# martinruenz/maskfusion

Measured on NVIDIA H100. Metric: frames/sec on 640x480 .klg replay, higher is better.
Workload: dtype f32

## Files before the change

maskfusion_b200/csrc/mf_capi.cu:

```cuda
#include "mf_host.h"
#include <string.h>
#include <stdio.h>
#include <zlib.h>
#include <limits.h>
#include <new>
#include <stack>

using namespace mfb;
namespace mfb { bool decodeJPEG(const uint8_t* data, size_t size, int& W, int& H, std::vector<uint8_t>& rgb, std::string& err); }

struct mf_context { MaskFusion* mf; };

static thread_local std::string g_err;
extern "C" const char* mf_last_error(void) { return g_err.c_str(); }
void mf_set_error(const std::string& e) { g_err = e; }
extern "C" int mf_abi_version(void) { return MF_ABI_VERSION; }

#define MF_TRY try {
#define MF_CATCH(ret)                                                              \
    } catch (const CudaError& e) { g_err = e.what; return ret; }                   \
    catch (const std::exception& e) { g_err = e.what(); return ret; }              \
    catch (...) { g_err = "unknown error"; return ret; }
static int mf_finalise(mf_context* ctx)
{
    try {
        cudaCheck(cudaSetDevice(ctx->mf->device), "cudaSetDevice");
        ctx->mf->finalisePending(); return 0;
    }
    catch (const CudaError& e) { g_err = e.what; return -1; }
    catch (...) { g_err = "unknown error"; return -1; }
}
#define MF_NEED(ctx) if (!(ctx) || !(ctx)->mf) { g_err = "null context"; return -1; } if (mf_finalise(ctx) != 0) return -1;
#define MF_MODEL(ctx, i) if ((i) < 0 || (i) >= (int)(ctx)->mf->models.size()) { g_err = "model index out of range"; return -2; } Model* m = (ctx)->mf->models[i].get();

#define MF_OWNED(m) if (!(m)->owned) { g_err = "model is owned by another rank (sharded mode): no device buffers here"; return -4; }

static Mat4 fromColMajor(const float* p) { Mat4 r; for (int rr = 0; rr < 4; ++rr) for (int c = 0; c < 4; ++c) r.m[rr * 4 + c] = p[c * 4 + rr]; return r; }
static void toColMajor(const Mat4& T, float* p) { for (int rr = 0; rr < 4; ++rr) for (int c = 0; c < 4; ++c) p[c * 4 + rr] = T.m[rr * 4 + c]; }

extern "C" void mf_config_defaults(mf_config* c, int width, int height)
{
    memset(c, 0, sizeof *c);
    c->width = width; c->height = height;
    if (width == 640 && height == 480) { c->fx = 528; c->fy = 528; c->cx = 320; c->cy = 240; }
    else { c->fx = 528.f * width / 640.f; c->fy = c->fx; c->cx = width / 2.f; c->cy = height / 2.f; }
    c->depthCutoff = 4.0f; c->maxDepthProcessed = 20.0f; c->icpWeight = 20.0f;
    c->rgbOnly = 0; c->pyramid = 1; c->fastOdom = 0; c->so3 = 1; c->frameToFrameRGB = 0;
    c->confGlobal = 10.0f; c->confObject = 0.01f;
    c->timeDelta = INT_MAX / 2;
    c->outlierCoeff = 0.1f;
    c->capacityGlobal = 3072 * 3072; c->capacityObject = 1024 * 1024;
    c->enableMultipleModels = 0; c->trackAllModels = 0; c->modelSpawnOffset = 22;
    c->minRelSizeNew = 0.015f; c->maxRelSizeNew = 0.4f;
    c->segThreshold = 0.3f; c->segWeightDistance = 150.f; c->segWeightConvexity = 2.8f;
    c->segMorphEdgeIterations = 0; c->segMorphEdgeRadius = 1; c->segMorphMaskIterations = 0; c->segMorphMaskRadius = 2;
}

extern "C" mf_context* mf_create(const mf_config* cfg, int device, void* stream)
{
    MF_TRY
    if (!cfg) { g_err = "null config"; return nullptr; }
    int n = 0;
    cudaError_t e = cudaGetDeviceCount(&n);
    if (e != cudaSuccess || n == 0) { g_err = std::string("no CUDA device: this library has no CPU fallback (") + cudaGetErrorString(e) + ")"; return nullptr; }
    mf_context* c = new mf_context;
    c->mf = new MaskFusion(*cfg, device, (cudaStream_t)stream);
    return c;
    MF_CATCH(nullptr)
}
extern "C" void mf_destroy(mf_context* ctx) { if (ctx) { delete ctx->mf; delete ctx; } }

extern "C" int mf_process_frame(mf_context* ctx, const uint8_t* rgb, const float* depth, int64_t ts, const uint8_t* mask, const float* in_pose,
                                float weight_multiplier, int bootstrap)
{
    MF_TRY MF_NEED(ctx)
    if (!rgb || !depth || ts < 0) { g_err = "processFrame: rgb/depth must be non-null and timestamp >= 0 (MaskFusion.cpp:201-203)"; return -3; }
    Mat4 ip; if (in_pose) ip = fromColMajor(in_pose);
    ctx->mf->processFrame(rgb, depth, ts, mask, in_pose ? &ip : nullptr, weight_multiplier, bootstrap != 0, false);
    return 0;
    MF_CATCH(-1)
}
extern "C" int mf_process_frame_device(mf_context* ctx, const void* d_rgb, const void* d_depth, int64_t ts, const void* d_mask, const float* in_pose,
                                       float weight_multiplier, int bootstrap)
{
    MF_TRY MF_NEED(ctx)
    if (!d_rgb || !d_depth || ts < 0) { g_err = "processFrame: rgb/depth must be non-null and timestamp >= 0"; return -3; }
    Mat4 ip; if (in_pose) ip = fromColMajor(in_pose);
    ctx->mf->processFrame((const uint8_t*)d_rgb, (const float*)d_depth, ts, (const uint8_t*)d_mask, in_pose ? &ip : nullptr, weight_multiplier,
                          bootstrap != 0, true);
    return 0;
    MF_CATCH(-1)
}
extern "C" int mf_set_input_event(mf_context* ctx, void* ev) { if (!ctx || !ctx->mf) { g_err = "null context"; return -1; } ctx->mf->inputReady = (cudaEvent_t)ev; return 0; }
extern "C" int mf_sync(mf_context* ctx) { MF_TRY MF_NEED(ctx) ctx->mf->sync(); return 0; MF_CATCH(-1) }
extern "C" int mf_tick(mf_context* ctx) { if (!ctx || !ctx->mf) return -1; return ctx->mf->tick; }
extern "C" int64_t mf_kernel_launches(mf_context* ctx) { if (!ctx || !ctx->mf) return -1; return ctx->mf->launches; }

extern "C" int mf_model_count(mf_context* ctx) { if (!ctx || !ctx->mf) return -1; return (int)ctx->mf->models.size(); }
extern "C" int mf_model_id(mf_context* ctx, int i) { MF_NEED(ctx) MF_MODEL(ctx, i) return m->id; }
extern "C" int mf_get_pose(mf_context* ctx, int i, float* p) { MF_NEED(ctx) MF_MODEL(ctx, i) toColMajor(m->pose, p); return 0; }
extern "C" int mf_set_pose(mf_context* ctx, int i, const float* p) { MF_NEED(ctx) MF_MODEL(ctx, i) m->overridePose(fromColMajor(p)); return 0; }
extern "C" int mf_model_set_conf_threshold(mf_context* ctx, int i, float t) { MF_NEED(ctx) MF_MODEL(ctx, i) m->confidenceThreshold = t; return 0; }
extern "C" int mf_model_surfel_count(mf_context* ctx, int i) { MF_TRY MF_NEED(ctx) MF_MODEL(ctx, i) return (int)m->lastCount(); MF_CATCH(-1) }

extern "C" int mf_download_surfels(mf_context* ctx, int i, float* out, int max_surfels)
{
    MF_TRY MF_NEED(ctx) MF_MODEL(ctx, i) MF_OWNED(m)
    MaskFusion* o = ctx->mf;
    uint32_t n = m->lastCount();
    if ((int)n > max_surfels) n = (uint32_t)max_surfels;
    if (!n) return 0;
    DevBuf<float4> tmp; tmp.alloc((size_t)n * 3);
    launch_planes_to_aos(m->current(), n, tmp, o->stream);
    cudaCheck(cudaMemcpyAsync(out, tmp.p, (size_t)n * 48, cudaMemcpyDeviceToHost, o->stream), "surfel D2H");
    o->sync();
    return (int)n;
    MF_CATCH(-1)
}
extern "C" int mf_upload_surfels(mf_context* ctx, int i, const float* in, int n)
{
    MF_TRY MF_NEED(ctx) MF_MODEL(ctx, i) MF_OWNED(m)
    MaskFusion* o = ctx->mf;
    if (n < 0 || (uint32_t)n > m->capacity) { g_err = "upload exceeds model capacity"; return -4; }
    if (n) {
        DevBuf<float4> tmp; tmp.alloc((size_t)n * 3);
        cudaCheck(cudaMemcpyAsync(tmp.p, in, (size_t)n * 48, cudaMemcpyHostToDevice, o->stream), "surfel H2D");
        launch_aos_to_planes(tmp, (uint32_t)n, m->current(), o->stream);
        o->sync();
    }
    uint32_t c = (uint32_t)n;
    cudaCheck(cudaMemcpyAsync(m->dCount(), &c, sizeof c, cudaMemcpyHostToDevice, o->stream), "count H2D");
    o->sync();
    return 0;
    MF_CATCH(-1)
}
extern "C" int mf_pose_log_size(mf_context* ctx, int i) { MF_NEED(ctx) MF_MODEL(ctx, i) return (int)(m->poseLog.size() / 8); }
extern "C" int mf_get_pose_log(mf_context* ctx, int i, double* out8, int max_entries)
{
    MF_NEED(ctx) MF_MODEL(ctx, i)
    int n = (int)(m->poseLog.size() / 8); if (n > max_entries) n = max_entries;
    memcpy(out8, m->poseLog.data(), (size_t)n * 8 * sizeof(double));
    return n;
}

extern "C" int mf_export_poses(mf_context* ctx, const char* export_dir)
{
    MF_TRY MF_NEED(ctx)
    if (!export_dir) { g_err = "export_poses: null directory"; return -2; }
    ctx->mf->sync();
    int written = 0;
    std::vector<Model*> all;
    for (auto& m : ctx->mf->models) all.push_back(m.get());
    for (auto& m : ctx->mf->inactiveModels) all.push_back(m.get());
    for (Model* m : all) {
        const std::string filename = std::string(export_dir) + "poses-" + std::to_string((int)m->id) + ".txt";
        FILE* fp = fopen(filename.c_str(), "w");
        if (!fp) { g_err = "cannot write " + filename; return -3; }
        for (size_t e = 0; e + 8 <= m->poseLog.size(); e += 8) {
            fprintf(fp, "%.6f", m->poseLog[e] * 1e-6);
            for (int k = 1; k < 8; ++k) fprintf(fp, " %.6f", (double)(float)m->poseLog[e + k]);
            fprintf(fp, "\n");
        }
        fclose(fp);
        ++written;
    }
    return written;
    MF_CATCH(-1)
}

extern "C" int mf_set_frame(mf_context* ctx, const uint8_t* rgb, const float* depth, const uint8_t* mask)
{
    MF_TRY MF_NEED(ctx)
    MaskFusion* o = ctx->mf;
    if (!mask) o->mask.zero(o->stream);
    o->setFrame(rgb, depth, mask, false);
    o->generateCUDATextures();
    return 0;
    MF_CATCH(-1)
}
extern "C" int mf_model_perform_tracking(mf_context* ctx, int i, float* transform16)
{
    MF_TRY MF_NEED(ctx) MF_MODEL(ctx, i) MF_OWNED(m)
    std::vector<Model*> ms{m};
    ctx->mf->trackModels(ms);
    ctx->mf->finalisePending();
    if (transform16) toColMajor(m->lastTransform, transform16);
    return 0;
    MF_CATCH(-1)
}
extern "C" int mf_model_predict_indices(mf_context* ctx, int i, int time)
{
    MF_TRY MF_NEED(ctx) MF_MODEL(ctx, i) MF_OWNED(m)
    m->predictIndices(time, ctx->mf->cfg.maxDepthProcessed, ctx->mf->cfg.timeDelta); return 0;
    MF_CATCH(-1)
}
extern "C" int mf_model_fuse(mf_context* ctx, int i, int time, float depth_cutoff, float weight_multiplier)
{
    MF_TRY MF_NEED(ctx) MF_MODEL(ctx, i) MF_OWNED(m)
    m->fuse(time, depth_cutoff, weight_multiplier); return 0;
    MF_CATCH(-1)
}
extern "C" int mf_model_clean(mf_context* ctx, int i, int time)
{
    MF_TRY MF_NEED(ctx) MF_MODEL(ctx, i) MF_OWNED(m)
    m->clean(time, ctx->mf->cfg.timeDelta, ctx->mf->cfg.maxDepthProcessed); return 0;
    MF_CATCH(-1)
}
extern "C" int mf_model_combined_predict(mf_context* ctx, int i, int time, int max_time)
{
    MF_TRY MF_NEED(ctx) MF_MODEL(ctx, i) MF_OWNED(m)
    m->combinedPredict(ctx->mf->cfg.maxDepthProcessed, time, max_time, ctx->mf->cfg.timeDelta); return 0;
    MF_CATCH(-1)
}
extern "C" int mf_model_init_from_frame(mf_context* ctx, int i, int time)
{
    MF_TRY MF_NEED(ctx) MF_MODEL(ctx, i) MF_OWNED(m)
    m->initialise(time); return 0;
    MF_CATCH(-1)
}

template <typename T>
static void d2h(MaskFusion* o, void* dst, const T* src, size_t n)
{
    if (!dst) return;
    cudaCheck(cudaMemcpyAsync(dst, src, n * sizeof(T), cudaMemcpyDeviceToHost, o->stream), "D2H");
}
static void planarOut(MaskFusion* o, const float4* map, int P, float* out)
{
    if (!out) return;
    launch_map_to_planar(map, P, o->scratch, o->stream);
    cudaCheck(cudaMemcpyAsync(out, o->scratch.p, (size_t)P * 3 * sizeof(float), cudaMemcpyDeviceToHost, o->stream), "D2H");
    o->sync();
}
extern "C" int mf_download_filtered_depth(mf_context* ctx, float* out)
{
    MF_TRY MF_NEED(ctx) d2h(ctx->mf, out, ctx->mf->depthFilt, ctx->mf->P); ctx->mf->sync(); return 0; MF_CATCH(-1)
}
extern "C" int mf_download_frame_maps(mf_context* ctx, int level, float* depth, float* vmap, float* nmap)
{
    MF_TRY MF_NEED(ctx)
    MaskFusion* o = ctx->mf;
    if (level < 0 || level > 2) { g_err = "level out of range"; return -2; }
    int Pl = (o->W >> level) * (o->H >> level);
    d2h(o, depth, level == 0 ? o->depthFilt : o->depthPyr[level].p, Pl); o->sync();
    planarOut(o, o->vmap[level], Pl, vmap);
    planarOut(o, o->nmap[level], Pl, nmap);
    return 0;
    MF_CATCH(-1)
}
extern "C" int mf_download_model_maps(mf_context* ctx, int i, int level, float* vmap, float* nmap)
{
    MF_TRY MF_NEED(ctx) MF_MODEL(ctx, i) MF_OWNED(m)
    MaskFusion* o = ctx->mf;
    if (level < 0 || level > 2) { g_err = "level out of range"; return -2; }
    int Pl = (o->W >> level) * (o->H >> level);
    planarOut(o, m->vmapG[level], Pl, vmap);
    planarOut(o, m->nmapG[level], Pl, nmap);
    return 0;
    MF_CATCH(-1)
}
extern "C" int mf_download_index_map(mf_context* ctx, int i, uint32_t* idx, float* vc, float* ct, float* nr)
{
    MF_TRY MF_NEED(ctx) MF_MODEL(ctx, i) MF_OWNED(m)
    MaskFusion* o = ctx->mf;
    m->flushIndex();
    d2h(o, idx, m->idx.p, o->P); d2h(o, vc, m->vertConf.p, o->P); d2h(o, ct, m->colorTime.p, o->P); d2h(o, nr, m->normRad.p, o->P);
    o->sync(); return 0;
    MF_CATCH(-1)
}
extern "C" int mf_download_prediction(mf_context* ctx, int i, uint8_t* image4, float* vc, float* nr, uint16_t* time)
{
    MF_TRY MF_NEED(ctx) MF_MODEL(ctx, i) MF_OWNED(m)
    MaskFusion* o = ctx->mf;
    d2h(o, image4, m->splatImage.p, o->P); d2h(o, vc, m->splatVertex.p, o->P); d2h(o, nr, m->splatNormal.p, o->P); d2h(o, time, m->splatTime.p, o->P);
    o->sync(); return 0;
    MF_CATCH(-1)
}
extern "C" int mf_download_fill_in(mf_context* ctx, int i, uint8_t* image4, float* v4, float* n4)
{
    MF_TRY MF_NEED(ctx) MF_MODEL(ctx, i) MF_OWNED(m)
    MaskFusion* o = ctx->mf;
    if (!m->fillIn) { g_err = "model has no fill-in textures"; return -5; }
    d2h(o, image4, m->fillImage.p, o->P); d2h(o, v4, m->fillVertex.p, o->P); d2h(o, n4, m->fillNormal.p, o->P);
    o->sync(); return 0;
    MF_CATCH(-1)
}
extern "C" int mf_download_association(mf_context* ctx, int i, uint8_t* flag, uint32_t* best, float* meas12)
{
    MF_TRY MF_NEED(ctx) MF_MODEL(ctx, i) MF_OWNED(m)
    MaskFusion* o = ctx->mf;
    d2h(o, flag, m->aflag.p, o->P); d2h(o, best, m->abest.p, o->P);
    if (meas12) {
        DevBuf<float4> tmp; tmp.alloc((size_t)o->P * 3);
        launch_planes_to_aos(SurfelPlanes{m->meas[0].p, m->meas[1].p, m->meas[2].p}, (uint32_t)o->P, tmp, o->stream);
        cudaCheck(cudaMemcpyAsync(meas12, tmp.p, (size_t)o->P * 48, cudaMemcpyDeviceToHost, o->stream), "D2H");
        o->sync();
    }
    o->sync(); return 0;
    MF_CATCH(-1)
}
extern "C" int mf_download_track_stats(mf_context* ctx, int i, double* A36, double* b6, float* err6)
{
    MF_TRY MF_NEED(ctx) MF_MODEL(ctx, i) MF_OWNED(m)
    MaskFusion* o = ctx->mf;
    TrackState st;
    cudaCheck(cudaMemcpyAsync(&st, m->trackState.p, sizeof st, cudaMemcpyDeviceToHost, o->stream), "D2H");
    o->sync();
    if (A36) memcpy(A36, st.lastA, sizeof st.lastA);
    if (b6) memcpy(b6, st.lastb, sizeof st.lastb);
    if (err6) { err6[0] = st.lastICPError; err6[1] = st.lastICPCount; err6[2] = st.lastRGBError; err6[3] = st.lastRGBCount; err6[4] = st.lastSO3Error; err6[5] = st.lastSO3Count; }
    return 0;
    MF_CATCH(-1)
}
extern "C" int mf_download_edge_map(mf_context* ctx, float* edge, uint8_t* binary)
{
    MF_TRY MF_NEED(ctx)
    MaskFusion* o = ctx->mf;
    if (!o->frameMapsValid) o->generateCUDATextures();
    launch_geometric_edges(o->vmap[0], o->nmap[0], o->W, o->H, o->cfg.segWeightDistance, o->cfg.segWeightConvexity, o->cfg.segThreshold,
                           o->edgeMap, o->edgeBinary, o->stream);
    launch_morph_close_invert(o->edgeBinary, o->edgeBuf, o->W, o->H, o->cfg.segMorphEdgeRadius, o->cfg.segMorphEdgeIterations, o->edgeInv, o->stream);
    o->launches += 2 + 2 * o->cfg.segMorphEdgeIterations;
    d2h(o, edge, o->edgeMap.p, o->P); d2h(o, binary, o->edgeInv.p, o->P);
    o->sync(); return 0;
    MF_CATCH(-1)
}

extern "C" int mf_morph_close(mf_context* ctx, uint8_t* image, int radius, int iterations, int ellipse, uint8_t* inverted)
{
    MF_TRY MF_NEED(ctx)
    if (!image || radius < 0 || iterations < 0) { g_err = "morph_close: bad arguments"; return -3; }
    MaskFusion* o = ctx->mf;
    DevBuf<uint8_t> a, b, c; a.alloc(o->P); b.alloc(o->P); c.alloc(o->P);
    cudaCheck(cudaMemcpyAsync(a.p, image, o->P, cudaMemcpyHostToDevice, o->stream), "H2D");
    if (ellipse) o->launches += launch_morph_close_ellipse(a, b, o->W, o->H, radius, iterations, nullptr, o->stream);
    else { launch_morph_close_invert(a, b, o->W, o->H, radius, iterations, c, o->stream); o->launches += 1 + 2 * iterations; }
    d2h(o, image, a.p, o->P);
    if (inverted && !ellipse) d2h(o, inverted, c.p, o->P);
    o->sync(); return 0;
    MF_CATCH(-1)
}

extern "C" int mf_attach_backbone(mf_context* ctx, void* backbone, int every_k)
{
    MF_TRY MF_NEED(ctx)
    ctx->mf->attachBackbone(backbone, every_k); return 0;
    MF_CATCH(-1)
}

extern "C" int mf_attach_detector(mf_context* ctx, mf_detector* detector, int every_k)
{
    MF_TRY MF_NEED(ctx)
    ctx->mf->attachDetector(detector, every_k); return 0;
    MF_CATCH(-1)
}
extern "C" int mf_download_frame_masks(mf_context* ctx, uint8_t* mask, int32_t* class_ids_256, int* n_masks)
{
    MF_TRY MF_NEED(ctx)
    MaskFusion* o = ctx->mf;
    if (!o->cfg.enableMultipleModels) { g_err = "not a multi-model context"; return -5; }
    FrameHdr h;
    cudaCheck(cudaMemcpyAsync(&h, o->dHdr, sizeof h, cudaMemcpyDeviceToHost, o->stream), "D2H");
    d2h(o, mask, o->frameMask, o->P);
    o->sync();
    if (mask && h.nMasks == 0) memset(mask, 0, o->P);
    if (class_ids_256) memcpy(class_ids_256, h.classIDs, sizeof h.classIDs);
    if (n_masks) *n_masks = h.nMasks;
    return 0;
    MF_CATCH(-1)
}

extern "C" int mf_debug_track_timing(int64_t* out, int cap) { return debug_track_timing((long long*)out, cap); }

extern "C" int mf_set_frame_classes(mf_context* ctx, const int32_t* class_ids, int n)
{
    MF_TRY MF_NEED(ctx)
    if (n < 0 || n > 256) { g_err = "class id list must have 0..256 entries"; return -3; }
    ctx->mf->setFrameClasses(class_ids, n);
    return 0;
    MF_CATCH(-1)
}
extern "C" int mf_download_segmentation(mf_context* ctx, uint8_t* mask, uint8_t* projected_ids)
{
    MF_TRY MF_NEED(ctx)
    MaskFusion* o = ctx->mf;
    d2h(o, mask, o->mask.p, o->P);
    if (projected_ids) { if (!o->projectedIDs.p) { g_err = "not a multi-model context"; return -5; } d2h(o, projected_ids, o->projectedIDs.p, o->P); }
    o->sync(); return 0;
    MF_CATCH(-1)
}
extern "C" int mf_shard_configure(mf_context* ctx, int rank, int world) { MF_TRY MF_NEED(ctx) ctx->mf->configureShard(rank, world); return 0; MF_CATCH(-1) }
extern "C" int mf_shard_frame_begin(mf_context* ctx, const void* rgb, const void* depth, int64_t ts, const void* mask, int on_device)
{
    MF_TRY MF_NEED(ctx)
    if (!rgb || !depth || ts < 0) { g_err = "frame_begin: rgb/depth must be non-null and timestamp >= 0"; return -3; }
    ctx->mf->frameBegin((const uint8_t*)rgb, (const float*)depth, ts, (const uint8_t*)mask, nullptr, false, on_device != 0);
    return 0;
    MF_CATCH(-1)
}
extern "C" int mf_shard_get_poses(mf_context* ctx, float* out, int capacity_models)
{
    MF_TRY MF_NEED(ctx)
    if (capacity_models < MF_MAX_MODELS) { g_err = "get_poses: the buffer must hold 64 rows of 32 floats"; return -2; }
    ctx->mf->getShardPoses(out);
    return (int)ctx->mf->models.size();
    MF_CATCH(-1)
}
extern "C" int mf_shard_unique_id(uint8_t* out128)
{
    MF_TRY
    if (!out128) { g_err = "null buffer"; return -1; }
    shardUniqueId(out128); return 0;
    MF_CATCH(-1)
}
extern "C" int mf_shard_comm_init(mf_context* ctx, const uint8_t* id128, int rank, int world)
{
    MF_TRY MF_NEED(ctx)
    if (!id128) { g_err = "null id"; return -1; }
    ctx->mf->initShardComm(id128, rank, world); return 0;
    MF_CATCH(-1)
}
extern "C" int mf_shard_process_frame(mf_context* ctx, const uint8_t* rgb, const float* depth, int64_t ts, const uint8_t* mask, const int32_t* class_ids,
                                      int n_class_ids, float weight_multiplier, int inputs_on_device)
{
    MF_TRY MF_NEED(ctx)
    MaskFusion* o = ctx->mf;
    if (!o->shardNccl) { g_err = "mf_shard_process_frame needs a communicator (mf_shard_comm_init)"; return -2; }
    if (o->rank == 0) {
        if (!rgb || !depth || ts < 0) { g_err = "processFrame: rgb/depth must be non-null and timestamp >= 0 on the loader rank"; return -3; }
        if (n_class_ids < 0 || n_class_ids > 256) { g_err = "class id list must have 0..256 entries"; return -3; }
        o->setFrameClasses(class_ids, class_ids ? n_class_ids : 0);
    }
    o->processFrame(rgb, depth, ts, mask, nullptr, weight_multiplier, false, inputs_on_device != 0);
    return 0;
    MF_CATCH(-1)
}
extern "C" int mf_shard_stats(mf_context* ctx, int64_t* out4)
{
    if (!ctx || !ctx->mf || !out4) { g_err = "null argument"; return -1; }
    MaskFusion* o = ctx->mf;
    out4[0] = (int64_t)o->shard.bytesMoved; out4[1] = o->shard.calls; out4[2] = o->shardNccl ? o->shard.world : 0; out4[3] = o->shard.version;
    return 0;
}
extern "C" int mf_shard_set_poses(mf_context* ctx, const float* gathered) { MF_TRY MF_NEED(ctx) ctx->mf->setShardPoses(gathered); return 0; MF_CATCH(-1) }
extern "C" int mf_shard_project(mf_context* ctx) { MF_TRY MF_NEED(ctx) ctx->mf->frameProject(); return 0; MF_CATCH(-1) }
extern "C" void* mf_shard_projection_keys(mf_context* ctx) { if (!ctx || !ctx->mf) return nullptr; return ctx->mf->projKeys.p; }
extern "C" int mf_shard_frame_end(mf_context* ctx, float weight_multiplier) { MF_TRY MF_NEED(ctx) ctx->mf->frameEnd(weight_multiplier); return 0; MF_CATCH(-1) }
extern "C" int mf_shard_attach_detector(mf_context* ctx, mf_detector* detector, int every_k, int detector_rank)
{
    MF_TRY MF_NEED(ctx)
    ctx->mf->attachShardDetector(detector, every_k, detector_rank); return 0;
    MF_CATCH(-1)
}
extern "C" int mf_shard_frame_masks(mf_context* ctx, void** d_ptr, size_t* bytes)
{
    MF_TRY MF_NEED(ctx)
    if (!d_ptr || !bytes) { g_err = "frame_masks: null output"; return -3; }
    void* p = nullptr; size_t n = 0;
    if (!ctx->mf->shardFrameMasks(&p, &n)) return 0;
    *d_ptr = p; *bytes = n;
    return 1;
    MF_CATCH(-1)
}
extern "C" int mf_model_owner(mf_context* ctx, int i) { MF_NEED(ctx) MF_MODEL(ctx, i) return m->ownerRank; }
extern "C" int mf_track_shares(int n_jobs, unsigned light_mask, int total_ctas, int ratio, int* shares)
{
    if (!shares || n_jobs < 1 || n_jobs > TRACK_MAX_JOBS || total_ctas < n_jobs) return -1;
    track_shares(n_jobs, light_mask, total_ctas, ratio, shares);
    return 0;
}
extern "C" int mf_shard_pick_owner(const int64_t* loads, int world) { if (!loads || world < 1 || world > 64) return -1; return MaskFusion::pickOwner(loads, world); }

extern "C" int mf_model_class_id(mf_context* ctx, int i) { MF_NEED(ctx) MF_MODEL(ctx, i) return m->classID; }
extern "C" int mf_set_profiling(mf_context* ctx, int on)
{
    MF_TRY MF_NEED(ctx)
    ctx->mf->sync();
    ctx->mf->prof.on = on != 0; ctx->mf->prof.used = 0;
    if (on) ctx->mf->prof.acc.clear();
    return 0;
    MF_CATCH(-1)
}
extern "C" int mf_get_stage_times(mf_context* ctx, char* buf, int bufsize)
{
    MF_TRY MF_NEED(ctx)
    ctx->mf->sync();
    std::string out;
    char line[256];
    for (auto& kv : ctx->mf->prof.acc) { snprintf(line, sizeof line, "%s %ld %.6f\n", kv.first.c_str(), kv.second.first, kv.second.second); out += line; }
    if ((int)out.size() + 1 > bufsize) { g_err = "buffer too small"; return -6; }
    memcpy(buf, out.c_str(), out.size() + 1);
    return (int)out.size();
    MF_CATCH(-1)
}
extern "C" int mf_debug_set_poses(mf_context* ctx, int i, const float* pose16, const float* last16)
{
    MF_NEED(ctx) MF_MODEL(ctx, i)
    m->pose = fromColMajor(pose16); m->lastPose = fromColMajor(last16);
    m->pushPose();
    return 0;
}
extern "C" int mf_icp_step(mf_context* ctx, int i, int level, const float* Rcurr9, const float* tcurr3, float* out29)
{
    MF_TRY MF_NEED(ctx) MF_MODEL(ctx, i) MF_OWNED(m)
    MaskFusion* o = ctx->mf;
    if (level < 0 || level > 2) { g_err = "level out of range"; return -2; }
    TrackPoses pp; memset(&pp, 0, sizeof pp);
    memcpy(pp.p[0], Rcurr9, 9 * sizeof(float)); memcpy(pp.p[0] + 9, tcurr3, 3 * sizeof(float));
    const float* P = m->pose.m;
    float R[9] = {P[0], P[1], P[2], P[4], P[5], P[6], P[8], P[9], P[10]};
    float c00 = R[4] * R[8] - R[5] * R[7], c01 = R[5] * R[6] - R[3] * R[8], c02 = R[3] * R[7] - R[4] * R[6];
    float det = (R[0] * c00 + R[1] * c01) + R[2] * c02, id = 1.0f / det;
    float Ri[9] = {c00 * id, (R[2] * R[7] - R[1] * R[8]) * id, (R[1] * R[5] - R[2] * R[4]) * id,
                   c01 * id, (R[0] * R[8] - R[2] * R[6]) * id, (R[2] * R[3] - R[0] * R[5]) * id,
                   c02 * id, (R[1] * R[6] - R[0] * R[7]) * id, (R[0] * R[4] - R[1] * R[3]) * id};
    memcpy(pp.p[1], Ri, sizeof Ri); pp.p[1][9] = P[3]; pp.p[1][10] = P[7]; pp.p[1][11] = P[11];
    DevBuf<float> out; out.alloc(32);
    DevBuf<unsigned> ticket; ticket.alloc(1); ticket.zero(o->stream);
    launch_icp_only(o->vmap[level], o->nmap[level], m->vmapG[level], m->nmapG[level], o->W >> level, o->H >> level, camLevel(o->cam, level), pp,
                    m->partial, ticket, out, o->numSMs, o->stream);
    o->launches += 1;
    cudaCheck(cudaMemcpyAsync(out29, out.p, 29 * sizeof(float), cudaMemcpyDeviceToHost, o->stream), "D2H");
    o->sync();
    return 0;
    MF_CATCH(-1)
}

struct mf_klg {
    FILE* fp; int W, H, numFrames, currentFrame; int flip;
    std::vector<unsigned char> dbuf, rbuf, dec;
};
extern "C" mf_klg* mf_klg_open(const char* path, int width, int height, int flip_colors)
{
    if (!path) { g_err = "mf_klg_open: null path"; return nullptr; }
    if (width <= 0 || height <= 0 || width > 16384 || height > 16384) { g_err = "mf_klg_open: width/height must be in 1..16384"; return nullptr; }
    FILE* fp = fopen(path, "rb");
    if (!fp) { g_err = std::string("Could not open log-file: ") + path; return nullptr; }
    int32_t n = 0;
    if (!fread(&n, sizeof(int32_t), 1, fp)) { fclose(fp); g_err = std::string("Could not open log-file: ") + path; return nullptr; }
    mf_klg* k = nullptr;
    try {
        k = new mf_klg;
        k->fp = fp; k->W = width; k->H = height; k->numFrames = n; k->currentFrame = 0; k->flip = flip_colors;
        size_t P = (size_t)width * height;
        k->dbuf.resize(P * 2 + 1024); k->rbuf.resize(P * 3 + 1024); k->dec.resize(P * 2);
    } catch (...) { fclose(fp); delete k; g_err = "mf_klg_open: out of memory"; return nullptr; }
    return k;
}
extern "C" int mf_klg_num_frames(mf_klg* k) { return k ? k->numFrames : -1; }
extern "C" int mf_klg_has_more(mf_klg* k) { return k ? (k->currentFrame + 1 < k->numFrames) : 0; }
extern "C" int mf_klg_get_next(mf_klg* k, uint8_t* rgb, float* depth, int64_t* timestamp)
{
    if (!k || !rgb || !depth) { g_err = "mf_klg_get_next: null reader or output buffer"; return -1; }
    MF_TRY
    const size_t P = (size_t)k->W * k->H;
    int64_t ts; int32_t dsz, rsz;
    if (!fread(&ts, sizeof ts, 1, k->fp) || !fread(&dsz, sizeof dsz, 1, k->fp) || !fread(&rsz, sizeof rsz, 1, k->fp)) { g_err = "klg: truncated frame header"; return -2; }
    if (dsz < 0 || rsz < 0 || (size_t)dsz > k->dbuf.size() || (size_t)rsz > k->rbuf.size()) { g_err = "klg: implausible frame sizes"; return -3; }
    if (dsz && !fread(k->dbuf.data(), dsz, 1, k->fp)) { g_err = "klg: truncated depth"; return -2; }
    if (rsz > 0 && !fread(k->rbuf.data(), rsz, 1, k->fp)) { g_err = "klg: truncated rgb"; return -2; }
    const uint16_t* d16 = (const uint16_t*)k->dbuf.data();
    if ((size_t)dsz != P * 2) {
        unsigned long len = (unsigned long)(P * 2);
        if (uncompress(k->dec.data(), &len, k->dbuf.data(), (unsigned long)dsz) != Z_OK) { g_err = "klg: zlib depth decode failed"; return -4; }
        d16 = (const uint16_t*)k->dec.data();
    }
    for (size_t i = 0; i < P; ++i) depth[i] = (float)((double)d16[i] * 0.001);
    if (rsz > 0) {
        if ((size_t)rsz != P * 3) {
            int jw = 0, jh = 0; std::vector<uint8_t> dec; std::string err;
            if (!mfb::decodeJPEG(k->rbuf.data(), (size_t)rsz, jw, jh, dec, err)) { g_err = "klg: " + err; return -5; }
            if (jw != k->W || jh != k->H) { g_err = "klg: JPEG frame size differs from the reader's resolution"; return -5; }
            for (size_t i = 0; i < P * 3; i += 3) { rgb[i] = dec[i + 2]; rgb[i + 1] = dec[i + 1]; rgb[i + 2] = dec[i]; }
        } else memcpy(rgb, k->rbuf.data(), P * 3);
    } else memset(rgb, 0, P * 3);
    if (k->flip) for (size_t i = 0; i < P * 3; i += 3) { uint8_t t = rgb[i]; rgb[i] = rgb[i + 2]; rgb[i + 2] = t; }
    if (timestamp) *timestamp = ts;
    k->currentFrame++;
    return 0;
    MF_CATCH(-6)
}
extern "C" void mf_klg_close(mf_klg* k) { if (k) { if (k->fp) fclose(k->fp); delete k; } }
extern "C" int mf_klg_write(const char* path, int width, int height, int num_frames, const int64_t* timestamps, const uint16_t* depth_mm, const uint8_t* rgb)
{
    if (!path || width <= 0 || height <= 0 || num_frames < 0 || (num_frames > 0 && (!timestamps || !depth_mm || !rgb))) { g_err = "mf_klg_write: bad arguments"; return -1; }
    FILE* fp = fopen(path, "wb");
    if (!fp) { g_err = std::string("cannot write ") + path; return -1; }
    const size_t P = (size_t)width * height;
    int32_t n = num_frames, dsz = (int32_t)(P * 2), rsz = (int32_t)(P * 3);
    fwrite(&n, sizeof n, 1, fp);
    for (int f = 0; f < num_frames; ++f) {
        fwrite(&timestamps[f], sizeof(int64_t), 1, fp);
        fwrite(&dsz, sizeof dsz, 1, fp); fwrite(&rsz, sizeof rsz, 1, fp);
        fwrite(depth_mm + (size_t)f * P, 2, P, fp);
        fwrite(rgb + (size_t)f * P * 3, 1, P * 3, fp);
    }
    fclose(fp);
// ... 3 lines not shown
```

maskfusion_b200/csrc/mf_common.cuh:

```cuda
#pragma once
#include <cuda_runtime.h>
#include <stdint.h>
#include <math.h>

#define MF_HD __host__ __device__ __forceinline__
#define MF_D __device__ __forceinline__

namespace mfb {

struct Cam { float fx, fy, cx, cy; };
MF_HD Cam camLevel(Cam c, int level) {
    int div = 1 << level;
    return Cam{c.fx / div, c.fy / div, c.cx / div, c.cy / div};
}

struct Rt { float m[12]; };

MF_D float qnanf() { return __int_as_float(0x7fffffff); }

MF_D float3 xform(const Rt& T, float3 p) {
    return make_float3(((T.m[0] * p.x + T.m[1] * p.y) + T.m[2] * p.z) + T.m[3],
                       ((T.m[4] * p.x + T.m[5] * p.y) + T.m[6] * p.z) + T.m[7],
                       ((T.m[8] * p.x + T.m[9] * p.y) + T.m[10] * p.z) + T.m[11]);
}
MF_D float3 rotate(const Rt& T, float3 n) {
    return make_float3((T.m[0] * n.x + T.m[1] * n.y) + T.m[2] * n.z,
                       (T.m[4] * n.x + T.m[5] * n.y) + T.m[6] * n.z,
                       (T.m[8] * n.x + T.m[9] * n.y) + T.m[10] * n.z);
}
MF_D float dot3(float3 a, float3 b) { return (a.x * b.x + a.y * b.y) + a.z * b.z; }
MF_D float3 cross3(float3 a, float3 b) {
    return make_float3(a.y * b.z - a.z * b.y, a.z * b.x - a.x * b.z, a.x * b.y - a.y * b.x);
}
MF_D float3 normalize3(float3 v) {
    float l = sqrtf(dot3(v, v));
    return make_float3(v.x / l, v.y / l, v.z / l);
}
MF_D float3 sub3(float3 a, float3 b) { return make_float3(a.x - b.x, a.y - b.y, a.z - b.z); }
MF_D float3 add3(float3 a, float3 b) { return make_float3(a.x + b.x, a.y + b.y, a.z + b.z); }

MF_D float det_expf(float x) {
    const float xin = x;
    x = fminf(fmaxf(x, -87.0f), 88.0f);
    float t = x * 1.44269504088896341f;
    float n = floorf(t + 0.5f);
    float r = (x - n * 0.693359375f) - n * (-2.12194440e-4f);
    float p = 1.9875691500e-4f;
    p = p * r + 1.3981999507e-3f;
    p = p * r + 8.3334519073e-3f;
    p = p * r + 4.1665795894e-2f;
    p = p * r + 1.6666665459e-1f;
    p = p * r + 5.0000001201e-1f;
    float r2 = r * r;
    float y = (p * r2 + r) + 1.0f;
    float res = y * __int_as_float((uint32_t)((int)n + 127) << 23);
    if (xin > 88.0f) res = __int_as_float(0x7f800000);
    if (!(xin > -87.0f)) res = (xin != xin) ? xin : 0.0f;
    return res;
}
MF_D float det_acosf(float x) {
    float a = fabsf(x);
    if (!(a <= 1.0f)) return qnanf();
    float p = -0.0012624911f;
    p = p * a + 0.0066700901f;
    p = p * a + -0.0170881256f;
    p = p * a + 0.0308918810f;
    p = p * a + -0.0501743046f;
    p = p * a + 0.0889789874f;
    p = p * a + -0.2145988016f;
    p = p * a + 1.5707963050f;
    float r = sqrtf(1.0f - a) * p;
    return x < 0.0f ? 3.14159265358979f - r : r;
}

MF_D float encodeColor(float r, float g, float b) {
    int rgb = (int)floorf(r * 255.0f + 0.5f);
    rgb = (rgb << 8) + (int)floorf(g * 255.0f + 0.5f);
    rgb = (rgb << 8) + (int)floorf(b * 255.0f + 0.5f);
    return (float)rgb;
}
MF_D float3 decodeColor(float c) {
    int ci = (int)c;
    return make_float3((float)((ci >> 16) & 0xFF) / 255.0f, (float)((ci >> 8) & 0xFF) / 255.0f, (float)(ci & 0xFF) / 255.0f);
}
MF_D float surfelRadius(float depth, float norm_z, float ifx, float ify) {
    float meanFocal = ((1.0f / fabsf(ifx)) + (1.0f / fabsf(ify))) / 2.0f;
    float radius = (depth / meanFocal) * 1.41421356237f;
    float radius_n = radius / fabsf(norm_z);
    float r2 = 2.0f * radius;
    return r2 < radius_n ? r2 : radius_n;
}
MF_D float surfelConfidence(float x, float y, float weighting, float cx, float cy) {
    float px = x - cx, py = y - cy;
    float radialDist = sqrtf(px * px + py * py) / 400.0f;
    return det_expf((-(radialDist * radialDist) / 0.72f)) * weighting;
}

MF_D int clampi(int v, int lo, int hi) { return v < lo ? lo : (v > hi ? hi : v); }

MF_D float4 ldStream(const float4* p) {
    float4 r;
    asm volatile("ld.global.nc.L1::no_allocate.v4.f32 {%0,%1,%2,%3}, [%4];" : "=f"(r.x), "=f"(r.y), "=f"(r.z), "=f"(r.w) : "l"(p));
    return r;
}
MF_D void stStream(float4* p, float4 v) {
    asm volatile("st.global.L1::no_allocate.v4.f32 [%0], {%1,%2,%3,%4};" ::"l"(p), "f"(v.x), "f"(v.y), "f"(v.z), "f"(v.w) : "memory");
}

constexpr uint64_t KEY_EMPTY = ~0ull;

}
```

maskfusion_b200/csrc/mf_host.cu:

```cuda
#include "mf_host.h"
#include <math.h>
#include <float.h>
#include <string.h>
#include <stdio.h>
#include <limits.h>
#include <stdlib.h>

namespace mfb {

void cudaCheck(cudaError_t e, const char* where)
{
    if (e != cudaSuccess) throw CudaError{std::string(where) + ": " + cudaGetErrorString(e)};
}

Profiler* g_prof = nullptr;
void prof_mark(cudaStream_t s, const char* name)
{
    Profiler* p = g_prof;
    if (!p || !p->on) return;
    if (p->used == (int)p->events.size()) {
        cudaEvent_t e; cudaEventCreate(&e); p->events.push_back(e); p->names.push_back(nullptr);
    }
    p->names[p->used] = name;
    cudaEventRecord(p->events[p->used], s);
    p->used++;
}
void Profiler::resolve()
{
    for (int i = 0; i + 1 < used; ++i) {
        if (!names[i]) continue;
        float ms = 0;
        if (cudaEventElapsedTime(&ms, events[i], events[i + 1]) == cudaSuccess) { auto& a = acc[names[i]]; a.first += 1; a.second += ms; }
    }
    used = 0;
}

Mat4 rigidInverse(const Mat4& T)
{
    Mat4 o = Mat4::identity();
    const float* m = T.m;
    float R[9] = {m[0], m[1], m[2], m[4], m[5], m[6], m[8], m[9], m[10]}, t[3] = {m[3], m[7], m[11]};
    for (int r = 0; r < 3; ++r) {
        for (int c = 0; c < 3; ++c) o.m[r * 4 + c] = R[c * 3 + r];
        o.m[r * 4 + 3] = -((R[0 * 3 + r] * t[0] + R[1 * 3 + r] * t[1]) + R[2 * 3 + r] * t[2]);
    }
    return o;
}
Mat4 mul(const Mat4& A, const Mat4& B)
{
    Mat4 o;
    for (int r = 0; r < 4; ++r)
        for (int c = 0; c < 4; ++c) {
            float s = 0;
            for (int k = 0; k < 4; ++k) s += A.m[r * 4 + k] * B.m[k * 4 + c];
            o.m[r * 4 + c] = s;
        }
    return o;
}
Rt toRt(const Mat4& T) { Rt r; for (int i = 0; i < 12; ++i) r.m[i] = T.m[i]; return r; }

static void rodrigues2(const float* R, float* out)
{
    double rx = R[7] - R[5], ry = R[2] - R[6], rz = R[3] - R[1];
    double s = sqrt((rx * rx + ry * ry + rz * rz) * 0.25);
    double c = ((double)(R[0] + R[4] + R[8]) - 1) * 0.5;
    c = c > 1. ? 1. : c < -1. ? -1. : c;
    double theta = acos(c);
    if (s < 1e-5) {
        double t;
        if (c > 0) rx = ry = rz = 0;
        else {
            t = (R[0] + 1) * 0.5; rx = sqrt(t > 0 ? t : 0.0);
            t = (R[4] + 1) * 0.5; ry = sqrt(t > 0 ? t : 0.0) * (R[1] < 0 ? -1.0 : 1.0);
            t = (R[8] + 1) * 0.5; rz = sqrt(t > 0 ? t : 0.0) * (R[2] < 0 ? -1.0 : 1.0);
            if (fabs(rx) < fabs(ry) && fabs(rx) < fabs(rz) && (R[5] > 0) != (ry * rz > 0)) rz = -rz;
            theta /= sqrt(rx * rx + ry * ry + rz * rz);
            rx *= theta; ry *= theta; rz *= theta;
        }
    } else {
        double vth = 1 / (2 * s); vth *= theta; rx *= vth; ry *= vth; rz *= vth;
    }
    out[0] = (float)rx; out[1] = (float)ry; out[2] = (float)rz;
}

static void rotToQuat(const float* R, float* q)
{
    float t = R[0] + R[4] + R[8];
    if (t > 0) {
        t = sqrtf(t + 1.0f); q[3] = 0.5f * t; t = 0.5f / t;
        q[0] = (R[7] - R[5]) * t; q[1] = (R[2] - R[6]) * t; q[2] = (R[3] - R[1]) * t;
    } else {
        int i = 0; if (R[4] > R[0]) i = 1; if (R[8] > R[i * 4]) i = 2;
        int j = (i + 1) % 3, k = (j + 1) % 3;
        t = sqrtf(R[i * 4] - R[j * 4] - R[k * 4] + 1.0f);
        q[i] = 0.5f * t; t = 0.5f / t;
        q[3] = (R[k * 3 + j] - R[j * 3 + k]) * t;
        q[j] = (R[j * 3 + i] + R[i * 3 + j]) * t;
        q[k] = (R[k * 3 + i] + R[i * 3 + k]) * t;
    }
}

Model::Model(MaskFusion* o, unsigned char id_, float conf, bool enableFillIn, int cap, int ownerRank_, bool ghost)
    : owner(o), ownerRank(ownerRank_), owned(!ghost), id(id_), pose(Mat4::identity()), lastPose(Mat4::identity()), initialC2Winv(Mat4::identity()),
      confidenceThreshold(conf), maxDepth(FLT_MAX), fillIn(enableFillIn), capacity((uint32_t)cap), lastTransform(Mat4::identity())
{
    const int W = o->W, H = o->H, P = o->P;
    cudaStream_t s = o->stream;
    if (ghost) return;
    pos[0].alloc(capacity); col[0].alloc(capacity); nrm[0].alloc(capacity);
    count.alloc(2); count.zero(s);
    cudaCheck(cudaMallocHost((void**)&hCount, 2 * sizeof(uint32_t)), "cudaMallocHost"); hCount[0] = hCount[1] = 0;
    cudaCheck(cudaMallocHost((void**)&hTrackOut, 40 * sizeof(float)), "cudaMallocHost");
    key.alloc(P); launch_fill_u64(key, KEY_EMPTY, P, s);
    idx.alloc(P); vertConf.alloc(P); colorTime.alloc(P); normRad.alloc(P); cleanTex.alloc((size_t)P); cleanTex.zero(s);
    idx.zero(s); vertConf.zero(s); colorTime.zero(s); normRad.zero(s);
    splatImage.alloc(P); splatVertex.alloc(P); splatNormal.alloc(P); splatTime.alloc(P);
    splatImage.zero(s); splatVertex.zero(s); splatNormal.zero(s); splatTime.zero(s);
    nonBlack.alloc(1); nonBlack.zero(s);
    if (fillIn) { fillImage.alloc(P); fillVertex.alloc(P); fillNormal.alloc(P); fillImage.zero(s); fillVertex.zero(s); fillNormal.zero(s); }
    aflag.alloc(P); abest.alloc(P); aflag.zero(s); abest.zero(s);
    for (int k = 0; k < 3; ++k) { meas[k].alloc(P); meas[k].zero(s); }
    slot.alloc(capacity); launch_fill_u32(slot, 0xffffffffu, capacity, s);
    keep.alloc((size_t)capacity + P);
    size_t nblk = ((size_t)capacity + P + 511) / 512 + 1;
    blockSums.alloc(nblk); blockSums2.alloc(nblk);
    cleanTicket.alloc(4); cleanTicket.zero(s); cleanLoaded.alloc(nblk); cleanLoaded.zero(s);
    cudaCheck(cudaMallocHost((void**)&hCleanStat, 2 * sizeof(uint32_t)), "cudaMallocHost"); hCleanStat[0] = hCleanStat[1] = 0;
    cand.alloc((size_t)capacity + P); candCount.alloc(1); candCount.zero(s);
    for (int l = 0; l < 3; ++l) {
        size_t Pl = (size_t)(W >> l) * (H >> l);
        vmapG[l].alloc(Pl); nmapG[l].alloc(Pl); cloud[l].alloc(Pl); lastDepth[l].alloc(Pl); lastImage[l].alloc(Pl); corres[l].alloc(l == 0 ? Pl + (size_t)o->numSMs * 512 : 1);
        vmapG[l].zero(s); nmapG[l].zero(s); lastDepth[l].zero(s); lastImage[l].zero(s);
    }
    if (id_ != 0) for (int l = 0; l < 3; ++l) { validBits[l].alloc(((size_t)(W >> l) * (H >> l) + 31) / 32 + 1); validBits[l].zero(s); }
    lastNextImage2.alloc((size_t)(W >> 2) * (H >> 2)); lastNextImage2.zero(s);
    trackState.alloc(1); trackState.zero(s);
    partial.alloc((size_t)TRACK_MAX_BLOCKS * 128); partial.zero(s);
    dpose.alloc(1); pushPose();
    o->launches += 3;
}

void Model::pushPose()
{
    if (!owned || !dpose.p) return;
    launch_set_pose(dpose, pose.m, lastPose.m, owner->stream);
    owner->launches += 1;
}

Model::~Model()
{
    if (hCount) cudaFreeHost(hCount);
    if (hTrackOut) cudaFreeHost(hTrackOut);
    if (hCleanStat) cudaFreeHost(hCleanStat);
}

unsigned Model::lastCount()
{
    if (!owned) throw CudaError{"model is owned by another rank (sharded mode): no surfel store here"};
    cudaCheck(cudaMemcpyAsync(hCount, dCount(), sizeof(uint32_t), cudaMemcpyDeviceToHost, owner->stream), "count D2H");
    owner->sync();
    return hCount[0];
}

void Model::initialise(int time)
{
    MaskFusion* o = owner;
    launch_init_model(o->rgb, o->depthRaw, o->depthFilt, o->cam, o->W, o->H, time, o->cfg.maxDepthProcessed, o->initFlagR, o->initFlagF,
                      blockSums, blockSums2, capacity, current(), dCount(), o->stream);
    o->launches += 5;
}

void Model::prepareTracking()
{
    MaskFusion* o = owner;
    cudaStream_t s = o->stream;
    const int W = o->W, H = o->H;
    float denom = (float)((H / 20) * (W / 20));
    float4* v[3] = {vmapG[0].p, vmapG[1].p, vmapG[2].p};
    float4* n[3] = {nmapG[0].p, nmapG[1].p, nmapG[2].p};
    const uint32_t* nb = fillIn ? nonBlack.p : nullptr;
    launch_model_maps(splatVertex, splatNormal, fillIn ? fillVertex.p : splatVertex.p, fillIn ? fillNormal.p : splatNormal.p, nb, denom, W, H,
                      dpose, 6.0f , v, n, lastDepth[0], s);
    o->launches += 1;
    if (validBits[0].p) {
        uint32_t* b3[3] = {validBits[0].p, validBits[1].p, validBits[2].p};
        launch_valid_bits3(n, W, H, b3, s);
        o->launches += 1;
    }
    const bool rgb = o->cfg.rgbOnly || o->cfg.icpWeight < 100;
    if (rgb) {
        launch_intensity_select(splatImage, fillIn ? fillImage.p : splatImage.p, nb, denom, (o->cfg.frameToFrameRGB && fillIn) ? 1 : 0, o->P, lastImage[0], s);
        launch_pyrdown2_pair(lastDepth[0], lastDepth[1], lastDepth[2], lastImage[0], lastImage[1], lastImage[2], W, H, s);
        const float* d3[3] = {lastDepth[0].p, lastDepth[1].p, lastDepth[2].p};
        float4* c3[3] = {cloud[0].p, cloud[1].p, cloud[2].p};
        launch_project_points3(d3, W, H, o->cam, c3, s);
        o->launches += 3;
    }
}

float Model::computeFusionWeight(float weightMultiplier) const
{
    Mat4 diff = mul(rigidInverse(pose), lastPose);
    const float* d = diff.m;
    float R[9] = {d[0], d[1], d[2], d[4], d[5], d[6], d[8], d[9], d[10]};
    float tn = sqrtf((d[3] * d[3] + d[7] * d[7]) + d[11] * d[11]);
    float rv[3]; rodrigues2(R, rv);
    float rn = sqrtf((rv[0] * rv[0] + rv[1] * rv[1]) + rv[2] * rv[2]);
    float weighting = tn > rn ? tn : rn;
    const float largest = 0.01f, minWeight = 0.5f;
    if (weighting > largest) weighting = largest;
    float w = 1.0f - (weighting / largest);
    return (w > minWeight ? w : minWeight) * weightMultiplier;
}

void Model::predictIndices(int time, float depthCutoff, int timeDelta, bool forClean)
{
    MaskFusion* o = owner;
    if (forClean) {
        idxDeferred = true; idxTime = time; idxDelta = timeDelta; idxDepth = depthCutoff;
        return;
    }
    idxDeferred = false;
    launch_predict_indices(current(), dCount(), dpose, o->cam, o->W, o->H, depthCutoff, time, timeDelta, key, idx, vertConf,
                           colorTime, normRad, forClean ? cleanTex.p : nullptr, confidenceThreshold, o->stream);
    if (forClean) { cleanTexTime = time; cleanTexConf = confidenceThreshold; }
    o->launches += 2;
}

void Model::flushIndex()
{
    if (!idxDeferred) return;
    idxDeferred = false;
    MaskFusion* o = owner;
    launch_predict_indices(current(), dCount(), dpose, o->cam, o->W, o->H, idxDepth, idxTime, idxDelta, key, idx, vertConf, colorTime, normRad, cleanTex.p, confidenceThreshold, o->stream);
    cleanTexTime = idxTime; cleanTexConf = confidenceThreshold;
    o->launches += 2;
}

void Model::fuse(int time, float depthCutoff, float weightMultiplier)
{
    MaskFusion* o = owner;
    flushIndex();
    float md = depthCutoff < maxDepth ? depthCutoff : maxDepth;
    float4* m[3] = {meas[0].p, meas[1].p, meas[2].p};
    launch_associate(o->rgb, o->depthRaw, o->depthFilt, o->mask, idx, vertConf, normRad, dpose, o->cam, o->W, o->H, md, time,
                     weightMultiplier, id, aflag, abest, m, slot, o->stream);
    launch_fuse_update(aflag, abest, m, slot, o->P, time, current(), o->stream);
    o->launches += 3;
}

void Model::clean(int time, int timeDelta, float )
{
    MaskFusion* o = owner;
    float4* m[3] = {meas[0].p, meas[1].p, meas[2].p};
    bool pingPong = false;
    if (capacity >= (1u << 20) && hCleanStat[1] > 0) {
        const uint32_t first = hCleanStat[0], nb = hCleanStat[1];
        pingPong = first < nb && (uint64_t)(nb - first) * 10 > (uint64_t)nb * 4;
    }
    if (pingPong && !pos[1 - target].p) { pos[1 - target].alloc(capacity); col[1 - target].alloc(capacity); nrm[1 - target].alloc(capacity); }
    int other = pingPong ? 1 - target : target, otherCount = 1 - countSel;
    const bool fused = idxDeferred && idxTime == time && idxDelta == timeDelta && (size_t)capacity + (size_t)o->P < 0x80000000ull;
    if (!fused) flushIndex();
    IndexFused f{key.p, idx.p, vertConf.p, colorTime.p, normRad.p, cleanTex.p, idxDepth};
    idxDeferred = false;
    const bool packedOK = fused || (cleanTexTime == time && cleanTexConf == confidenceThreshold);
    CleanWindowImages win{packedOK ? cleanTex.p : nullptr, vertConf.p, colorTime.p, idx.p};
    if (++cleanEpoch == 0) ++cleanEpoch;
    CleanInPlace ip{cleanTicket.p, cleanLoaded.p, cleanTicket.p + 1, cleanEpoch, pingPong};
    launch_clean(planes(target), planes(other), dCount(), count.p + otherCount, capacity, aflag, m, dpose, o->cam, o->W, o->H,
                 time, timeDelta, confidenceThreshold, o->cfg.outlierCoeff, id, win, o->depthFilt, o->mask, keep, blockSums,
                 cand, candCount, o->stream, ip, fused ? &f : nullptr);
    if (capacity >= (1u << 20))
        cudaCheck(cudaMemcpyAsync(hCleanStat, cleanTicket.p + 1, 2 * sizeof(uint32_t), cudaMemcpyDeviceToHost, o->stream), "clean statistic D2H");
    target = other; countSel = otherCount;
    o->launches += fused ? 6 : 5;
}

void Model::combinedPredict(float depthCutoff, int time, int maxTime, int timeDelta)
{
    MaskFusion* o = owner;
    launch_combined_predict(current(), dCount(), dpose, o->cam, o->W, o->H, depthCutoff, confidenceThreshold, time, maxTime,
                            timeDelta, o->rayTab, key, splatImage, splatVertex, splatNormal, splatTime, fillIn ? 1 : 0, o->depthFilt, o->rgb, 0,
                            o->cfg.frameToFrameRGB ? 1 : 0, fillImage, fillVertex, fillNormal, fillIn ? nonBlack.p : nullptr, o->stream, capacity);
    o->launches += 2;
}

MaskFusion::MaskFusion(const mf_config& c, int dev, cudaStream_t st) : cfg(c), device(dev)
{
    cudaCheck(cudaSetDevice(dev), "cudaSetDevice");
    cudaDeviceProp prop;
    cudaCheck(cudaGetDeviceProperties(&prop, dev), "cudaGetDeviceProperties");
    numSMs = prop.multiProcessorCount;
    set_num_sms(numSMs);
    W = c.width; H = c.height; P = W * H;
    if (W % 4 || H % 4) throw CudaError{"width and height must be multiples of 4 (3-level pyramid)"};
    cam = Cam{c.fx, c.fy, c.cx, c.cy};
    ownStream = (st == nullptr);
    if (ownStream) cudaCheck(cudaStreamCreateWithFlags(&stream, cudaStreamNonBlocking), "cudaStreamCreate"); else stream = st;
    g_prof = &prof;
    for (int k = 0; k < 2; ++k) { inBuf[k].alloc(packetBytes()); inBuf[k].zero(stream); rgbBuf[k].alloc(P); depthFiltBuf[k].alloc(P); }
    selectSet(0);
    mask.alloc(P); mask.zero(stream);
    cudaCheck(cudaStreamCreateWithFlags(&preStream, cudaStreamNonBlocking), "cudaStreamCreate");
    cudaCheck(cudaEventCreateWithFlags(&preDone, cudaEventDisableTiming), "cudaEventCreate");
    cudaCheck(cudaEventCreateWithFlags(&inputsCopied, cudaEventDisableTiming), "cudaEventCreate");
    cudaCheck(cudaEventCreateWithFlags(&evMain, cudaEventDisableTiming), "cudaEventCreate");
    cudaCheck(cudaEventCreateWithFlags(&evComm, cudaEventDisableTiming), "cudaEventCreate");
    for (int l = 0; l < 3; ++l) {
        size_t Pl = (size_t)(W >> l) * (H >> l);
        if (l > 0) depthPyr[l].alloc(Pl);
        vmap[l].alloc(Pl); nmap[l].alloc(Pl); nextImage[l].alloc(Pl); nextGrad[l].alloc(Pl); rgbValid[l].alloc(Pl);
    }
    edgeMap.alloc(P); edgeBinary.alloc(P); edgeBuf.alloc(P); edgeInv.alloc(P);
    dJobs.alloc(TRACK_MAX_JOBS);
    cudaCheck(cudaMallocHost((void**)&hJobs, TRACK_MAX_JOBS * sizeof(TrackJob)), "cudaMallocHost");
    initFlagR.alloc(P); initFlagF.alloc(P);
    scratch.alloc((size_t)P * 4);
    rayTab.alloc(P); launch_ray_table(cam, W, H, rayTab, stream);
    if (c.enableMultipleModels) {
        dRes.alloc(1); dRes.zero(stream);
        cudaCheck(cudaMallocHost((void**)&hRes, sizeof(FrameResult)), "cudaMallocHost"); memset(hRes, 0, sizeof(FrameResult));
        cudaCheck(cudaEventCreateWithFlags(&resEvt, cudaEventDisableTiming), "cudaEventCreate");
        poseTable.alloc((size_t)MF_MAX_MODELS * 32); poseTable.zero(stream);
        gathered.alloc((size_t)64 * MF_MAX_MODELS * 32); gathered.zero(stream);
        compModel.alloc(((size_t)P / 2 + 2) * MF_MAX_MODELS); compMask.alloc(((size_t)P / 2 + 2) * 256);
        projKeys.alloc(P); launch_fill_u64(projKeys, KEY_EMPTY, P, stream); projectedIDs.alloc(P); projectedIDs.zero(stream);
        ccL.alloc(P); ccDense.alloc(P); ccLabA.alloc(P); ccLabB.alloc(P); ccArea.alloc((size_t)P + 1); ccBox.alloc(((size_t)P / 2 + 2) * 4); mapToMask.alloc((size_t)P / 2 + 2); absorbId.alloc((size_t)P / 2 + 2);
        maskPixels.alloc(256); ccCounter.alloc(1); ccCounter.zero(stream);
        segTmp.alloc(P); ignoreMap.alloc(P); ignoreMap.zero(stream);
        tblIdToIndex.alloc(256); tblIndexToId.alloc(256); tblIsModel.alloc(256); tblMaskToID.alloc(256); tblIsPerson.alloc(256);
        tblIdToIndex.zero(stream); tblIndexToId.zero(stream); tblIsModel.zero(stream); tblIsPerson.zero(stream);
        tblMaskToID.zero(stream); cudaCheck(cudaMemsetAsync(tblMaskToID.p + 255, 255, 1, stream), "memset");
        maskOverlap.alloc((size_t)MF_MAX_MODELS * 256);
    }
    models.emplace_back(new Model(this, nextID++, c.confGlobal, true, c.capacityGlobal));
    sync();
}

MaskFusion::~MaskFusion()
{
    if (detector && bbMoldDone) cudaEventSynchronize(bbMoldDone);
    cudaStreamSynchronize(stream);
    if (g_prof == &prof) g_prof = nullptr;
    for (cudaEvent_t e : prof.events) cudaEventDestroy(e);
    if (trackDone) cudaEventDestroy(trackDone);
    if (preStream) { cudaStreamSynchronize(preStream); cudaStreamDestroy(preStream); }
    if (preDone) cudaEventDestroy(preDone);
    if (inputsCopied) cudaEventDestroy(inputsCopied);
    if (evMain) cudaEventDestroy(evMain);
    if (evComm) cudaEventDestroy(evComm);
    models.clear();
    inactiveModels.clear();
    if (hJobs) cudaFreeHost(hJobs);
    if (hRes) cudaFreeHost(hRes);
    if (resEvt) cudaEventDestroy(resEvt);
    if (bbFrameReady) cudaEventDestroy(bbFrameReady);
    if (bbMoldDone) cudaEventDestroy(bbMoldDone);
    if (ownStream) cudaStreamDestroy(stream);
}

void MaskFusion::sync()
{
    if (prof.on) prof_mark(stream, nullptr);
    cudaCheck(cudaStreamSynchronize(stream), "cudaStreamSynchronize");
    if (prof.on) prof.resolve();
    finalisePending();
}

void MaskFusion::uploadInputs(const uint8_t* rgbIn, const float* depthIn, const uint8_t* maskIn, int64_t timestamp, bool onDevice, cudaStream_t s)
{
    if (!s) s = stream;
    cudaMemcpyKind kind = onDevice ? cudaMemcpyDeviceToDevice : cudaMemcpyHostToDevice;
    g_prof = &prof;
    prof_mark(s, onDevice ? "copy_d2d_frame" : "copy_h2d_frame");
    if (onDevice && inputReady) { cudaCheck(cudaStreamWaitEvent(s, inputReady, 0), "cudaStreamWaitEvent"); inputReady = nullptr; }
    cudaCheck(cudaMemcpyAsync(rgb3, rgbIn, (size_t)P * 3, kind, s), "rgb upload");
    cudaCheck(cudaMemcpyAsync(depthRaw, depthIn, (size_t)P * sizeof(float), kind, s), "depth upload");
    if (cfg.enableMultipleModels) {
        FrameHdr h; memset(&h, 0, sizeof h);
        h.timestamp = timestamp;
        h.maskGiven = maskIn != nullptr;
        if (maskIn && !classIDs.empty()) {
            if (classIDs.size() > 256) throw CudaError{"more than 256 mask labels"};
            cudaCheck(cudaMemcpyAsync(frameMask, maskIn, (size_t)P, kind, s), "mask upload");
            h.nMasks = (int)classIDs.size();
            for (size_t i = 0; i < classIDs.size(); ++i) h.classIDs[i] = classIDs[i];
        }
        launch_frame_header(h, dHdr, s);
        launches += 1;
    }
    if (!onDevice) { cudaCheck(cudaEventRecord(inputsCopied, s), "cudaEventRecord"); copyPending = true; }
    else if (s != stream) { cudaCheck(cudaEventRecord(inputsCopied, s), "cudaEventRecord"); cudaCheck(cudaStreamWaitEvent(stream, inputsCopied, 0), "cudaStreamWaitEvent"); }
}

void MaskFusion::preprocess(cudaStream_t s)
{
    if (!s) s = stream;
    launch_unpack_rgb(rgb3, rgb, P, s);
    launch_bilateral(depthRaw, depthFilt, W, H, s);
    launches += 2;
    frameMapsValid = false; intensityValid = false;
}

void MaskFusion::setFrame(const uint8_t* rgbIn, const float* depthIn, const uint8_t* maskIn, bool onDevice, cudaStream_t s)
{
    if (!s) s = stream;
    if (maskIn) cudaCheck(cudaMemcpyAsync(mask, maskIn, (size_t)P, onDevice ? cudaMemcpyDeviceToDevice : cudaMemcpyHostToDevice, s), "mask upload");
    uploadInputs(rgbIn, depthIn, nullptr, 0, onDevice, s);
    preprocess(s);
}

void MaskFusion::generateCUDATextures(cudaStream_t s)
{
    if (!s) s = stream;
    const float* d[3] = {depthFilt, depthPyr[1].p, depthPyr[2].p};
    float4* v3[3] = {vmap[0].p, vmap[1].p, vmap[2].p};
    float4* n3[3] = {nmap[0].p, nmap[1].p, nmap[2].p};
    launch_pyrdown2_f(depthFilt, W, H, depthPyr[1], depthPyr[2], s);
    launch_vmap_nmap3(d, W, H, cam, cfg.depthCutoff, v3, n3, s);
    launches += 2;
    frameMapsValid = true;
}

void MaskFusion::frameIntensity(cudaStream_t s)
{
    if (!s) s = stream;
    const bool rgbTerm = cfg.rgbOnly || cfg.icpWeight < 100;
    launch_intensity(rgb, P, nextImage[0], s);
    launch_pyrdown2_u8(nextImage[0], W, H, nextImage[1], nextImage[2], s);
    launches += 2;
    if (rgbTerm) {
        const uint8_t* i3[3] = {nextImage[0].p, nextImage[1].p, nextImage[2].p};
        short2* g3[3] = {nextGrad[0].p, nextGrad[1].p, nextGrad[2].p};
        uint8_t* r3[3] = {rgbValid[0].p, rgbValid[1].p, rgbValid[2].p};
        launch_sobel3(i3, W, H, g3, r3, s);
        launches += 1;
    }
    intensityValid = true;
}

void MaskFusion::trackModels(const std::vector<Model*>& ms, bool viaResult)
{
    if (ms.empty()) return;
    if ((int)ms.size() > TRACK_MAX_JOBS) throw CudaError{"too many tracked models for one batch"};
    const bool rgbTerm = cfg.rgbOnly || cfg.icpWeight < 100;
    if (!frameMapsValid) generateCUDATextures();
    if ((rgbTerm || cfg.so3) && !intensityValid) frameIntensity();
    unsigned lightMask = 0;
    for (size_t j = 0; j < ms.size(); ++j) {
        Model* m = ms[j];
        if (!viaResult) m->lastPose = m->pose;
        m->prepareTracking();
        TrackJob& J = hJobs[j];
        for (int l = 0; l < 3; ++l) {
            J.vmapC[l] = vmap[l]; J.nmapC[l] = nmap[l]; J.nextImage[l] = nextImage[l]; J.nextGrad[l] = nextGrad[l]; J.rgbValid[l] = rgbValid[l];
            J.vmapG[l] = m->vmapG[l]; J.nmapG[l] = m->nmapG[l]; J.lastDepth[l] = m->lastDepth[l]; J.lastImage[l] = m->lastImage[l];
            J.cloud[l] = m->cloud[l]; J.corres[l] = m->corres[l];
        }
        J.lastNextImage2 = m->lastNextImage2; J.st = m->trackState; J.partial = m->partial;
        J.dpose = m->dpose;
        for (int l = 0; l < 3; ++l) J.validBits[l] = m->validBits[l].p;
        if (J.validBits[0] != nullptr) lightMask |= 1u << j;
    }
    if (preWaitPending) {
        cudaCheck(cudaStreamWaitEvent(stream, preDone, 0), "cudaStreamWaitEvent");
        preWaitPending = false;
    }
    prof_mark(stream, "copy_jobs");
    cudaCheck(cudaMemcpyAsync(dJobs, hJobs, ms.size() * sizeof(TrackJob), cudaMemcpyHostToDevice, stream), "jobs upload");
    launches += launch_tracking(dJobs, (int)ms.size(), W, H, cam, cfg.rgbOnly != 0, cfg.icpWeight, cfg.pyramid != 0, cfg.fastOdom != 0,
                                cfg.so3 != 0, numSMs, stream, lightMask);
    prof_mark(stream, "copy_pose_d2h");
    for (Model* m : ms) {
        if (!viaResult)
            cudaCheck(cudaMemcpyAsync(m->hTrackOut, (const char*)m->trackState.p + offsetof(TrackState, out), 40 * sizeof(float),
                                      cudaMemcpyDeviceToHost, stream), "pose D2H");
        if (cfg.so3)
            cudaCheck(cudaMemcpyAsync(m->lastNextImage2, nextImage[2], (size_t)(W >> 2) * (H >> 2), cudaMemcpyDeviceToDevice, stream), "so3 swap");
    }
    if (viaResult) return;
    if (!trackDone) cudaCheck(cudaEventCreateWithFlags(&trackDone, cudaEventDisableTiming), "cudaEventCreate");
    cudaCheck(cudaEventRecord(trackDone, stream), "cudaEventRecord");
    pendingModels = ms; pendingTrack = true;
}

void MaskFusion::finalisePending()
{
    if (pendingTrack) {
        cudaCheck(cudaEventSynchronize(trackDone), "cudaEventSynchronize");
        for (Model* m : pendingModels) {
            memcpy(m->pose.m, m->hTrackOut, 16 * sizeof(float));
            memcpy(m->lastTransform.m, m->hTrackOut + 16, 16 * sizeof(float));
        }
        pendingTrack = false; pendingModels.clear();
    }
    if (pendingResult) applyFrameResult();
    if (pendingLog) { pendingLog = false; logPoses(pendingTimestamp); }
}

void MaskFusion::logPoses(int64_t timestamp)
{
    Model* g = models[0].get();
    for (size_t i = 0; i < models.size(); ++i) {
        Model* m = models[i].get();
        Mat4 T = (i == 0) ? g->pose : mul(g->pose, rigidInverse(m->pose));
        float R[9] = {T.m[0], T.m[1], T.m[2], T.m[4], T.m[5], T.m[6], T.m[8], T.m[9], T.m[10]}, q[4];
        rotToQuat(R, q);
        double e[8] = {(double)timestamp, T.m[3], T.m[7], T.m[11], q[0], q[1], q[2], q[3]};
        m->poseLog.insert(m->poseLog.end(), e, e + 8);
    }
}

void MaskFusion::predict()
{
    for (auto& m : models) if (m->owned) m->combinedPredict(cfg.maxDepthProcessed, tick, tick, cfg.timeDelta);
}

void MaskFusion::globalProjection() { segTables(); projectLocal(); projectResolve(); }

void MaskFusion::segTables()
{
    if (models.size() > MF_MAX_MODELS - 1) throw CudaError{"global projection / segmentation support up to 63 models"};
    SegTables t; memset(&t, 0, sizeof t);
    for (size_t i = 0; i < models.size(); ++i) { t.idToIndex[models[i]->id] = (uint8_t)i; t.indexToId[i] = models[i]->id; t.isModel[models[i]->id] = 1; }
    launch_seg_tables(t, tblIdToIndex, tblIndexToId, tblIsModel, stream);
    launches += 1;
}

void MaskFusion::projectLocal()
{
    if (models.size() > MF_MAX_MODELS - 1) throw CudaError{"global projection supports up to 63 models"};
    for (size_t i = 0; i < models.size(); ++i) {
        Model* m = models[i].get();
        if (!m->owned) continue;
        launch_splat_project_only(m->current(), m->dCount(), m->dpose, cam, W, H, cfg.depthCutoff, 12.0f , tick, tick,
                                  cfg.timeDelta, (uint32_t)i << 26, rayTab, projKeys, stream, m->capacity);
        launches += 1;
    }
}

void MaskFusion::projectResolve()
{
    launch_proj_resolve(projKeys, P, tblIndexToId, projectedIDs, stream);
    launches += 1;
}

void MaskFusion::performSegmentation(bool allowNew)
{
    const int nModels = (int)models.size();
    if (!frameMapsValid) generateCUDATextures();
    launch_geometric_edges(vmap[0], nmap[0], W, H, cfg.segWeightDistance, cfg.segWeightConvexity, cfg.segThreshold, edgeMap, edgeBinary, stream);
    launch_morph_close_invert(edgeBinary, edgeBuf, W, H, cfg.segMorphEdgeRadius, cfg.segMorphEdgeIterations, edgeInv, stream);
    launches += 2 + 2 * cfg.segMorphEdgeIterations;
    if (detWaitPending) { cudaCheck(cudaStreamWaitEvent(stream, bbMoldDone, 0), "cudaStreamWaitEvent"); detWaitPending = false; }
    if (maskCommPending) { cudaCheck(cudaStreamWaitEvent(stream, evComm, 0), "cudaStreamWaitEvent"); maskCommPending = false; }
    launch_person_table(dHdr, personClassID, tblIsPerson, stream);
    launch_apply_ignore(frameMask, tblIsPerson, dHdr, P, ignoreMap, edgeInv, stream);
    launch_cc(edgeInv, W, H, ccL, ccDense, ccLabA, ccArea, ccBox, ccCounter, stream);
    launch_remove_edges(ccLabA, ccLabB, depthRaw, ccArea, W, H, 5, stream);
    int* lab = ccLabB;
    launch_clear_hist(ccCounter, dHdr, nModels, compModel, compMask, stream);
    maskPixels.zero(stream);
// ... 444 lines not shown
```

maskfusion_b200/csrc/mf_host.h:

```cpp
#pragma once
#include <cuda_runtime.h>
#include <stdint.h>
#include <memory>
#include <string>
#include <vector>
#include <map>
#include "../../include/maskfusion_b200.h"
#include "mf_kernels.h"

namespace mfb {

struct Mat4 {
    float m[16];
    static Mat4 identity() { Mat4 r; for (int i = 0; i < 16; ++i) r.m[i] = (i % 5 == 0) ? 1.f : 0.f; return r; }
};
Mat4 rigidInverse(const Mat4& T);
Mat4 mul(const Mat4& A, const Mat4& B);
Rt toRt(const Mat4& T);

struct Profiler {
    bool on = false; int used = 0;
    std::vector<cudaEvent_t> events; std::vector<const char*> names;
    std::map<std::string, std::pair<long, double>> acc;
    void resolve();
};
extern Profiler* g_prof;

class MaskFusion;

struct ShardComm {
    void* comm = nullptr; int rank = 0, world = 1, version = 0; size_t bytesMoved = 0; long calls = 0;
    ~ShardComm();
    void init(const unsigned char* id128, int rank, int world);
    void broadcast(void* buf, size_t bytes, int root, cudaStream_t s);
    void allGatherFloats(const float* send, float* recv, size_t countPerRank, cudaStream_t s);
    void allReduceMinU64(uint64_t* buf, size_t count, cudaStream_t s);
};
void shardUniqueId(unsigned char* out128);
void launch_pack_rows(const LifeParams& lp, float* table, cudaStream_t s);
void launch_lifecycle(const LifeParams& lp, const float* gathered, FrameResult* res, cudaStream_t s);
void launch_set_count(uint32_t* c, uint32_t v, cudaStream_t s);

class Model {
public:
    Model(MaskFusion* owner, unsigned char id, float confidenceThresh, bool enableFillIn, int capacity, int ownerRank = 0, bool ghost = false);
    ~Model();
    Model(const Model&) = delete;

    void initialise(int time);
    void prepareTracking();
    void predictIndices(int time, float depthCutoff, int timeDelta, bool forClean = true);
    void fuse(int time, float depthCutoff, float weightMultiplier);
    void clean(int time, int timeDelta, float depthCutoff);
    void combinedPredict(float depthCutoff, int time, int maxTime, int timeDelta);
    float computeFusionWeight(float weightMultiplier) const;
    void overridePose(const Mat4& p) { lastPose = pose; pose = p; pushPose(); }
    void makeStatic(const Mat4& globalPose) { initialC2Winv = mul(pose, rigidInverse(globalPose)); isStatic = true; }
    void updateStaticPose(const Mat4& globalPose) { overridePose(mul(initialC2Winv, globalPose)); }
    void pushPose();
    bool allowsFillIn() const { return fillIn; }
    unsigned lastCount();
    SurfelPlanes planes(int b) const { return SurfelPlanes{pos[b].p, col[b].p, nrm[b].p}; }
    SurfelPlanes current() const { return planes(target); }
    uint32_t* dCount() const { return count.p + countSel; }

    MaskFusion* owner;
    int ownerRank = 0; bool owned = true;
    unsigned char id; int classID = -1;
    Mat4 pose, lastPose, initialC2Winv;
    bool isStatic = false, nonstatic = false; unsigned age = 0;
    float confidenceThreshold, maxDepth;
    bool fillIn;
    uint32_t capacity;
    int target = 0, countSel = 0;
    DevBuf<float4> pos[2], col[2], nrm[2];
    DevBuf<uint32_t> count;
    uint32_t* hCount = nullptr;
    DevBuf<uint64_t> key;
    DevBuf<uint32_t> idx; DevBuf<float4> vertConf, colorTime, normRad, cleanTex;
    DevBuf<uchar4> splatImage, fillImage; DevBuf<float4> splatVertex, splatNormal, fillVertex, fillNormal; DevBuf<uint16_t> splatTime;
    DevBuf<uint32_t> nonBlack;
    DevBuf<uint8_t> aflag; DevBuf<uint32_t> abest; DevBuf<float4> meas[3]; DevBuf<uint32_t> slot;
    DevBuf<uint8_t> keep; DevBuf<uint32_t> blockSums, blockSums2, cand, candCount;
    uint32_t* hCleanStat = nullptr;
    DevBuf<uint32_t> cleanTicket, cleanLoaded; uint32_t cleanEpoch = 0;
    DevBuf<float4> vmapG[3], nmapG[3], cloud[3];
    DevBuf<float> lastDepth[3]; DevBuf<uint8_t> lastImage[3]; DevBuf<uint8_t> lastNextImage2;
    DevBuf<DataTerm> corres[3];
    DevBuf<uint32_t> validBits[3];
    DevBuf<TrackState> trackState; DevBuf<float> partial;
    DevBuf<DevPose> dpose;
    float* hTrackOut = nullptr;
    Mat4 lastTransform;
    std::vector<double> poseLog;
    bool tracked = false;
    bool idxDeferred = false; int idxTime = 0, idxDelta = 0; float idxDepth = 0.f;
    int cleanTexTime = -1; float cleanTexConf = -1.f;
    void flushIndex();
};

class MaskFusion {
public:
    MaskFusion(const mf_config& cfg, int device, cudaStream_t stream);
    ~MaskFusion();

    bool processFrame(const uint8_t* rgb, const float* depth, int64_t timestamp, const uint8_t* mask, const Mat4* inPose,
                      float weightMultiplier, bool bootstrap, bool inputsOnDevice);
    void setFrame(const uint8_t* rgb, const float* depth, const uint8_t* mask, bool onDevice, cudaStream_t s = nullptr);
    void uploadInputs(const uint8_t* rgb, const float* depth, const uint8_t* mask, int64_t timestamp, bool onDevice, cudaStream_t s = nullptr);
    void preprocess(cudaStream_t s = nullptr);
    void generateCUDATextures(cudaStream_t s = nullptr);
    void frameIntensity(cudaStream_t s = nullptr);
    void trackModels(const std::vector<Model*>& ms, bool viaResult = false);
    void predict();
    void sync();
    void finalisePending();
    void logPoses(int64_t timestamp);
    bool pendingTrack = false, pendingLog = false; int64_t pendingTimestamp = 0; std::vector<Model*> pendingModels; cudaEvent_t trackDone = nullptr;
    void globalProjection();
    void segTables();
    void performSegmentation(bool allowNew);
    unsigned char getNextModelID(bool assign);
    Model* spawnObjectModel();
    void setFrameClasses(const int32_t* ids, int n) { classIDs.assign(ids, ids + n); }

    void configureShard(int rank, int world);
    void initShardComm(const unsigned char* id128, int rank, int world);
    void frameBegin(const uint8_t* rgb, const float* depth, int64_t timestamp, const uint8_t* mask, const Mat4* inPose, bool bootstrap, bool onDevice);
    void getShardPoses(float* out);
    void setShardPoses(const float* gathered);
    void frameProject();
    void frameEnd(float weightMultiplier);
    void applyFrameResult();
    LifeParams lifeParams() const;
    ShardComm shard; bool shardNccl = false;
    void* backbone = nullptr; int backboneEvery = 0; cudaEvent_t bbFrameReady = nullptr, bbMoldDone = nullptr; bool bbMoldPending = false;
    void attachBackbone(void* bb, int everyK);
    void runBackbone(cudaStream_t producer = nullptr);
    mf_detector* detector = nullptr; int detectorEvery = 0; bool detWaitPending = false;
    void attachDetector(mf_detector* det, int everyK);
    void runDetector(cudaStream_t producer, bool wanted);
    void waitDetector();
    int detRank = -1; bool fExchange = false, maskCommPending = false;
    void attachShardDetector(mf_detector* det, int everyK, int detectorRank);
    bool shardFrameMasks(void** ptr, size_t* bytes);
    bool spawnedInApply = false, commOnPre = false; cudaEvent_t evMain = nullptr, evComm = nullptr;
    FrameResult* hRes = nullptr; DevBuf<FrameResult> dRes; cudaEvent_t resEvt = nullptr; bool pendingResult = false;
    DevBuf<float> poseTable, gathered;
    float fWeight = 1.f; int fTick = 0; bool fTracked = false;
    std::vector<std::unique_ptr<Model>> inactiveModels;
    bool enableSmartModelDelete = true; unsigned modelKeepMinSurfels = 4000; float modelKeepConfThreshold = 0.3f;
    void projectLocal(); void projectResolve();
    static int pickOwner(const int64_t* loads, int world);
    int rank = 0, world = 1;
    int64_t fTimestamp = 0; Mat4 fInPose; bool fHasPose = false, fBootstrap = false;

    mf_config cfg; Cam cam; int W, H, P; int device; cudaStream_t stream; bool ownStream;
    int numSMs = 132;
    int tick = 1;
    int64_t launches = 0;
    std::vector<std::unique_ptr<Model>> models;
    unsigned char nextID = 0;
    DevBuf<uint8_t> inBuf[2]; DevBuf<uchar4> rgbBuf[2]; DevBuf<float> depthFiltBuf[2];
    uint8_t* rgb3 = nullptr; uchar4* rgb = nullptr; float* depthRaw = nullptr; float* depthFilt = nullptr;
    uint8_t* frameMask = nullptr; FrameHdr* dHdr = nullptr;
    int curSet = 0;
    size_t packetBytes() const { return (size_t)P * 8 + sizeof(FrameHdr); }
    void selectSet(int k)
    {
        curSet = k; rgb3 = inBuf[k].p; depthRaw = reinterpret_cast<float*>(inBuf[k].p + (size_t)P * 3); frameMask = inBuf[k].p + (size_t)P * 7;
        dHdr = reinterpret_cast<FrameHdr*>(inBuf[k].p + (size_t)P * 8); rgb = rgbBuf[k]; depthFilt = depthFiltBuf[k];
    }
    cudaStream_t preStream = nullptr; cudaEvent_t preDone = nullptr, inputsCopied = nullptr; bool preWaitPending = false, copyPending = false;
    cudaEvent_t inputReady = nullptr;
    DevBuf<uint8_t> mask;
    DevBuf<float> depthPyr[3]; DevBuf<float4> vmap[3], nmap[3];
    DevBuf<uint8_t> nextImage[3]; DevBuf<short2> nextGrad[3]; DevBuf<uint8_t> rgbValid[3];
    DevBuf<float> edgeMap; DevBuf<uint8_t> edgeBinary, edgeBuf, edgeInv;
    DevBuf<TrackJob> dJobs; TrackJob* hJobs = nullptr;
    DevBuf<uint8_t> initFlagR, initFlagF;
    DevBuf<float> scratch;
    DevBuf<float4> rayTab;
    bool frameMapsValid = false, intensityValid = false;
    Profiler prof;
    std::vector<int32_t> classIDs;
    int spawnOffset = 0;
    DevBuf<uint64_t> projKeys; DevBuf<uint8_t> projectedIDs;
    DevBuf<int> ccL, ccDense, ccLabA, ccLabB, ccArea, ccBox, mapToMask, absorbId, maskPixels, compModel, compMask;
    DevBuf<uint32_t> ccCounter; DevBuf<unsigned> maskOverlap;
    DevBuf<uint8_t> segTmp, ignoreMap, tblIdToIndex, tblIndexToId, tblIsModel, tblMaskToID, tblIsPerson;
    float minMaskModelOverlap = 0.05f; int minMappedComponentSize = 160; int personClassID = 255;
};

}
```

maskfusion_b200/csrc/mf_kernels.h:

```cpp
#pragma once
#include <cuda_runtime.h>
#include <cuda_bf16.h>
#include <stdint.h>
#include <string>
#include <vector>
#include "mf_common.cuh"

struct mf_backbone;
struct mf_rpn;
struct mf_detector;

namespace mfb {

struct SurfelPlanes { float4* pos; float4* col; float4* nrm; };

struct CudaError { std::string what; };
void cudaCheck(cudaError_t e, const char* where);

template <typename T>
struct DevBuf {
    T* p = nullptr; size_t n = 0;
    DevBuf() {}
    DevBuf(const DevBuf&) = delete;
    DevBuf& operator=(const DevBuf&) = delete;
    ~DevBuf() { if (p) cudaFree(p); }
    void alloc(size_t count) { if (p) cudaFree(p); p = nullptr; n = 0; if (count) cudaCheck(cudaMalloc((void**)&p, count * sizeof(T)), "cudaMalloc"); n = count; }
    void zero(cudaStream_t s) { if (n) cudaCheck(cudaMemsetAsync(p, 0, n * sizeof(T), s), "memset"); }
    operator T*() const { return p; }
};

struct DataTerm { short2 zero; short2 one; float diff; int valid; };

#define TRACK_MAX_JOBS 32
#define TRACK_MAX_BLOCKS 1024
struct TrackPoses { float p[TRACK_MAX_JOBS][16]; };

struct DevPose { Rt pose; Rt tinv; float fusionW; float pad[7]; };

#ifdef __CUDACC__
__device__ inline void rodrigues2Dev(const float* R, float* out)
{
    double rx = R[7] - R[5], ry = R[2] - R[6], rz = R[3] - R[1];
    double s = sqrt((rx * rx + ry * ry + rz * rz) * 0.25);
    double c = ((double)(R[0] + R[4] + R[8]) - 1) * 0.5;
    c = c > 1. ? 1. : c < -1. ? -1. : c;
    double theta = acos(c);
    if (s < 1e-5) {
        double t;
        if (c > 0) rx = ry = rz = 0;
        else {
            t = (R[0] + 1) * 0.5; rx = sqrt(t > 0 ? t : 0.0);
            t = (R[4] + 1) * 0.5; ry = sqrt(t > 0 ? t : 0.0) * (R[1] < 0 ? -1.0 : 1.0);
            t = (R[8] + 1) * 0.5; rz = sqrt(t > 0 ? t : 0.0) * (R[2] < 0 ? -1.0 : 1.0);
            if (fabs(rx) < fabs(ry) && fabs(rx) < fabs(rz) && (R[5] > 0) != (ry * rz > 0)) rz = -rz;
            theta /= sqrt(rx * rx + ry * ry + rz * rz);
            rx *= theta; ry *= theta; rz *= theta;
        }
    } else {
        double vth = 1 / (2 * s); vth *= theta; rx *= vth; ry *= vth; rz *= vth;
    }
    out[0] = (float)rx; out[1] = (float)ry; out[2] = (float)rz;
}

__device__ inline void derivePose(DevPose* d, const float* m, const float* last)
{
    float inv[16];
    {
        const float R[9] = {m[0], m[1], m[2], m[4], m[5], m[6], m[8], m[9], m[10]}, t[3] = {m[3], m[7], m[11]};
        for (int r = 0; r < 3; ++r) {
            for (int c = 0; c < 3; ++c) inv[r * 4 + c] = R[c * 3 + r];
            inv[r * 4 + 3] = -((R[0 * 3 + r] * t[0] + R[1 * 3 + r] * t[1]) + R[2 * 3 + r] * t[2]);
        }
        inv[12] = 0.f; inv[13] = 0.f; inv[14] = 0.f; inv[15] = 1.f;
    }
    for (int k = 0; k < 12; ++k) { d->pose.m[k] = m[k]; d->tinv.m[k] = inv[k]; }
    float diff[16];
    for (int r = 0; r < 4; ++r)
        for (int c = 0; c < 4; ++c) {
            float s = 0;
            for (int k = 0; k < 4; ++k) s += inv[r * 4 + k] * last[k * 4 + c];
            diff[r * 4 + c] = s;
        }
    const float R[9] = {diff[0], diff[1], diff[2], diff[4], diff[5], diff[6], diff[8], diff[9], diff[10]};
    float tn = sqrtf((diff[3] * diff[3] + diff[7] * diff[7]) + diff[11] * diff[11]);
    float rv[3]; rodrigues2Dev(R, rv);
    float rn = sqrtf((rv[0] * rv[0] + rv[1] * rv[1]) + rv[2] * rv[2]);
    float weighting = tn > rn ? tn : rn;
    const float largest = 0.01f, minWeight = 0.5f;
    if (weighting > largest) weighting = largest;
    float w = 1.0f - (weighting / largest);
    d->fusionW = w > minWeight ? w : minWeight;
}
#endif

struct FrameHdr { long long timestamp; int nMasks; int detectError; int classIDs[256]; int maskGiven; };
#define MF_MAX_MODELS 64
struct FrameResult {
    int hasNewLabel, newClassID, nMasks, nComponents; long long timestamp;
    int dead[MF_MAX_MODELS]; unsigned deadCount[MF_MAX_MODELS];
    float poses[MF_MAX_MODELS][32];
    int detectError;
};
struct SegTables { unsigned char idToIndex[256], indexToId[256], isModel[256]; };
struct VoteParams {
    int nModels, allowNew, personClassID; unsigned minNew, maxNew; float minMaskModelOverlap; unsigned char nextModelID;
    int modelClass[MF_MAX_MODELS]; unsigned char modelID[MF_MAX_MODELS];
};
struct LifeModel { int tracked, owned, ownerRank, pad; DevPose* dpose; const float* trackOut; unsigned* count; float initialC2Winv[16]; };
struct LifeParams { int nModels, rank; LifeModel m[MF_MAX_MODELS]; };

struct TrackState {
    float Rprev[9], tprev[3], RprevInv[9];
    float Rcurr[9], tcurr[3];
    float trR[9], trT[3];
    double resultRt[16];
    double resultR[9], lastResultR[9];
    float R_lr[9];
    float so3LastError, so3LastCount; int so3Done;
    float krk[9], kt[3];
    float sigmaVal; int levelBreak;
    float lastICPError, lastICPCount, lastRGBError, lastRGBCount, lastSO3Error, lastSO3Count;
    double lastA[36], lastb[6];
    float out[40];
    unsigned ticket[4];
};

struct TrackJob {
    const float4* vmapC[3]; const float4* nmapC[3];
    const uint8_t* nextImage[3]; const short2* nextGrad[3]; const uint8_t* rgbValid[3];
    const float4* vmapG[3]; const float4* nmapG[3];
    const float* lastDepth[3]; const uint8_t* lastImage[3];
    const uint8_t* lastNextImage2;
    const float4* cloud[3];
    DataTerm* corres[3];
    DevPose* dpose;
    TrackState* st;
    float* partial;
    const uint32_t* validBits[3];
};

void set_num_sms(int n);
int num_sms();
void prof_mark(cudaStream_t s, const char* name);

int launch_gemm_bf16(const void* A, const void* B, const float* bias, const void* residual, void* out, int M, int N, int K, int relu, cudaStream_t s,
                     const int* conv3x3 = nullptr, bool outF32 = false);
int cnn_conv(const void* in, int Hin, int Win, int Cin, int Cout, int k, int stride, int pad, const void* W, const float* B, void* col, void* out, int relu,
             cudaStream_t s);
bool cnn_conv_implicit(int k, int stride, int pad, int Cin, int Hin, int Win);
void launch_im2col(const void* in, int nimg, int Hin, int Win, int Cin, int Hout, int Wout, int k, int stride, int pad, int Kpad, void* col, cudaStream_t s);
struct MoldGeom { float scale; int newW, newH, offx, offy; };
MoldGeom cnn_mold_geometry(int S, int W, int H);
const char* cnn_last_error();
int cnn_fail(const std::string& msg);
int cnn_check_launch(const char* what);
int cnn_download(cudaStream_t s, void* dst, const void* src, size_t width, size_t rows = 1, size_t pitch = 0);

mf_backbone* rpn_backbone(mf_rpn* h);
const float* rpn_rois(mf_rpn* h);
const void* rpn_pooled(mf_rpn* h);

enum { MRCNN_BACKBONE, MRCNN_RPN, MRCNN_DETECTOR };
struct LayerGeom { int cin, rows, k, stride, pad, K; };
int mrcnn_num_layers(int part);
LayerGeom mrcnn_layer(int part, int i);
struct WeightStore {
    int part;
    std::vector<size_t> wOff, bOff;
    std::vector<float> hW, hB;
    DevBuf<__nv_bfloat16> dW;
    DevBuf<float> dB;
    WeightStore(int part, unsigned seed, cudaStream_t s);
    int load(const char* path, cudaStream_t s);
    int get(int i, float* w, float* b, int rows = -1) const;
    const __nv_bfloat16* w(int i) const { return dW.p + wOff[i]; }
    const float* b(int i) const { return dB.p + bOff[i]; }
};

cudaStream_t detector_stream(mf_detector* h);
int detector_reserve_image(mf_detector* h, int W, int H);
int detector_frame_masks(mf_detector* h, uint8_t* mask, FrameHdr* hdr);

void launch_unpack_rgb(const uint8_t* rgb3, uchar4* out, int P, cudaStream_t s);
void launch_bilateral(const float* depth, float* out, int W, int H, cudaStream_t s);
void launch_pyrdown2_f(const float* src, int sw, int sh, float* dst1, float* dst2, cudaStream_t s);
void launch_pyrdown2_u8(const uint8_t* src, int sw, int sh, uint8_t* dst1, uint8_t* dst2, cudaStream_t s);
void launch_pyrdown2_pair(const float* srcF, float* dstF1, float* dstF2, const uint8_t* srcU, uint8_t* dstU1, uint8_t* dstU2, int sw, int sh, cudaStream_t s);
void launch_vmap_nmap3(const float* const* depth, int W, int H, Cam cam, float cutoff, float4* const* vmap, float4* const* nmap, cudaStream_t s);
void launch_sobel3(const uint8_t* const* img, int W, int H, short2* const* grad, uint8_t* const* rgbValid, cudaStream_t s);
void launch_project_points3(const float* const* depth, int W, int H, Cam cam, float4* const* cloud, cudaStream_t s);
void launch_intensity(const uchar4* img, int P, uint8_t* out, cudaStream_t s);
void launch_intensity_select(const uchar4* imgPred, const uchar4* imgFill, const uint32_t* nonBlack, float denom, int forceFill, int P, uint8_t* out, cudaStream_t s);
float track_min_scale(int level);
void launch_model_maps(const float4* srcVp, const float4* srcNp, const float4* srcVf, const float4* srcNf, const uint32_t* nonBlack, float denom,
                       int W, int H, const DevPose* dpose, float maxDepthRGB, float4* const* v, float4* const* n, float* depth0, cudaStream_t s);
void launch_valid_bits3(const float4* const* nmap, int W, int H, uint32_t* const* bits, cudaStream_t s);
void launch_map_to_planar(const float4* m, int P, float* out, cudaStream_t s);

void launch_fill_u32(uint32_t* p, uint32_t v, size_t n, cudaStream_t s);
void launch_fill_u64(uint64_t* p, uint64_t v, size_t n, cudaStream_t s);
void launch_set_pose(DevPose* d, const float* pose16, const float* lastPose16, cudaStream_t s);
void launch_predict_indices(const SurfelPlanes& sp, const uint32_t* count, const DevPose* dpose, Cam cam, int W, int H, float maxDepth, int time,
                            int timeDelta, uint64_t* key, uint32_t* idx, float4* vertConf, float4* colorTime, float4* normRad, float4* cleanTex, float cleanConf,
                            cudaStream_t s);
void launch_associate(const uchar4* rgb, const float* depthRaw, const float* depthFilt, const uint8_t* mask, const uint32_t* idx,
                      const float4* vertConf, const float4* normRad, const DevPose* dpose, Cam cam, int W, int H, float maxDepth, int time,
                      float weightMultiplier, uint8_t maskID, uint8_t* flag, uint32_t* best, float4* const* meas, uint32_t* slot, cudaStream_t s);
void launch_fuse_update(const uint8_t* flag, const uint32_t* best, float4* const* meas, uint32_t* slot, int P, int time,
                        const SurfelPlanes& sp, cudaStream_t s);
struct CleanWindowImages { const float4* packed; const float4* vertConf; const float4* colorTime; const uint32_t* idx; };
struct IndexFused { uint64_t* key; uint32_t* idx; float4* vertConf; float4* colorTime; float4* normRad; float4* cleanTex; float maxDepth; };
struct CleanInPlace { uint32_t* ticket; uint32_t* loaded; uint32_t* firstMoved; uint32_t epoch; bool pingPong; };
void launch_clean(const SurfelPlanes& src, const SurfelPlanes& dst, const uint32_t* count, uint32_t* newCount, uint32_t capacity,
                  const uint8_t* aflag, float4* const* meas, const DevPose* dpose, Cam cam, int W, int H, int time, int timeDelta, float confThreshold,
                  float outlierCoeff, uint8_t maskID, const CleanWindowImages& win,
                  const float* depthFilt, const uint8_t* mask, uint8_t* keep, uint32_t* blockSums, uint32_t* cand, uint32_t* candCount, cudaStream_t s,
                  const CleanInPlace& inplace, const IndexFused* fused = nullptr);
void launch_combined_predict(const SurfelPlanes& sp, const uint32_t* count, const DevPose* dpose, Cam cam, int W, int H, float maxDepth,
                             float confThreshold, int time, int maxTime, int timeDelta, const float4* rayTab, uint64_t* key, uchar4* image, float4* vertexConf,
                             float4* normalRad, uint16_t* timeTex, int doFill, const float* depthFilt, const uchar4* rgb, int ptVN, int ptImg,
                             uchar4* fillImage, float4* fillVertex, float4* fillNormal, uint32_t* nonBlackSamples, cudaStream_t s, uint32_t capacity = 0);
void launch_ray_table(Cam cam, int W, int H, float4* tab, cudaStream_t s);
void launch_init_model(const uchar4* rgb, const float* depthRaw, const float* depthFilt, Cam cam, int W, int H, int time, float maxDepth,
                       uint8_t* fr, uint8_t* ff, uint32_t* sumR, uint32_t* sumF, uint32_t capacity, const SurfelPlanes& sp, uint32_t* count,
                       cudaStream_t s);
void launch_planes_to_aos(const SurfelPlanes& sp, uint32_t n, float4* out, cudaStream_t s);
void launch_aos_to_planes(const float4* in, uint32_t n, const SurfelPlanes& sp, cudaStream_t s);

void track_shares(int nJobs, unsigned lightMask, int totalCTAs, int ratio, int* G);
int launch_tracking(TrackJob* d_jobs, int nJobs, int W, int H, Cam cam, bool rgbOnly, float icpWeight,
                    bool pyramid, bool fastOdom, bool so3, int numSMs, cudaStream_t s, unsigned lightMask = false);
int debug_track_timing(long long* out, int cap);
void launch_icp_only(const float4* vmapC, const float4* nmapC, const float4* vmapG, const float4* nmapG, int W, int H, Cam cam,
                     const TrackPoses& pp, float* partial, unsigned* ticket, float* out29, int numSMs, cudaStream_t s);

void launch_geometric_edges(const float4* vmap, const float4* nmap, int W, int H, float wD, float wC, float thr, float* edge, uint8_t* binary, cudaStream_t s);
int launch_morph_close_ellipse(uint8_t* data, uint8_t* buf, int W, int H, int radius, int iterations, const FrameHdr* onlyIfMasks, cudaStream_t s);
void launch_morph_close_invert(uint8_t* data, uint8_t* buf, int W, int H, int radius, int iterations, uint8_t* inverted, cudaStream_t s);

}

namespace mfb {
void launch_cc(const uint8_t* img, int W, int H, int* L, int* dense, int* lab, int* area, int* box, uint32_t* counter, cudaStream_t s);
void launch_remove_edges(int* labA, int* labB, const float* depth, const int* area, int W, int H, int iterations, cudaStream_t s);
void launch_seg_tables(const SegTables& t, uint8_t* idToIndex, uint8_t* indexToId, uint8_t* isModel, cudaStream_t s);
void launch_frame_header(const FrameHdr& h, FrameHdr* d, cudaStream_t s);
void launch_person_table(const FrameHdr* hdr, int personClassID, uint8_t* isPerson, cudaStream_t s);
void launch_clear_hist(const uint32_t* ccCounter, const FrameHdr* hdr, int nModels, int* compModel, int* compMask, cudaStream_t s);
void launch_seg_hist(const int* lab, const uint8_t* projID, const uint8_t* mask, int P, const uint8_t* idToIndex, int nModels, const FrameHdr* hdr,
                     int* compModel, int* compMask, cudaStream_t s);
void launch_component_map(const uint32_t* ccCounter, const int* area, const int* compModel, const int* compMask, int nModels, const FrameHdr* hdr,
                          const uint8_t* indexToId, int minMapped, int* mapToMask, int* absorb, int* maskPixels, cudaStream_t s);
void launch_vote(const FrameHdr* hdr, const VoteParams& vp, const int* maskPixels, const unsigned* maskOverlap, const uint32_t* ccCounter,
                 uint8_t* maskToID, FrameResult* res, cudaStream_t s);
void launch_seg_assign(const int* lab, const int* mapToMask, const uint8_t* ignore, int P, uint8_t* seg, cudaStream_t s);
void launch_mask_overlap(const uint8_t* seg, const uint8_t* projID, const uint8_t* idToIndex, const uint8_t* isModelId, int P, unsigned* maskOverlap, cudaStream_t s);
void launch_seg_final(const uint8_t* seg, const int* lab, const int* mapToMask, const int* absorb, const uint8_t* maskToID, const int* box, int P, int W,
                      uint8_t* out, cudaStream_t s);
void launch_apply_ignore(const uint8_t* mask, const uint8_t* isPerson, const FrameHdr* hdr, int P, uint8_t* ignore, uint8_t* edges, cudaStream_t s);
void launch_proj_resolve(uint64_t* key, int P, const uint8_t* indexToId, uint8_t* out, cudaStream_t s);
void launch_splat_project_only(const SurfelPlanes& sp, const uint32_t* count, const DevPose* dpose, Cam cam, int W, int H, float maxDepth, float confThreshold,
                               int time, int maxTime, int timeDelta, uint32_t drawBase, const float4* rayTab, uint64_t* key, cudaStream_t s, uint32_t capacity = 0);
}
```

maskfusion_b200/csrc/mf_surfel.cu:

```cuda
#include "mf_common.cuh"
#include "mf_kernels.h"
#include "mf_host.h"

namespace mfb {

#define MAX_POINT_SIZE 2047.0f

__global__ void __launch_bounds__(256) k_index_project(const float4* __restrict__ pos, const float4* __restrict__ col,
                                                       const uint32_t* __restrict__ countPtr, const DevPose* __restrict__ dpose, Cam cam, int W, int H,
                                                       float maxDepth, float ftime, float ftimeDelta,
                                                       unsigned long long* __restrict__ key)
{
    const Rt tinv = dpose->tinv;
    const uint32_t count = *countPtr;
    for (uint32_t id = blockIdx.x * blockDim.x + threadIdx.x; id < count; id += gridDim.x * blockDim.x) {
        float4 p = ldStream(pos + id);
        float lastTime = ldStream(col + id).w;
        float3 ph = xform(tinv, make_float3(p.x, p.y, p.z));
        if (ph.z > maxDepth || ph.z <= 0 || ftime - lastTime > ftimeDelta) continue;
        float x = ((cam.fx * ph.x) / ph.z) + cam.cx;
        float y = ((cam.fy * ph.y) / ph.z) + cam.cy;
        float zn = ph.z / maxDepth;
        if (!(zn < 1.0f)) continue;
        float fx_ = floorf(x), fy_ = floorf(y);
        if (!(fx_ >= 0 && fy_ >= 0 && fx_ < (float)W && fy_ < (float)H)) continue;
        unsigned long long k = ((unsigned long long)__float_as_uint(zn) << 32) | id;
        unsigned long long* dst = key + ((int)fy_ * W + (int)fx_);
        if (k < *dst) atomicMin(dst, k);
    }
}

__global__ void k_index_resolve(const float4* __restrict__ pos, const float4* __restrict__ col, const float4* __restrict__ nrm,
                                const DevPose* __restrict__ dpose, int P, unsigned long long* __restrict__ key, uint32_t* __restrict__ idx,
                                float4* __restrict__ vertConf, float4* __restrict__ colorTime, float4* __restrict__ normRad,
                                float4* __restrict__ cleanTex, float cleanConf, float cleanTime)
{
    const Rt tinv = dpose->tinv;
    int i = blockIdx.x * blockDim.x + threadIdx.x;
    if (i >= P) return;
    unsigned long long k = key[i];
    if (k == KEY_EMPTY) {
        idx[i] = 0;
        float4 z = make_float4(0, 0, 0, 0);
        vertConf[i] = z; colorTime[i] = z; normRad[i] = z;
        if (cleanTex) cleanTex[i] = z;
        return;
    }
    key[i] = KEY_EMPTY;
    uint32_t id = (uint32_t)(k & 0xffffffffull);
    float4 p = pos[id], c = col[id], n = nrm[id];
    float3 ph = xform(tinv, make_float3(p.x, p.y, p.z));
    float3 nn = normalize3(rotate(tinv, make_float3(n.x, n.y, n.z)));
    idx[i] = id;
    vertConf[i] = make_float4(ph.x, ph.y, ph.z, p.w);
    colorTime[i] = c;
    normRad[i] = make_float4(nn.x, nn.y, nn.z, n.w);
    if (cleanTex) {
        const uint32_t zb = (__float_as_uint(ph.z) & 0x7fffffffu) | (p.w > cleanConf ? 0x80000000u : 0u);
        const uint32_t tb = (__float_as_uint(c.z) & 0x7fffffffu) | (c.w == cleanTime ? 0x80000000u : 0u);
        cleanTex[i] = id != 0u ? make_float4(ph.x, ph.y, __uint_as_float(zb), __uint_as_float(tb)) : make_float4(0, 0, 0, 0);
    }
}

MF_D float3 getVertex(const float* __restrict__ depth, int W, int H, int tx, int ty, float x, float y, Cam cam, float ifx, float ify)
{
    float z = depth[clampi(ty, 0, H - 1) * W + clampi(tx, 0, W - 1)];
    return make_float3((x - cam.cx) * z * ifx, (y - cam.cy) * z * ify, z);
}
MF_D float3 normalCentral(const float* __restrict__ depth, int W, int H, int tx, int ty, float x, float y, Cam cam, float ifx, float ify, float3 vp)
{
    float3 xf = getVertex(depth, W, H, tx + 1, ty, x + 1, y, cam, ifx, ify);
    float3 xb = getVertex(depth, W, H, tx - 1, ty, x - 1, y, cam, ifx, ify);
    float3 yf = getVertex(depth, W, H, tx, ty + 1, x, y + 1, cam, ifx, ify);
    float3 yb = getVertex(depth, W, H, tx, ty - 1, x, y - 1, cam, ifx, ify);
    float3 dx = make_float3(((xb.x + vp.x) / 2) - ((xf.x + vp.x) / 2), ((xb.y + vp.y) / 2) - ((xf.y + vp.y) / 2), ((xb.z + vp.z) / 2) - ((xf.z + vp.z) / 2));
    float3 dy = make_float3(((yb.x + vp.x) / 2) - ((yf.x + vp.x) / 2), ((yb.y + vp.y) / 2) - ((yf.y + vp.y) / 2), ((yb.z + vp.z) / 2) - ((yf.z + vp.z) / 2));
    return normalize3(cross3(dx, dy));
}
MF_D float3 normalForward(const float* __restrict__ depth, int W, int H, int tx, int ty, Cam cam, float ifx, float ify, float3 vp)
{
    float3 vx = getVertex(depth, W, H, tx + 1, ty, (float)(tx + 1), (float)ty, cam, ifx, ify);
    float3 vy = getVertex(depth, W, H, tx, ty + 1, (float)tx, (float)(ty + 1), cam, ifx, ify);
    return normalize3(cross3(sub3(vx, vp), sub3(vy, vp)));
}

__global__ void __launch_bounds__(256) k_associate(const uchar4* __restrict__ rgb, const float* __restrict__ depthRaw,
                                                   const float* __restrict__ depthFilt, const uint8_t* __restrict__ mask,
                                                   const uint32_t* __restrict__ idx, const float4* __restrict__ vertConf,
                                                   const float4* __restrict__ normRad, const DevPose* __restrict__ dpose, Cam cam, int W, int H,
                                                   float maxDepth, int time, float weightMultiplier, uint8_t maskID,
                                                   uint8_t* __restrict__ flag, uint32_t* __restrict__ best,
                                                   float4* __restrict__ m0, float4* __restrict__ m1, float4* __restrict__ m2,
                                                   uint32_t* __restrict__ slot)
{
    int i = blockIdx.x * blockDim.x + threadIdx.x, j = blockIdx.y * blockDim.y + threadIdx.y;
    if (i >= W || j >= H) return;
    const int p = i * H + j;
    const float ifx = 1.0f / cam.fx, ify = 1.0f / cam.fy;
    float tcx = (float)i / (float)W + 0.5f / (float)W;
    float tcy = (float)j / (float)H + 0.5f / (float)H;
    float x = tcx * (float)W, y = tcy * (float)H;
    uint8_t f = 0;
    float3 vl = getVertex(depthRaw, W, H, i, j, x, y, cam, ifx, ify);
    bool cand = ((int)x) % 2 == time % 2 && ((int)y) % 2 == time % 2 && mask[j * W + i] == maskID && vl.z > 0 && vl.z <= maxDepth;
    if (cand) {
        cand = depthRaw[j * W + clampi(i - 1, 0, W - 1)] != 0 && depthRaw[clampi(j - 1, 0, H - 1) * W + i] != 0 &&
               depthRaw[j * W + clampi(i + 1, 0, W - 1)] != 0 && depthRaw[clampi(j + 1, 0, H - 1) * W + i] != 0;
    }
    if (cand) {
        const Rt pose = dpose->pose;
        const float weighting = dpose->fusionW * weightMultiplier;
        float3 vg = xform(pose, vl);
        float3 vf = getVertex(depthFilt, W, H, i, j, x, y, cam, ifx, ify);
        float3 nl = normalCentral(depthFilt, W, H, i, j, x, y, cam, ifx, ify, vf);
        float3 ng = rotate(pose, nl);
        uchar4 c8 = rgb[j * W + i];
        float enc = encodeColor((float)c8.x / 255.0f, (float)c8.y / 255.0f, (float)c8.z / 255.0f);
        float conf = surfelConfidence(x, y, weighting, cam.cx, cam.cy);
        float rad = surfelRadius(vf.z, nl.z, ifx, ify);

        float bestDist = 1000;
        float xl = (x - cam.cx) * ifx, yl = (y - cam.cy) * ify;
        float lambda = sqrtf((xl * xl + yl * yl) + 1);
        float3 ray = make_float3(xl, yl, 1);
        uint32_t b = 0; int operation = 0;
        for (int dx = -1; dx <= 1; ++dx)
            for (int dy = -1; dy <= 1; ++dy) {
                int q = clampi(j + dy, 0, H - 1) * W + clampi(i + dx, 0, W - 1);
                uint32_t cur = idx[q];
                if (cur > 0u) {
                    float4 vc = vertConf[q];
                    float zdiff = vc.z - vl.z;
                    if (fabsf(zdiff * lambda) < 0.05f) {
                        float3 cr = cross3(ray, make_float3(vc.x, vc.y, vc.z));
                        float dist = sqrtf(dot3(cr, cr));
                        float4 nr = normRad[q];
                        if (dist < bestDist) {
                            float3 a = make_float3(nr.x, nr.y, nr.z);
                            bool okn = fabsf(nr.z) < 0.75f ||
                                       fabsf(det_acosf(dot3(a, nl) / (sqrtf(dot3(a, a)) * sqrtf(dot3(nl, nl))))) < 0.5f;
                            if (okn) { operation = 1; bestDist = dist; b = cur; }
                        }
                    }
                }
            }
        f = operation ? 1 : 2;
        m0[p] = make_float4(vg.x, vg.y, vg.z, conf);
        m1[p] = make_float4(enc, 0.f, (float)time, operation ? -1.f : -2.f);
        m2[p] = make_float4(ng.x, ng.y, ng.z, rad);
        best[p] = b;
        if (operation) atomicMin(slot + b, (uint32_t)p);
    }
    flag[p] = f;
}

__global__ void k_fuse_update(const uint8_t* __restrict__ flag, const uint32_t* __restrict__ best,
                              const float4* __restrict__ m0, const float4* __restrict__ m1, const float4* __restrict__ m2,
                              const uint32_t* __restrict__ slot, int P, int time,
                              float4* __restrict__ pos, float4* __restrict__ col, float4* __restrict__ nrm)
{
    int p = blockIdx.x * blockDim.x + threadIdx.x;
    if (p >= P || flag[p] != 1) return;
    uint32_t id = best[p];
    if (slot[id] != (uint32_t)p) return;
    float4 sp = pos[id], sc = col[id], sn = nrm[id];
    float4 np_ = m0[p], nc = m1[p], nn = m2[p];
    float c_k = sp.w, a = np_.w;
    if (nn.w < (1.0f + 0.5f) * sn.w) {
        float d = c_k + a;
        sp = make_float4(((c_k * sp.x) + (a * np_.x)) / d, ((c_k * sp.y) + (a * np_.y)) / d, ((c_k * sp.z) + (a * np_.z)) / d, d);
        float3 oc = decodeColor(sc.x), ncl = decodeColor(nc.x);
        sc.x = encodeColor(((c_k * oc.x) + (a * ncl.x)) / d, ((c_k * oc.y) + (a * ncl.y)) / d, ((c_k * oc.z) + (a * ncl.z)) / d);
        sc.w = (float)time;
        float4 avg = make_float4(((c_k * sn.x) + (a * nn.x)) / d, ((c_k * sn.y) + (a * nn.y)) / d, ((c_k * sn.z) + (a * nn.z)) / d,
                                 ((c_k * sn.w) + (a * nn.w)) / d);
        float3 u = normalize3(make_float3(avg.x, avg.y, avg.z));
        sn = make_float4(u.x, u.y, u.z, avg.w);
    } else {
        sp.w = c_k + a;
        sc.w = (float)time;
    }
    pos[id] = sp; col[id] = sc; nrm[id] = sn;
}

__global__ void k_slot_release(const uint8_t* __restrict__ flag, const uint32_t* __restrict__ best, int P, uint32_t* __restrict__ slot)
{
    int p = blockIdx.x * blockDim.x + threadIdx.x;
    if (p >= P || flag[p] != 1) return;
    slot[best[p]] = 0xffffffffu;
}

struct CleanParams {
    Rt tinv; Cam cam; int W, H; int time; float ftimeDelta; float confThreshold; float outlierCoeff; uint8_t maskID;
};

struct CleanEntry { float xn, yn, lx, ly, lz, init, rad, lnz; };

struct CleanTexels { const float4* packed; const float4* vertConf; const float4* colorTime; const uint32_t* idx; };
template <bool PACKED>
MF_D void cleanWindow(const CleanEntry& e, const CleanParams& P, const CleanTexels& tx, int& count, int& zCount)
{
    const int W = P.W, H = P.H;
    const float cols = (float)W, rows = (float)H, ftime = (float)P.time;
    const float stepX = 1.0f / cols, stepY = 1.0f / rows;
    const float scale = 1.0f, wm = 2;
    const float ixs = stepX * 0.5f / scale, iys = stepY * 0.5f / scale;
    int txs[5], tys[5]; int nx = 0, ny = 0;
#pragma unroll
    for (int k = 0; k < 5; ++k) { txs[k] = -1; tys[k] = -1; }
    for (float i = e.xn - (scale * ixs * wm); i < e.xn + (scale * ixs * wm); i += ixs) {
        int t = clampi((int)floorf(i * cols), 0, W - 1);
#pragma unroll
        for (int k = 0; k < 5; ++k) if (k == nx) txs[k] = t;
        ++nx;
    }
    for (float j = e.yn - (scale * iys * wm); j < e.yn + (scale * iys * wm); j += iys) {
        int t = clampi((int)floorf(j * rows), 0, H - 1);
#pragma unroll
        for (int k = 0; k < 5; ++k) if (k == ny) tys[k] = t;
        ++ny;
    }
    int mxs[5], mys[5];
#pragma unroll
    for (int a = 0; a < 5; ++a) {
        mxs[a] = 0; mys[a] = 0;
#pragma unroll
        for (int c = 0; c < 5; ++c) { mxs[a] += (txs[c] == txs[a]) ? 1 : 0; mys[a] += (tys[c] == tys[a]) ? 1 : 0; }
    }
    int ux[3] = {0, 0, 0}, wx[3] = {0, 0, 0}, uy[3] = {0, 0, 0}, wy[3] = {0, 0, 0};
    int nux = 0, nuy = 0;
#pragma unroll
    for (int a = 0; a < 5; ++a) {
        if (!(txs[a] < 0 || (a > 0 && txs[a] == txs[a - 1]))) {
#pragma unroll
            for (int k = 0; k < 3; ++k) if (k == nux) { ux[k] = txs[a]; wx[k] = mxs[a]; }
            ++nux;
        }
        if (!(tys[a] < 0 || (a > 0 && tys[a] == tys[a - 1]))) {
#pragma unroll
            for (int k = 0; k < 3; ++k) if (k == nuy) { uy[k] = tys[a]; wy[k] = mys[a]; }
            ++nuy;
        }
    }
    count = 0; zCount = 0;
    if (PACKED) {
        float4 t[3][3];
#pragma unroll
        for (int b = 0; b < 3; ++b)
#pragma unroll
            for (int k = 0; k < 3; ++k) t[b][k] = __ldg(tx.packed + (uy[b] * W + ux[k]));
#pragma unroll
        for (int b = 0; b < 3; ++b)
#pragma unroll
            for (int k = 0; k < 3; ++k) {
                const uint32_t zb = __float_as_uint(t[b][k].z), tb = __float_as_uint(t[b][k].w);
                if (b >= nuy || k >= nux || (zb & 0x7fffffffu) == 0u) continue;
                const float mz = __uint_as_float(zb & 0x7fffffffu), initT = __uint_as_float(tb & 0x7fffffffu);
                const bool confOK = (zb >> 31) != 0u, lastNow = (tb >> 31) != 0u;
                const float ddx = t[b][k].x - e.lx, ddy = t[b][k].y - e.ly;
                if (initT < e.init && confOK && mz > e.lz && mz - e.lz < 0.01f && sqrtf(ddx * ddx + ddy * ddy) < e.rad * 1.4f)
                    count += wx[k] * wy[b];
                if (lastNow && confOK && mz > e.lz && mz - e.lz > 0.01f && e.lnz > 0.85f)
                    zCount += wx[k] * wy[b];
            }
        return;
    }
#pragma unroll
    for (int b = 0; b < 3; ++b) {
        if (b >= nuy) break;
        float4 mc[3], tt[3]; uint32_t oc[3];
#pragma unroll
        for (int k = 0; k < 3; ++k) {
            const int q = uy[b] * W + ux[k];
            mc[k] = __ldg(tx.vertConf + q); tt[k] = __ldg(tx.colorTime + q); oc[k] = __ldg(tx.idx + q);
        }
#pragma unroll
        for (int k = 0; k < 3; ++k) {
            if (k >= nux || oc[k] == 0u) continue;
            const float initT = tt[k].z, lastT = tt[k].w;
            const float ddx = mc[k].x - e.lx, ddy = mc[k].y - e.ly;
            if (initT < e.init && mc[k].w > P.confThreshold && mc[k].z > e.lz && mc[k].z - e.lz < 0.01f && sqrtf(ddx * ddx + ddy * ddy) < e.rad * 1.4f)
                count += wx[k] * wy[b];
            if (lastT == ftime && mc[k].w > P.confThreshold && mc[k].z > e.lz && mc[k].z - e.lz > 0.01f && e.lnz > 0.85f)
                zCount += wx[k] * wy[b];
        }
    }
}

MF_D bool cleanFinish(float4& vp, float4& vc, float x, float y, float lpz, int count, int zCount, const CleanParams& P,
                      const float* __restrict__ depthFilt, const uint8_t* __restrict__ mask)
{
    const int W = P.W, H = P.H;
    const float ftime = (float)P.time;
    bool test = true;
    if (count > 8 || zCount > 4) test = false;
    if (vc.w == -2) vc.w = ftime;
    if (vc.w == -1 || ((ftime - vc.w) > 20 && vp.w < P.confThreshold)) test = false;
    if (vc.w > 0 && ftime - vc.w > P.ftimeDelta) test = true;
    float fxs = floorf(x), fys = floorf(y);
    int sx = (fxs != fxs) ? 0 : (fxs < 0 ? 0 : (fxs > (float)(W - 1) ? W - 1 : (int)fxs));
    int sy = (fys != fys) ? 0 : (fys < 0 ? 0 : (fys > (float)(H - 1) ? H - 1 : (int)fys));
    float wDepth = depthFilt[sy * W + sx];
    uint8_t maskValue = mask[sy * W + sx];
    if ((maskValue != P.maskID) && maskValue < 255 && (wDepth > lpz - 0.05f && wDepth < lpz + 0.05f)) {
        float f = (0.5f + 0.5f * (1 - P.outlierCoeff / 10.0f));
        if (maskValue == 0) vp.w *= f;
        else if (P.maskID == 0) vp.w *= 0.25f * f;
        else vp.w *= f;
    }
    return test;
}

#define SCAN_BLOCK 512
#define CAND_BUF 2048
__global__ void __launch_bounds__(256, 8) k_clean_p1(float4* __restrict__ pos, float4* __restrict__ col, const uint32_t* __restrict__ countPtr,
                                                  const uint8_t* __restrict__ aflag, float4* __restrict__ m0, float4* __restrict__ m1, int Ppix,
                                                  CleanParams P, const DevPose* __restrict__ dpose, const float* __restrict__ depthFilt, const uint8_t* __restrict__ mask,
                                                  uint8_t* __restrict__ keep, uint32_t* __restrict__ cand, uint32_t* __restrict__ candCount,
                                                  unsigned long long* __restrict__ indexKey, float indexMaxDepth)
{
    __shared__ uint32_t sBuf[8][CAND_BUF / 8];
    P.tinv = dpose->tinv;
    const uint32_t count = *countPtr;
    const uint32_t total = count + (uint32_t)Ppix;
    const float cols = (float)P.W, rows = (float)P.H, ftime = (float)P.time;
    const int lane = threadIdx.x & 31, warp = threadIdx.x >> 5;
    uint32_t staged = 0;
    auto flush = [&]() {
        uint32_t gbase = 0;
        if (lane == 0) gbase = atomicAdd(candCount, staged);
        gbase = __shfl_sync(0xffffffffu, gbase, 0);
        for (uint32_t i = lane; i < staged; i += 32) cand[gbase + i] = sBuf[warp][i];
        __syncwarp();
        staged = 0;
    };
    const uint32_t stride = gridDim.x * blockDim.x;
    float4 vpN = make_float4(0, 0, 0, 0), vcN = vpN;
    { const uint32_t e0 = blockIdx.x * blockDim.x + threadIdx.x; if (e0 < count) { vpN = pos[e0]; vcN = col[e0]; } }
    for (uint32_t base = blockIdx.x * blockDim.x; base < total; base += stride) {
        const uint32_t e = base + threadIdx.x;
        bool valid = false, need = false, noWindow = false;
        const bool isOld = e < count;
        float4 vp = vpN, vc = vcN;
        if (e + stride < count) { vpN = pos[e + stride]; vcN = col[e + stride]; }
        if (isOld) valid = true;
        else if (e < total) { uint32_t p = e - count; if (aflag[p] == 2) { vp = m0[p]; vc = m1[p]; valid = true; } }
        if (valid) {
            float3 lp = xform(P.tinv, make_float3(vp.x, vp.y, vp.z));
            float x = ((P.cam.fx * lp.x) / lp.z) + P.cam.cx;
            float y = ((P.cam.fy * lp.y) / lp.z) + P.cam.cy;
            need = ftime - vc.w < P.ftimeDelta && lp.z > 0 && x > 0 && y > 0 && x < cols && y < rows;
            if (indexKey && isOld && !(lp.z > indexMaxDepth || lp.z <= 0 || ftime - vc.w > P.ftimeDelta)) {
                const float zn = lp.z / indexMaxDepth;
                const float fx_ = floorf(x), fy_ = floorf(y);
                if (zn < 1.0f && fx_ >= 0 && fy_ >= 0 && fx_ < cols && fy_ < rows) {
                    const unsigned long long k = ((unsigned long long)__float_as_uint(zn) << 32) | e;
                    unsigned long long* dst = indexKey + ((int)fy_ * P.W + (int)fx_);
                    if (k < *dst) atomicMin(dst, k);
                    if (!need) { need = true; noWindow = true; }
                }
            }
            if (!need) {
                const float w0 = vp.w, t0 = vc.w;
                bool k = cleanFinish(vp, vc, x, y, lp.z, 0, 0, P, depthFilt, mask);
                if (isOld) { if (vp.w != w0) pos[e].w = vp.w; if (vc.w != t0) col[e].w = vc.w; }
                else { uint32_t p = e - count; m0[p].w = vp.w; m1[p].w = vc.w; }
                keep[e] = k ? 1 : 0;
            }
        } else if (e < total) keep[e] = 0;
        const unsigned nb = __ballot_sync(0xffffffffu, need);
        if (nb) {
            if (staged + 32 > CAND_BUF / 8) flush();
            if (need) sBuf[warp][staged + __popc(nb & ((1u << lane) - 1))] = noWindow ? (e | 0x80000000u) : e;
            staged += (uint32_t)__popc(nb);
            __syncwarp();
        }
    }
    if (staged) flush();
}

template <bool PACKED>
__global__ void __launch_bounds__(256, 4) k_clean_p2(float4* __restrict__ pos, float4* __restrict__ col, const float4* __restrict__ nrm,
                                                  const uint32_t* __restrict__ countPtr, float4* __restrict__ m0, float4* __restrict__ m1,
                                                  const float4* __restrict__ m2, CleanParams P, const DevPose* __restrict__ dpose, CleanTexels cleanTex,
                                                  const float* __restrict__ depthFilt, const uint8_t* __restrict__ mask, uint8_t* __restrict__ keep,
                                                  const uint32_t* __restrict__ cand, const uint32_t* __restrict__ candCount)
{
    P.tinv = dpose->tinv;
    const uint32_t count = *countPtr, n = *candCount;
    const float cols = (float)P.W, rows = (float)P.H;
    for (uint32_t j = blockIdx.x * blockDim.x + threadIdx.x; j < n; j += gridDim.x * blockDim.x) {
        const uint32_t ce_ = cand[j];
        const bool noWindow = (ce_ >> 31) != 0;
        const uint32_t e = ce_ & 0x7fffffffu;
        const bool isOld = e < count;
        const uint32_t p = e - count;
        float4 vp, vc, vn;
        if (isOld) { vp = pos[e]; vc = col[e]; vn = nrm[e]; } else { vp = m0[p]; vc = m1[p]; vn = m2[p]; }
        const float w0 = vp.w, t0 = vc.w;
        float3 lp = xform(P.tinv, make_float3(vp.x, vp.y, vp.z));
        float x = ((P.cam.fx * lp.x) / lp.z) + P.cam.cx;
        float y = ((P.cam.fy * lp.y) / lp.z) + P.cam.cy;
        float3 ln = normalize3(rotate(P.tinv, make_float3(vn.x, vn.y, vn.z)));
        CleanEntry ce; ce.xn = x / cols; ce.yn = y / rows; ce.lx = lp.x; ce.ly = lp.y; ce.lz = lp.z; ce.init = vc.z; ce.rad = vn.w; ce.lnz = fabsf(ln.z);
        int c1 = 0, c2 = 0;
        if (!noWindow) cleanWindow<PACKED>(ce, P, cleanTex, c1, c2);
        bool k = cleanFinish(vp, vc, x, y, lp.z, c1, c2, P, depthFilt, mask);
        if (isOld) { if (vp.w != w0) pos[e].w = vp.w; if (vc.w != t0) col[e].w = vc.w; }
        else { m0[p].w = vp.w; m1[p].w = vc.w; }
        keep[e] = k ? 1 : 0;
    }
}

__global__ void __launch_bounds__(256) k_keep_block_sums(const uint8_t* __restrict__ keep, const uint32_t* __restrict__ countPtr, int Ppix,
                                                         uint32_t* __restrict__ blockSums, uint32_t* __restrict__ candCount, uint32_t* __restrict__ ticket)
{
    const uint32_t total = *countPtr + (uint32_t)Ppix;
    const uint32_t nblk = (total + SCAN_BLOCK - 1) / SCAN_BLOCK;
    if (blockIdx.x == 0 && threadIdx.x == 0) { *candCount = 0; *ticket = 0; }
    const uint32_t lane = threadIdx.x & 31, gw = (blockIdx.x * blockDim.x + threadIdx.x) >> 5, nw = (gridDim.x * blockDim.x) >> 5;
    for (uint32_t blk = gw; blk < nblk; blk += nw) {
        const uint32_t e0 = blk * SCAN_BLOCK + lane * 16;
        uint4 v = make_uint4(0, 0, 0, 0);
        if (e0 < total) v = *reinterpret_cast<const uint4*>(keep + e0);
        if (e0 < total && total - e0 < 16) {
            const uint32_t r = total - e0;
            uint32_t w[4] = {v.x, v.y, v.z, v.w};
#pragma unroll
            for (int q = 0; q < 4; ++q) { const uint32_t lo = (uint32_t)q * 4; w[q] = r <= lo ? 0u : (r - lo >= 4 ? w[q] : (w[q] & ((1u << (8 * (r - lo))) - 1u))); }
            v = make_uint4(w[0], w[1], w[2], w[3]);
        }
        uint32_t c = __popc(v.x & 0x01010101u) + __popc(v.y & 0x01010101u) + __popc(v.z & 0x01010101u) + __popc(v.w & 0x01010101u);
#pragma unroll
        for (int off = 16; off > 0; off >>= 1) c += __shfl_xor_sync(0xffffffffu, c, off);
        if (lane == 0) blockSums[blk] = c;
    }
}

__global__ void __launch_bounds__(1024) k_scan_block_sums(uint32_t* __restrict__ blockSums, const uint32_t* __restrict__ countPtr,
                                                          int extra, uint32_t capacity, uint32_t* __restrict__ newCount, uint32_t* __restrict__ firstMoved)
{
    const uint32_t total = *countPtr + (uint32_t)extra;
    const uint32_t nblk = (total + SCAN_BLOCK - 1) / SCAN_BLOCK;
    __shared__ uint32_t wtot[32];
    __shared__ uint32_t sFirst;
    if (threadIdx.x == 0) sFirst = nblk;
    __syncthreads();
    const uint32_t per = (nblk + 1023) / 1024;
    const uint32_t b0 = threadIdx.x * per, b1 = min(b0 + per, nblk);
    uint32_t run = 0, first = 0xffffffffu;
    for (uint32_t i = b0; i < b1; ++i) { const uint32_t v = blockSums[i]; run += v; if (v != SCAN_BLOCK && first == 0xffffffffu) first = i; }
    if (first != 0xffffffffu) atomicMin(&sFirst, first);
    const int lane = threadIdx.x & 31, warp = threadIdx.x >> 5;
    uint32_t incl = run;
#pragma unroll
    for (int off = 1; off < 32; off <<= 1) { const uint32_t t = __shfl_up_sync(0xffffffffu, incl, off); if (lane >= off) incl += t; }
    if (lane == 31) wtot[warp] = incl;
    __syncthreads();
    if (warp == 0) {
        uint32_t w = wtot[lane], wi = w;
#pragma unroll
        for (int off = 1; off < 32; off <<= 1) { const uint32_t t = __shfl_up_sync(0xffffffffu, wi, off); if (lane >= off) wi += t; }
        wtot[lane] = wi - w;
        if (lane == 31) { *newCount = wi < capacity ? wi : capacity; }
    }
    __syncthreads();
    uint32_t offs = wtot[warp] + incl - run;
    for (uint32_t i = b0; i < b1; ++i) { const uint32_t v = blockSums[i]; blockSums[i] = offs; offs += v; }
    if (threadIdx.x == 0) { firstMoved[0] = sFirst; firstMoved[1] = nblk; }
}

__global__ void __launch_bounds__(SCAN_BLOCK) k_clean_scatter(const float4* __restrict__ pos, const float4* __restrict__ col, const float4* __restrict__ nrm,
                                                              const uint32_t* __restrict__ countPtr, const float4* __restrict__ m0,
                                                              const float4* __restrict__ m1, const float4* __restrict__ m2, int Ppix,
                                                              const uint8_t* __restrict__ keep, const uint32_t* __restrict__ blockOffs,
                                                              uint32_t capacity, float4* __restrict__ opos, float4* __restrict__ ocol,
                                                              float4* __restrict__ onrm)
{
    const uint32_t count = *countPtr;
    const uint32_t total = count + (uint32_t)Ppix;
    const uint32_t nblk = (total + SCAN_BLOCK - 1) / SCAN_BLOCK;
    __shared__ uint32_t wsum[SCAN_BLOCK / 32];
    for (uint32_t blk = blockIdx.x; blk < nblk; blk += gridDim.x) {
        uint32_t e = blk * SCAN_BLOCK + threadIdx.x;
        bool k = e < total && keep[e];
        unsigned bal = __ballot_sync(0xffffffffu, k);
        int lane = threadIdx.x & 31, warp = threadIdx.x >> 5;
        if (lane == 0) wsum[warp] = __popc(bal);
        __syncthreads();
        uint32_t woff = 0;
        for (int w = 0; w < warp; ++w) woff += wsum[w];
        uint32_t dst = blockOffs[blk] + woff + __popc(bal & ((1u << lane) - 1));
        if (k && dst < capacity) {
            float4 a, b, c;
            if (e < count) { a = ldStream(pos + e); b = ldStream(col + e); c = ldStream(nrm + e); }
            else { uint32_t p = e - count; a = m0[p]; b = m1[p]; c = m2[p]; }
            stStream(opos + dst, a); stStream(ocol + dst, b); stStream(onrm + dst, c);
        }
        __syncthreads();
    }
}

__global__ void __launch_bounds__(SCAN_BLOCK) k_clean_compact(float4* __restrict__ pos, float4* __restrict__ col, float4* __restrict__ nrm,
                                                              const uint32_t* __restrict__ countPtr, const float4* __restrict__ m0,
                                                              const float4* __restrict__ m1, const float4* __restrict__ m2, int Ppix,
                                                              const uint8_t* __restrict__ keep, const uint32_t* __restrict__ blockOffs,
                                                              uint32_t capacity, uint32_t* __restrict__ ticket, uint32_t* __restrict__ loaded,
                                                              const uint32_t* __restrict__ firstMoved, uint32_t epoch)
{
    const uint32_t count = *countPtr;
    const uint32_t total = count + (uint32_t)Ppix;
    const uint32_t nblk = (total + SCAN_BLOCK - 1) / SCAN_BLOCK;
    const uint32_t first = *firstMoved;
    __shared__ uint32_t wsum[SCAN_BLOCK / 32];
    __shared__ uint32_t sBlk[2];
    const int lane = threadIdx.x & 31, warp = threadIdx.x >> 5;
    if (threadIdx.x == 0) sBlk[0] = first + atomicAdd(ticket, 1u);
    __syncthreads();
    for (uint32_t it = 0;; ++it) {
        const uint32_t blk = sBlk[it & 1];
        if (blk >= nblk) break;
        if (threadIdx.x == 0) sBlk[(it + 1) & 1] = first + atomicAdd(ticket, 1u);
        const uint32_t e = blk * SCAN_BLOCK + threadIdx.x;
        const bool k = e < total && keep[e];
        const unsigned bal = __ballot_sync(0xffffffffu, k);
        if (lane == 0) wsum[warp] = __popc(bal);
        __syncthreads();
        uint32_t woff = 0, nb = 0;
#pragma unroll
        for (int w = 0; w < SCAN_BLOCK / 32; ++w) { const uint32_t c = wsum[w]; if (w < warp) woff += c; nb += c; }
        const uint32_t off = blockOffs[blk];
        const uint32_t dst = off + woff + __popc(bal & ((1u << lane) - 1));
        const bool isOld = e < count;
        const bool move = k && dst < capacity && !(isOld && dst == e);
        float4 a = make_float4(0, 0, 0, 0), b = a, c = a;
        if (move) {
            if (isOld) { a = __ldcg(pos + e); b = __ldcg(col + e); c = __ldcg(nrm + e); }
            else { const uint32_t p = e - count; a = m0[p]; b = m1[p]; c = m2[p]; }
        }
        const unsigned probe = __float_as_uint(a.x) & __float_as_uint(b.y) & __float_as_uint(c.z);
        __syncthreads_or(probe == 0x7fedcba9u);
        if (threadIdx.x == 0) {
            asm volatile("st.release.gpu.global.u32 [%0], %1;" ::"l"(loaded + blk), "r"(epoch) : "memory");
            if (nb) {
                const uint32_t s0 = off / SCAN_BLOCK, s1 = (off + nb - 1) / SCAN_BLOCK;
                for (uint32_t s = s0; s <= s1 && s < blk; ++s) {
                    if (s < first) continue;
                    unsigned v;
                    do { asm volatile("ld.acquire.gpu.global.u32 %0, [%1];" : "=r"(v) : "l"(loaded + s) : "memory"); } while (v != epoch);
                }
            }
        }
        __syncthreads();
        if (move) { stStream(pos + dst, a); stStream(col + dst, b); stStream(nrm + dst, c); }
    }
}

struct SplatVS { float3 pos; float conf; float3 n; float rad, size, xw, yw; bool ok; };

MF_D SplatVS splatVertex(float4 p, float4 c, float4 nr, const Rt& tinv, Cam cam, int W, int H, float maxDepth,
                         float confThreshold, float ftime, float fmaxTime, float ftimeDelta)
{
    SplatVS o; o.ok = false;
    float3 ph = xform(tinv, make_float3(p.x, p.y, p.z));
    if (ph.z > maxDepth || ph.z < 0 || p.w < confThreshold || ftime - c.w > ftimeDelta || c.w > fmaxTime) return o;
    o.pos = ph; o.conf = p.w;
    o.n = normalize3(rotate(tinv, make_float3(nr.x, nr.y, nr.z)));
    o.rad = nr.w;
    float3 x1 = normalize3(make_float3(o.n.y - o.n.z, -o.n.x, o.n.x));
    x1 = make_float3(x1.x * o.rad * 1.41421356f, x1.y * o.rad * 1.41421356f, x1.z * o.rad * 1.41421356f);
    float3 y1 = cross3(o.n, x1);
    float px[4], py[4];
#pragma unroll
    for (int q = 0; q < 4; ++q) {
        float3 d = (q == 0 || q == 3) ? x1 : y1;
        float sg = (q < 2) ? 1.0f : -1.0f;
        float3 pp = make_float3(ph.x + sg * d.x, ph.y + sg * d.y, ph.z + sg * d.z);
        px[q] = ((cam.fx * pp.x) / pp.z) + cam.cx;
        py[q] = ((cam.fy * pp.y) / pp.z) + cam.cy;
    }
    float xmin = fminf(px[0], fminf(px[1], fminf(px[2], px[3]))), xmax = fmaxf(px[0], fmaxf(px[1], fmaxf(px[2], px[3])));
    float ymin = fminf(py[0], fminf(py[1], fminf(py[2], py[3]))), ymax = fmaxf(py[0], fmaxf(py[1], fmaxf(py[2], py[3])));
    float sz = fmaxf(0.0f, fmaxf(fabsf(xmax - xmin), fabsf(ymax - ymin)));
    if (!(sz >= 1.0f)) sz = 1.0f;
    if (sz > MAX_POINT_SIZE) sz = MAX_POINT_SIZE;
    o.size = sz;
    o.xw = ((cam.fx * ph.x) / ph.z) + cam.cx;
    o.yw = ((cam.fy * ph.y) / ph.z) + cam.cy;
    if (!(o.xw >= 0 && o.xw <= (float)W && o.yw >= 0 && o.yw <= (float)H)) return o;
    if (!(ph.z / maxDepth <= 1.0f)) return o;
    o.ok = true;
    return o;
}

MF_D float3 pixelRay(Cam cam, float fcx, float fcy)
{
    return normalize3(make_float3((fcx - cam.cx) / cam.fx, (fcy - cam.cy) / cam.fy, 1.0f));
}
__global__ void k_ray_table(Cam cam, int W, int H, float4* __restrict__ tab)
{
    int px = blockIdx.x * blockDim.x + threadIdx.x, py = blockIdx.y * blockDim.y + threadIdx.y;
    if (px >= W || py >= H) return;
    float3 l = pixelRay(cam, (float)px + 0.5f, (float)py + 0.5f);
    tab[py * W + px] = make_float4(l.x, l.y, l.z, 0.f);
}

MF_D bool splatFragmentRay(const SplatVS& v, float3 l, float3& cp)
{
    float t = dot3(v.pos, v.n) / dot3(l, v.n);
    cp = make_float3(t * l.x, t * l.y, t * l.z);
    float sqrRad = v.rad * v.rad;
    float3 d = sub3(cp, v.pos);
    return !(dot3(d, d) > sqrRad);
}
MF_D bool splatFragment(const SplatVS& v, Cam cam, float fcx, float fcy, float3& cp) { return splatFragmentRay(v, pixelRay(cam, fcx, fcy), cp); }

MF_D void splatRange(const SplatVS& v, int W, int H, int& x0, int& x1, int& y0, int& y1)
{
    float h = v.size * 0.5f;
    float lo = ceilf(v.xw - h - 0.5f), hi = ceilf(v.xw + h - 0.5f) - 1.0f;
    x0 = lo < 0 ? 0 : (int)lo; x1 = hi > (float)(W - 1) ? W - 1 : (int)hi;
    lo = ceilf(v.yw - h - 0.5f); hi = ceilf(v.yw + h - 0.5f) - 1.0f;
    y0 = lo < 0 ? 0 : (int)lo; y1 = hi > (float)(H - 1) ? H - 1 : (int)hi;
}

#define SPLAT_SEG 8
#ifndef SPLAT_BS
#define SPLAT_BS 128
#endif
#ifndef SPLAT_MIN_BLOCKS
#define SPLAT_MIN_BLOCKS 8
#endif
#define SPLAT_Q 64

struct __align__(16) SplatEntry { float px, py, pz, pn, nx, ny, nz, rad; int x0, y0, w; uint32_t id; };

MF_D void splatExact(const SplatEntry& e, int pix, const float4* __restrict__ rayTab, unsigned long long* __restrict__ key, float maxDepth)
{
    SplatVS sv; sv.pos = make_float3(e.px, e.py, e.pz); sv.n = make_float3(e.nx, e.ny, e.nz); sv.rad = e.rad;
    const float4 l4 = __ldg(rayTab + pix);
    float3 cp;
    if (!splatFragmentRay(sv, make_float3(l4.x, l4.y, l4.z), cp)) return;
    const float fd = (cp.z / (2 * maxDepth)) + 0.5f;
    if (!(fd >= 0.0f && fd < 1.0f)) return;
    const unsigned long long k = ((unsigned long long)__float_as_uint(fd) << 32) | e.id;
    if (k < key[pix]) atomicMin(key + pix, k);
}

__global__ void __launch_bounds__(SPLAT_BS, SPLAT_MIN_BLOCKS) k_splat_project(const float4* __restrict__ pos, const float4* __restrict__ col, const float4* __restrict__ nrm,
                                                       const uint32_t* __restrict__ countPtr, const DevPose* __restrict__ dpose, Cam cam, int W, int H,
                                                       float maxDepth, float confThreshold, float ftime, float fmaxTime, float ftimeDelta,
                                                       uint32_t drawBase, const float4* __restrict__ rayTab, unsigned long long* __restrict__ key)
{
    constexpr int NW = SPLAT_BS / 32;
    static_assert(SPLAT_BS % 32 == 0 && SPLAT_BS <= 256, "the queue packs the entry slot into 8 bits");
    __shared__ SplatEntry ent[2][SPLAT_BS];
    __shared__ int offs[2][SPLAT_BS];
    __shared__ __align__(16) float4 spos[SPLAT_BS];
    __shared__ uint32_t queue[NW][SPLAT_Q];
    __shared__ int wtot[NW], wcnt[NW];
    __shared__ Rt tinv;
    __shared__ float inv2md;
    __shared__ __align__(8) unsigned long long bar;
    const uint32_t count = *countPtr;
    const int lane = threadIdx.x & 31, warp = threadIdx.x >> 5;
    const uint32_t stride = gridDim.x * SPLAT_BS;
    const unsigned barAddr = (unsigned)__cvta_generic_to_shared(&bar);
    const unsigned sposAddr = (unsigned)__cvta_generic_to_shared(spos);
    auto fetch = [&](uint32_t b) {
        const unsigned bytes = min((uint32_t)SPLAT_BS, count - b) * 16u;
        asm volatile("mbarrier.arrive.expect_tx.shared::cta.b64 _, [%0], %1;" ::"r"(barAddr), "r"(bytes) : "memory");
        asm volatile("cp.async.bulk.shared::cluster.global.mbarrier::complete_tx::bytes [%0], [%1], %2, [%3];"
                     ::"r"(sposAddr), "l"(pos + b), "r"(bytes), "r"(barAddr) : "memory");
    };
    if (threadIdx.x < 12) tinv.m[threadIdx.x] = dpose->tinv.m[threadIdx.x];
    if (threadIdx.x == 0) {
        inv2md = 1.0f / (2 * maxDepth);
        asm volatile("mbarrier.init.shared::cta.b64 [%0], 1;" ::"r"(barAddr));
        asm volatile("fence.mbarrier_init.release.cluster;" ::: "memory");
        if (blockIdx.x * SPLAT_BS < count) fetch(blockIdx.x * SPLAT_BS);
    }
    __syncthreads();
    unsigned parity = 0;
    for (uint32_t base = blockIdx.x * SPLAT_BS; base < count; base += stride, parity ^= 1u) {
        const uint32_t id = base + threadIdx.x;
        SplatVS v; v.ok = false;
        int x0 = 0, x1 = -1, y0 = 0, y1 = -1;
        asm volatile(
            "{\n\t.reg .pred p;\n\t"
            "SPLAT_WAIT:\n\t"
            "mbarrier.try_wait.parity.shared::cta.b64 p, [%0], %1;\n\t"
            "@!p bra SPLAT_WAIT;\n\t}" ::"r"(barAddr), "r"(parity) : "memory");
        if (id < count) {
            const float4 p = spos[threadIdx.x];
            float3 ph = xform(tinv, make_float3(p.x, p.y, p.z));
            const float cxw = ((cam.fx * ph.x) / ph.z) + cam.cx, cyw = ((cam.fy * ph.y) / ph.z) + cam.cy;
            if (!(ph.z > maxDepth || ph.z < 0 || p.w < confThreshold) && cxw >= 0 && cxw <= (float)W && cyw >= 0 && cyw <= (float)H) {
                float4 c = ldStream(col + id), nr = ldStream(nrm + id);
                v = splatVertex(p, c, nr, tinv, cam, W, H, maxDepth, confThreshold, ftime, fmaxTime, ftimeDelta);
                if (v.ok) splatRange(v, W, H, x0, x1, y0, y1);
            }
        }
        const bool draw = v.ok && x1 >= x0 && y1 >= y0;
        const int nunit = draw ? (y1 - y0 + 1) * ((x1 - x0 + SPLAT_SEG) / SPLAT_SEG) : 0;
        int incl = nunit;
#pragma unroll
        for (int o = 1; o < 32; o <<= 1) { int t = __shfl_up_sync(0xffffffffu, incl, o); if (lane >= o) incl += t; }
        unsigned db = __ballot_sync(0xffffffffu, draw);
        if (lane == 31) wtot[warp] = incl;
        if (lane == 0) wcnt[warp] = __popc(db);
        __syncthreads();
        if (threadIdx.x == 0 && base + stride < count) {
            asm volatile("fence.proxy.async.shared::cta;" ::: "memory");
            fetch(base + stride);
        }
        SplatEntry* __restrict__ E = ent[parity];
        int* __restrict__ O = offs[parity];
        int fbase = 0, sbase = 0, total = 0, nent = 0;
#pragma unroll
        for (int w = 0; w < NW; ++w) { if (w < warp) { fbase += wtot[w]; sbase += wcnt[w]; } total += wtot[w]; nent += wcnt[w]; }
        if (draw) {
            const int slot = sbase + __popc(db & ((1u << lane) - 1));
            SplatEntry e; e.px = v.pos.x; e.py = v.pos.y; e.pz = v.pos.z; e.pn = dot3(v.pos, v.n); e.nx = v.n.x; e.ny = v.n.y; e.nz = v.n.z; e.rad = v.rad;
            e.x0 = x0; e.y0 = y0; e.w = x1 - x0 + 1; e.id = drawBase + id;
            E[slot] = e;
            O[slot] = fbase + incl - nunit;
        }
        __syncthreads();
        uint32_t* __restrict__ q = queue[warp];
        int qn = 0;
        for (int ub = threadIdx.x - lane + blockIdx.y * SPLAT_BS; ub < total; ub += SPLAT_BS * gridDim.y) {
            const int u = ub + lane;
            int slot = 0, pix = 0, n = 0;
            if (u < total) {
                int lo = 0, hi = nent - 1;
                while (lo < hi) { int mid = (lo + hi + 1) >> 1; if (O[mid] <= u) lo = mid; else hi = mid - 1; }
                slot = lo;
                const int t = u - O[slot], w = E[slot].w, x0e = E[slot].x0;
                const int nseg = (w + SPLAT_SEG - 1) / SPLAT_SEG;
                const int row = t / nseg, xs = x0e + (t - row * nseg) * SPLAT_SEG;
                n = min(SPLAT_SEG, x0e + w - xs);
                pix = (E[slot].y0 + row) * W + xs;
            }
            const int nmax = __reduce_max_sync(0xffffffffu, n);
            for (int i = 0; i < nmax; ++i, ++pix) {
                bool cand = false;
                if (i < n) {
                    const float4 pp = *reinterpret_cast<const float4*>(&E[slot].px), nr = *reinterpret_cast<const float4*>(&E[slot].nx);
                    const float4 l4 = __ldg(rayTab + pix);
                    const unsigned long long cur = key[pix];
                    const float ta = __fdividef(pp.w, dot3(make_float3(l4.x, l4.y, l4.z), make_float3(nr.x, nr.y, nr.z)));
                    cand = cur == KEY_EMPTY || !(__fmaf_rn(ta * l4.z, inv2md, 0.5f) > __uint_as_float((unsigned)(cur >> 32)) * 1.00001f);
                    if (cand) {
                        const float ax = __fmaf_rn(ta, l4.x, -pp.x), ay = __fmaf_rn(ta, l4.y, -pp.y), az = __fmaf_rn(ta, l4.z, -pp.z);
                        const float re = nr.w + 8e-6f * fabsf(ta);
                        cand = !(__fmaf_rn(ax, ax, __fmaf_rn(ay, ay, az * az)) > re * re * 1.0001f);
                    }
                }
                const unsigned m = __ballot_sync(0xffffffffu, cand);
                if (cand) q[qn + __popc(m & ((1u << lane) - 1))] = (uint32_t)pix << 8 | (uint32_t)slot;
                qn += __popc(m);
                if (qn >= 32) {
                    qn -= 32;
                    __syncwarp();
                    const uint32_t it = q[qn + lane];
                    __syncwarp();
                    splatExact(E[it & 255u], (int)(it >> 8), rayTab, key, maxDepth);
                }
            }
        }
        __syncwarp();
        if (lane < qn) {
            const uint32_t it = q[lane];
            splatExact(E[it & 255u], (int)(it >> 8), rayTab, key, maxDepth);
        }
    }
}

__global__ void k_splat_resolve(const float4* __restrict__ pos, const float4* __restrict__ col, const float4* __restrict__ nrm,
                                const DevPose* __restrict__ dpose, Cam cam, int W, int H, float maxDepth, float confThreshold, float ftime, float fmaxTime,
                                float ftimeDelta, const float4* __restrict__ rayTab, unsigned long long* __restrict__ key,
                                uchar4* __restrict__ image, float4* __restrict__ vertexConf, float4* __restrict__ normalRad,
                                uint16_t* __restrict__ timeTex,
                                int doFill, const float* __restrict__ depthFilt, const uchar4* __restrict__ rgb, int ptVN, int ptImg,
                                uchar4* __restrict__ fillImage, float4* __restrict__ fillVertex, float4* __restrict__ fillNormal,
                                uint32_t* __restrict__ nonBlackSamples)
{
    const Rt tinv = dpose->tinv;
    int px = blockIdx.x * blockDim.x + threadIdx.x, py = blockIdx.y * blockDim.y + threadIdx.y;
    if (px >= W || py >= H) return;
    int i = py * W + px;
    unsigned long long k = key[i];
    uchar4 im = make_uchar4(0, 0, 0, 0);
    float4 vc = make_float4(0, 0, 0, 0), nr = vc;
    uint16_t tt = 0;
    if (k != KEY_EMPTY) {
        key[i] = KEY_EMPTY;
        uint32_t id = (uint32_t)(k & 0xffffffffull);
        float4 p = pos[id], c = col[id], n = nrm[id];
        SplatVS v = splatVertex(p, c, n, tinv, cam, W, H, maxDepth, confThreshold, ftime, fmaxTime, ftimeDelta);
        float3 cp; float fcx = (float)px + 0.5f, fcy = (float)py + 0.5f;
        const float4 l4 = __ldg(rayTab + i);
        splatFragmentRay(v, make_float3(l4.x, l4.y, l4.z), cp);
        float3 cl = decodeColor(c.x);
        im = make_uchar4((uint8_t)(int)floorf(cl.x * 255.0f + 0.5f), (uint8_t)(int)floorf(cl.y * 255.0f + 0.5f),
                         (uint8_t)(int)floorf(cl.z * 255.0f + 0.5f), 255);
        float z = cp.z;
        vc = make_float4((fcx - cam.cx) * z * (1.f / cam.fx), (fcy - cam.cy) * z * (1.f / cam.fy), z, v.conf);
        nr = make_float4(v.n.x, v.n.y, v.n.z, v.rad);
        tt = (uint16_t)(uint32_t)c.z;
    }
    image[i] = im; vertexConf[i] = vc; normalRad[i] = nr; timeTex[i] = tt;
    if (nonBlackSamples && (px % 20) == 10 && (py % 20) == 10 && px / 20 < W / 20 && py / 20 < H / 20) {
        if (im.x > 0 && im.y > 0 && im.z > 0) atomicAdd(nonBlackSamples, 1u);
    }
    if (doFill) {
        const float ifx = 1.0f / cam.fx, ify = 1.0f / cam.fy;
        float3 vp = getVertex(depthFilt, W, H, px, py, (float)px, (float)py, cam, ifx, ify);
        fillVertex[i] = (vc.z == 0 || ptVN) ? make_float4(vp.x, vp.y, vp.z, 1.f) : vc;
        if (nr.z == 0 || ptVN) {
            float3 n = normalForward(depthFilt, W, H, px, py, cam, ifx, ify, vp);
            fillNormal[i] = make_float4(n.x, n.y, n.z, 1.f);
        } else fillNormal[i] = nr;
        float sum = ((float)im.x / 255.0f + (float)im.y / 255.0f) + (float)im.z / 255.0f;
        fillImage[i] = (sum == 0 || ptImg) ? rgb[i] : im;
    }
}

__global__ void __launch_bounds__(SCAN_BLOCK) k_init_flags(const float* __restrict__ depthRaw, const float* __restrict__ depthFilt,
                                                           int W, int H, float maxDepth, uint8_t* __restrict__ fr, uint8_t* __restrict__ ff,
                                                           uint32_t* __restrict__ sumR, uint32_t* __restrict__ sumF)
{
    const int P = W * H;
    __shared__ uint32_t ws[2][SCAN_BLOCK / 32];
    int p = blockIdx.x * SCAN_BLOCK + threadIdx.x;
    bool kr = false, kf = false;
    if (p < P) {
        int i = p / H, j = p - i * H;
        float zr = depthRaw[j * W + i], zf = depthFilt[j * W + i];
        kr = !(zr <= 0 || zr > maxDepth);
        kf = !(zf <= 0 || zf > maxDepth);
        fr[p] = kr; ff[p] = kf;
    }
    unsigned br = __ballot_sync(0xffffffffu, kr), bf = __ballot_sync(0xffffffffu, kf);
    if ((threadIdx.x & 31) == 0) { ws[0][threadIdx.x >> 5] = __popc(br); ws[1][threadIdx.x >> 5] = __popc(bf); }
    __syncthreads();
    if (threadIdx.x == 0) {
        uint32_t a = 0, b = 0;
        for (int w = 0; w < SCAN_BLOCK / 32; ++w) { a += ws[0][w]; b += ws[1][w]; }
        sumR[blockIdx.x] = a; sumF[blockIdx.x] = b;
    }
}

__global__ void __launch_bounds__(SCAN_BLOCK) k_init_scatter(const uchar4* __restrict__ rgb, const float* __restrict__ depthRaw,
                                                             const float* __restrict__ depthFilt, Cam cam, int W, int H, int time,
                                                             const uint8_t* __restrict__ fr, const uint8_t* __restrict__ ff,
                                                             const uint32_t* __restrict__ offR, const uint32_t* __restrict__ offF,
                                                             uint32_t capacity, float4* __restrict__ pos, float4* __restrict__ col,
                                                             float4* __restrict__ nrm)
{
    const int P = W * H;
    __shared__ uint32_t ws[2][SCAN_BLOCK / 32];
    int p = blockIdx.x * SCAN_BLOCK + threadIdx.x;
    bool kr = p < P && fr[p], kf = p < P && ff[p];
    unsigned br = __ballot_sync(0xffffffffu, kr), bf = __ballot_sync(0xffffffffu, kf);
    int lane = threadIdx.x & 31, warp = threadIdx.x >> 5;
    if (lane == 0) { ws[0][warp] = __popc(br); ws[1][warp] = __popc(bf); }
    __syncthreads();
    uint32_t wr = 0, wf = 0;
    for (int w = 0; w < warp; ++w) { wr += ws[0][w]; wf += ws[1][w]; }
    if (p >= P) return;
    int i = p / H, j = p - i * H;
    const float ifx = 1.0f / cam.fx, ify = 1.0f / cam.fy;
    float tcx = (float)(((double)((float)i / (float)W)) + 1.0 / (double)(2 * (float)W));
    float tcy = (float)(((double)((float)j / (float)H)) + 1.0 / (double)(2 * (float)H));
    float x = tcx * (float)W, y = tcy * (float)H;
    if (kr) {
        uint32_t dst = offR[blockIdx.x] + wr + __popc(br & ((1u << lane) - 1));
        if (dst < capacity) {
            float3 vp = getVertex(depthRaw, W, H, i, j, x, y, cam, ifx, ify);
            uchar4 c8 = rgb[j * W + i];
            pos[dst] = make_float4(vp.x, vp.y, vp.z, surfelConfidence(x, y, 1.0f, cam.cx, cam.cy));
            col[dst] = make_float4(encodeColor((float)c8.x / 255.0f, (float)c8.y / 255.0f, (float)c8.z / 255.0f), 0.f, 1.f, (float)time);
        }
    }
    if (kf) {
        uint32_t dst = offF[blockIdx.x] + wf + __popc(bf & ((1u << lane) - 1));
        if (dst < capacity) {
            float3 vp = getVertex(depthFilt, W, H, i, j, x, y, cam, ifx, ify);
            float3 nl = normalCentral(depthFilt, W, H, i, j, x, y, cam, ifx, ify, vp);
            nrm[dst] = make_float4(nl.x, nl.y, nl.z, surfelRadius(vp.z, nl.z, ifx, ify));
        }
    }
}

__global__ void __launch_bounds__(1024) k_scan_small(uint32_t* __restrict__ a, int n, uint32_t capacity, uint32_t* __restrict__ total)
{
    __shared__ uint32_t sh[1024];
    __shared__ uint32_t carry;
    if (threadIdx.x == 0) carry = 0;
    __syncthreads();
    for (int base = 0; base < n; base += 1024) {
        int i = base + threadIdx.x;
        uint32_t v = i < n ? a[i] : 0;
        sh[threadIdx.x] = v;
        __syncthreads();
        for (int off = 1; off < 1024; off <<= 1) {
            uint32_t t = threadIdx.x >= off ? sh[threadIdx.x - off] : 0;
            __syncthreads();
            sh[threadIdx.x] += t;
            __syncthreads();
        }
        uint32_t incl = sh[threadIdx.x];
        if (i < n) a[i] = carry + incl - v;
        __syncthreads();
        if (threadIdx.x == 1023) carry += incl;
        __syncthreads();
    }
    if (threadIdx.x == 0 && total) *total = carry < capacity ? carry : capacity;
}

__global__ void k_fill_u32(uint32_t* p, uint32_t v, size_t n)
{
    size_t i = (size_t)blockIdx.x * blockDim.x + threadIdx.x;
    if (i < n) p[i] = v;
}
__global__ void k_fill_u64(unsigned long long* p, unsigned long long v, size_t n)
{
    size_t i = (size_t)blockIdx.x * blockDim.x + threadIdx.x;
    if (i < n) p[i] = v;
}
__global__ void k_zero_f4(float4* p, uint32_t from, uint32_t to)
{
    uint32_t i = from + blockIdx.x * blockDim.x + threadIdx.x;
    if (i < to) p[i] = make_float4(0, 0, 0, 0);
}

__global__ void k_planes_to_aos(const float4* __restrict__ pos, const float4* __restrict__ col, const float4* __restrict__ nrm, uint32_t n, float4* __restrict__ out)
{
    uint32_t i = blockIdx.x * blockDim.x + threadIdx.x;
    if (i >= n) return;
    out[(size_t)i * 3] = pos[i]; out[(size_t)i * 3 + 1] = col[i]; out[(size_t)i * 3 + 2] = nrm[i];
}
__global__ void k_aos_to_planes(const float4* __restrict__ in, uint32_t n, float4* __restrict__ pos, float4* __restrict__ col, float4* __restrict__ nrm)
{
    uint32_t i = blockIdx.x * blockDim.x + threadIdx.x;
    if (i >= n) return;
    pos[i] = in[(size_t)i * 3]; col[i] = in[(size_t)i * 3 + 1]; nrm[i] = in[(size_t)i * 3 + 2];
}

static int g_numSMs = 0;
void set_num_sms(int n) { g_numSMs = n > 0 ? n : 132; }
int num_sms()
{
    if (!g_numSMs) { int dev = 0, n = 0; cudaGetDevice(&dev); cudaDeviceGetAttribute(&n, cudaDevAttrMultiProcessorCount, dev); set_num_sms(n); }
    return g_numSMs;
}
static inline int persistentBlocks(int perSM) { return num_sms() * perSM; }

struct Pose2 { float p[16], l[16]; };
__global__ void k_set_pose(DevPose* d, Pose2 in)
{
    if (threadIdx.x == 0 && blockIdx.x == 0) derivePose(d, in.p, in.l);
}
void launch_set_pose(DevPose* d, const float* pose16, const float* lastPose16, cudaStream_t s)
{
    Pose2 in;
    for (int k = 0; k < 16; ++k) { in.p[k] = pose16[k]; in.l[k] = lastPose16[k]; }
    k_set_pose<<<1, 32, 0, s>>>(d, in);
}

void launch_fill_u32(uint32_t* p, uint32_t v, size_t n, cudaStream_t s) { if (n) k_fill_u32<<<(unsigned)((n + 255) / 256), 256, 0, s>>>(p, v, n); }
void launch_fill_u64(uint64_t* p, uint64_t v, size_t n, cudaStream_t s) { if (n) k_fill_u64<<<(unsigned)((n + 255) / 256), 256, 0, s>>>((unsigned long long*)p, v, n); }

void launch_predict_indices(const SurfelPlanes& sp, const uint32_t* count, const DevPose* tinv, Cam cam, int W, int H, float maxDepth, int time,
                            int timeDelta, uint64_t* key, uint32_t* idx, float4* vertConf, float4* colorTime, float4* normRad, float4* cleanTex, float cleanConf, cudaStream_t s)
{
    prof_mark(s, "k_index_project"); k_index_project<<<persistentBlocks(8), 256, 0, s>>>(sp.pos, sp.col, count, tinv, cam, W, H, maxDepth, (float)time, (float)timeDelta,
                                                        (unsigned long long*)key);
    int P = W * H;
    prof_mark(s, "k_index_resolve"); k_index_resolve<<<(P + 255) / 256, 256, 0, s>>>(sp.pos, sp.col, sp.nrm, tinv, P, (unsigned long long*)key, idx, vertConf, colorTime, normRad, cleanTex, cleanConf, (float)time);
}

void launch_associate(const uchar4* rgb, const float* depthRaw, const float* depthFilt, const uint8_t* mask, const uint32_t* idx,
                      const float4* vertConf, const float4* normRad, const DevPose* pose, Cam cam, int W, int H, float maxDepth, int time,
                      float weighting, uint8_t maskID, uint8_t* flag, uint32_t* best, float4* const* meas, uint32_t* slot, cudaStream_t s)
{
    dim3 b(32, 8), g((W + 31) / 32, (H + 7) / 8);
    prof_mark(s, "k_associate"); k_associate<<<g, b, 0, s>>>(rgb, depthRaw, depthFilt, mask, idx, vertConf, normRad, pose, cam, W, H, maxDepth, time, weighting, maskID,
                                flag, best, meas[0], meas[1], meas[2], slot);
}

void launch_fuse_update(const uint8_t* flag, const uint32_t* best, float4* const* meas, uint32_t* slot, int P, int time,
                        const SurfelPlanes& sp, cudaStream_t s)
{
    prof_mark(s, "k_fuse_update"); k_fuse_update<<<(P + 255) / 256, 256, 0, s>>>(flag, best, meas[0], meas[1], meas[2], slot, P, time, sp.pos, sp.col, sp.nrm);
    prof_mark(s, "k_slot_release"); k_slot_release<<<(P + 255) / 256, 256, 0, s>>>(flag, best, P, slot);
}

void launch_clean(const SurfelPlanes& src, const SurfelPlanes& dst, const uint32_t* count, uint32_t* newCount, uint32_t capacity,
                  const uint8_t* aflag, float4* const* meas, const DevPose* tinv, Cam cam, int W, int H, int time, int timeDelta, float confThreshold,
                  float outlierCoeff, uint8_t maskID, const CleanWindowImages& win,
                  const float* depthFilt, const uint8_t* mask, uint8_t* keep, uint32_t* blockSums, uint32_t* cand, uint32_t* candCount, cudaStream_t s,
                  const CleanInPlace& inplace, const IndexFused* fused)
{
    const CleanTexels texels{win.packed, win.vertConf, win.colorTime, win.idx};
    CleanParams P;
    P.tinv = Rt{};
    P.cam = cam; P.W = W; P.H = H; P.time = time; P.ftimeDelta = (float)timeDelta; P.confThreshold = confThreshold;
    P.outlierCoeff = outlierCoeff; P.maskID = maskID;
    int Ppix = W * H;
    int blocks = persistentBlocks(4);
    prof_mark(s, "k_clean_p1"); k_clean_p1<<<persistentBlocks(8), 256, 0, s>>>(src.pos, src.col, count, aflag, meas[0], meas[1], Ppix, P, tinv, depthFilt, mask, keep, cand, candCount,
                                                                               fused ? (unsigned long long*)fused->key : nullptr, fused ? fused->maxDepth : 0.f);
    if (fused) {
        prof_mark(s, "k_index_resolve"); k_index_resolve<<<(Ppix + 255) / 256, 256, 0, s>>>(src.pos, src.col, src.nrm, tinv, Ppix, (unsigned long long*)fused->key, fused->idx, fused->vertConf,
                                                                                          fused->colorTime, fused->normRad, fused->cleanTex, confThreshold, (float)time);
    }
    prof_mark(s, "k_clean_p2");
    if (texels.packed) k_clean_p2<true><<<persistentBlocks(8), 256, 0, s>>>(src.pos, src.col, src.nrm, count, meas[0], meas[1], meas[2], P, tinv, texels, depthFilt, mask, keep, cand, candCount);
    else k_clean_p2<false><<<persistentBlocks(8), 256, 0, s>>>(src.pos, src.col, src.nrm, count, meas[0], meas[1], meas[2], P, tinv, texels, depthFilt, mask, keep, cand, candCount);
    prof_mark(s, "k_keep_block_sums"); k_keep_block_sums<<<persistentBlocks(8), 256, 0, s>>>(keep, count, Ppix, blockSums, candCount, inplace.ticket);
    prof_mark(s, "k_scan_block_sums"); k_scan_block_sums<<<1, 1024, 0, s>>>(blockSums, count, Ppix, capacity, newCount, inplace.firstMoved);
    if (!inplace.pingPong) {
        prof_mark(s, "k_clean_compact"); k_clean_compact<<<blocks, SCAN_BLOCK, 0, s>>>(src.pos, src.col, src.nrm, count, meas[0], meas[1], meas[2], Ppix, keep, blockSums, capacity,
                                                      inplace.ticket, inplace.loaded, inplace.firstMoved, inplace.epoch);
    } else {
        prof_mark(s, "k_clean_scatter"); k_clean_scatter<<<blocks, SCAN_BLOCK, 0, s>>>(src.pos, src.col, src.nrm, count, meas[0], meas[1], meas[2], Ppix, keep, blockSums, capacity,
                                                      dst.pos, dst.col, dst.nrm);
    }
}

void launch_ray_table(Cam cam, int W, int H, float4* tab, cudaStream_t s)
{
    dim3 b(32, 8), g((W + 31) / 32, (H + 7) / 8);
    k_ray_table<<<g, b, 0, s>>>(cam, W, H, tab);
}

static dim3 splatGrid(uint32_t capacity, int W, int H)
{
    if ((size_t)W * H > (1u << 24)) throw CudaError{"splat rasteriser: more than 2^24 pixels (its exact-path queue keeps 24-bit pixel indices)"};
    static const int perSM = [] {
        int n = 0;
        cudaCheck(cudaOccupancyMaxActiveBlocksPerMultiprocessor(&n, k_splat_project, SPLAT_BS, 0), "k_splat_project occupancy");
        if (n < 1) throw CudaError{"k_splat_project does not fit on an SM"};
        return n;
    }();
    const int persistent = persistentBlocks(perSM);
    if (capacity == 0 || capacity >= (1u << 20)) return dim3(persistent);
    const int cols = (int)std::min<uint32_t>((capacity + SPLAT_BS - 1) / SPLAT_BS, (uint32_t)persistent);
    return dim3(cols, 8);
}
void launch_combined_predict(const SurfelPlanes& sp, const uint32_t* count, const DevPose* tinv, Cam cam, int W, int H, float maxDepth,
                             float confThreshold, int time, int maxTime, int timeDelta, const float4* rayTab, uint64_t* key, uchar4* image, float4* vertexConf,
                             float4* normalRad, uint16_t* timeTex, int doFill, const float* depthFilt, const uchar4* rgb, int ptVN, int ptImg,
                             uchar4* fillImage, float4* fillVertex, float4* fillNormal, uint32_t* nonBlackSamples, cudaStream_t s, uint32_t capacity)
{
    prof_mark(s, "k_splat_project"); k_splat_project<<<splatGrid(capacity, W, H), SPLAT_BS, 0, s>>>(sp.pos, sp.col, sp.nrm, count, tinv, cam, W, H, maxDepth, confThreshold, (float)time,
                                                        (float)maxTime, (float)timeDelta, 0u, rayTab, (unsigned long long*)key);
    if (nonBlackSamples) cudaMemsetAsync(nonBlackSamples, 0, sizeof(uint32_t), s);
    dim3 b(32, 8), g((W + 31) / 32, (H + 7) / 8);
    prof_mark(s, "k_splat_resolve"); k_splat_resolve<<<g, b, 0, s>>>(sp.pos, sp.col, sp.nrm, tinv, cam, W, H, maxDepth, confThreshold, (float)time, (float)maxTime,
                                    (float)timeDelta, rayTab, (unsigned long long*)key, image, vertexConf, normalRad, timeTex, doFill, depthFilt, rgb,
                                    ptVN, ptImg, fillImage, fillVertex, fillNormal, nonBlackSamples);
}

void launch_init_model(const uchar4* rgb, const float* depthRaw, const float* depthFilt, Cam cam, int W, int H, int time, float maxDepth,
                       uint8_t* fr, uint8_t* ff, uint32_t* sumR, uint32_t* sumF, uint32_t capacity, const SurfelPlanes& sp, uint32_t* count,
                       cudaStream_t s)
{
    int P = W * H, nb = (P + SCAN_BLOCK - 1) / SCAN_BLOCK;
    prof_mark(s, "k_zero_f4"); k_zero_f4<<<(P + 255) / 256, 256, 0, s>>>(sp.nrm, 0, (uint32_t)(P < (int)capacity ? P : (int)capacity));
    prof_mark(s, "k_init_flags"); k_init_flags<<<nb, SCAN_BLOCK, 0, s>>>(depthRaw, depthFilt, W, H, maxDepth, fr, ff, sumR, sumF);
    prof_mark(s, "k_scan_small"); k_scan_small<<<1, 1024, 0, s>>>(sumR, nb, capacity, count);
    prof_mark(s, "k_scan_small"); k_scan_small<<<1, 1024, 0, s>>>(sumF, nb, capacity, nullptr);
    prof_mark(s, "k_init_scatter"); k_init_scatter<<<nb, SCAN_BLOCK, 0, s>>>(rgb, depthRaw, depthFilt, cam, W, H, time, fr, ff, sumR, sumF, capacity, sp.pos, sp.col, sp.nrm);
}

void launch_planes_to_aos(const SurfelPlanes& sp, uint32_t n, float4* out, cudaStream_t s) { if (n) k_planes_to_aos<<<(n + 255) / 256, 256, 0, s>>>(sp.pos, sp.col, sp.nrm, n, out); }
void launch_aos_to_planes(const float4* in, uint32_t n, const SurfelPlanes& sp, cudaStream_t s) { if (n) k_aos_to_planes<<<(n + 255) / 256, 256, 0, s>>>(in, n, sp.pos, sp.col, sp.nrm); }

}

namespace mfb {
void launch_splat_project_only(const SurfelPlanes& sp, const uint32_t* count, const DevPose* tinv, Cam cam, int W, int H, float maxDepth, float confThreshold,
                               int time, int maxTime, int timeDelta, uint32_t drawBase, const float4* rayTab, uint64_t* key, cudaStream_t s, uint32_t capacity)
{
    prof_mark(s, "k_splat_project_ids");
    k_splat_project<<<splatGrid(capacity, W, H), SPLAT_BS, 0, s>>>(sp.pos, sp.col, sp.nrm, count, tinv, cam, W, H, maxDepth, confThreshold, (float)time,
                                                        (float)maxTime, (float)timeDelta, drawBase, rayTab, (unsigned long long*)key);
}
}
```

Before: 730.2.

## Split surfel last-seen time into separate plane to cut streaming bandwidth

Moves the per-surfel last-seen timestamp out of the col float4 into its own float plane, so index projection, clean pass 1 and splat projection read 4 bytes instead of 16 for the time check. Fuse update now writes only the timestamp and pos on a confidence-only update, skipping col/nrm stores. The index projection loop gains software prefetch and deferred atomicMin, clean pass 1 gets double-buffered candidate staging with a 2x unroll, and an occupancy bound becomes tunable. This adds an extra buffer per surfel to allocate and carry through compaction, scatter and AoS conversion, and k_splat_project receives the float time pointer reinterpreted as float4, which is risky unless that kernel was also changed.

```diff
diff --git a/maskfusion_b200/csrc/mf_capi.cu b/maskfusion_b200/csrc/mf_capi.cu
--- a/maskfusion_b200/csrc/mf_capi.cu
+++ b/maskfusion_b200/csrc/mf_capi.cu
@@ -292,7 +292,7 @@
     d2h(o, flag, m->aflag.p, o->P); d2h(o, best, m->abest.p, o->P);
     if (meas12) {
         DevBuf<float4> tmp; tmp.alloc((size_t)o->P * 3);
-        launch_planes_to_aos(SurfelPlanes{m->meas[0].p, m->meas[1].p, m->meas[2].p}, (uint32_t)o->P, tmp, o->stream);
+        launch_planes_to_aos(SurfelPlanes{m->meas[0].p, m->meas[1].p, m->meas[2].p, nullptr}, (uint32_t)o->P, tmp, o->stream);
         cudaCheck(cudaMemcpyAsync(meas12, tmp.p, (size_t)o->P * 48, cudaMemcpyDeviceToHost, o->stream), "D2H");
         o->sync();
     }
diff --git a/maskfusion_b200/csrc/mf_common.cuh b/maskfusion_b200/csrc/mf_common.cuh
--- a/maskfusion_b200/csrc/mf_common.cuh
+++ b/maskfusion_b200/csrc/mf_common.cuh
@@ -103,8 +103,16 @@
     asm volatile("ld.global.nc.L1::no_allocate.v4.f32 {%0,%1,%2,%3}, [%4];" : "=f"(r.x), "=f"(r.y), "=f"(r.z), "=f"(r.w) : "l"(p));
     return r;
 }
+MF_D float ldStream(const float* p) {
+    float r;
+    asm volatile("ld.global.nc.L1::no_allocate.f32 %0, [%1];" : "=f"(r) : "l"(p));
+    return r;
+}
 MF_D void stStream(float4* p, float4 v) {
     asm volatile("st.global.L1::no_allocate.v4.f32 [%0], {%1,%2,%3,%4};" ::"l"(p), "f"(v.x), "f"(v.y), "f"(v.z), "f"(v.w) : "memory");
+}
+MF_D void stStream(float* p, float v) {
+    asm volatile("st.global.L1::no_allocate.f32 [%0], %1;" ::"l"(p), "f"(v) : "memory");
 }
 
 constexpr uint64_t KEY_EMPTY = ~0ull;
diff --git a/maskfusion_b200/csrc/mf_host.cu b/maskfusion_b200/csrc/mf_host.cu
--- a/maskfusion_b200/csrc/mf_host.cu
+++ b/maskfusion_b200/csrc/mf_host.cu
@@ -107,7 +107,7 @@
     const int W = o->W, H = o->H, P = o->P;
     cudaStream_t s = o->stream;
     if (ghost) return;
-    pos[0].alloc(capacity); col[0].alloc(capacity); nrm[0].alloc(capacity);
+    pos[0].alloc(capacity); col[0].alloc(capacity); nrm[0].alloc(capacity); lastSeen[0].alloc(capacity);
     count.alloc(2); count.zero(s);
     cudaCheck(cudaMallocHost((void**)&hCount, 2 * sizeof(uint32_t)), "cudaMallocHost"); hCount[0] = hCount[1] = 0;
     cudaCheck(cudaMallocHost((void**)&hTrackOut, 40 * sizeof(float)), "cudaMallocHost");
@@ -258,7 +258,9 @@
         const uint32_t first = hCleanStat[0], nb = hCleanStat[1];
         pingPong = first < nb && (uint64_t)(nb - first) * 10 > (uint64_t)nb * 4;
     }
-    if (pingPong && !pos[1 - target].p) { pos[1 - target].alloc(capacity); col[1 - target].alloc(capacity); nrm[1 - target].alloc(capacity); }
+    if (pingPong && !pos[1 - target].p) {
+        pos[1 - target].alloc(capacity); col[1 - target].alloc(capacity); nrm[1 - target].alloc(capacity); lastSeen[1 - target].alloc(capacity);
+    }
     int other = pingPong ? 1 - target : target, otherCount = 1 - countSel;
     const bool fused = idxDeferred && idxTime == time && idxDelta == timeDelta && (size_t)capacity + (size_t)o->P < 0x80000000ull;
     if (!fused) flushIndex();
diff --git a/maskfusion_b200/csrc/mf_host.h b/maskfusion_b200/csrc/mf_host.h
--- a/maskfusion_b200/csrc/mf_host.h
+++ b/maskfusion_b200/csrc/mf_host.h
@@ -60,7 +60,7 @@
     void pushPose();
     bool allowsFillIn() const { return fillIn; }
     unsigned lastCount();
-    SurfelPlanes planes(int b) const { return SurfelPlanes{pos[b].p, col[b].p, nrm[b].p}; }
+    SurfelPlanes planes(int b) const { return SurfelPlanes{pos[b].p, col[b].p, nrm[b].p, lastSeen[b].p}; }
     SurfelPlanes current() const { return planes(target); }
     uint32_t* dCount() const { return count.p + countSel; }
 
@@ -73,7 +73,7 @@
     bool fillIn;
     uint32_t capacity;
     int target = 0, countSel = 0;
-    DevBuf<float4> pos[2], col[2], nrm[2];
+    DevBuf<float4> pos[2], col[2], nrm[2]; DevBuf<float> lastSeen[2];
     DevBuf<uint32_t> count;
     uint32_t* hCount = nullptr;
     DevBuf<uint64_t> key;
diff --git a/maskfusion_b200/csrc/mf_kernels.h b/maskfusion_b200/csrc/mf_kernels.h
--- a/maskfusion_b200/csrc/mf_kernels.h
+++ b/maskfusion_b200/csrc/mf_kernels.h
@@ -12,7 +12,7 @@
 
 namespace mfb {
 
-struct SurfelPlanes { float4* pos; float4* col; float4* nrm; };
+struct SurfelPlanes { float4* pos; float4* col; float4* nrm; float* time; };
 
 struct CudaError { std::string what; };
 void cudaCheck(cudaError_t e, const char* where);
diff --git a/maskfusion_b200/csrc/mf_surfel.cu b/maskfusion_b200/csrc/mf_surfel.cu
--- a/maskfusion_b200/csrc/mf_surfel.cu
+++ b/maskfusion_b200/csrc/mf_surfel.cu
@@ -6,32 +6,48 @@
 
 #define MAX_POINT_SIZE 2047.0f
 
-__global__ void __launch_bounds__(256) k_index_project(const float4* __restrict__ pos, const float4* __restrict__ col,
-                                                       const uint32_t* __restrict__ countPtr, const DevPose* __restrict__ dpose, Cam cam, int W, int H,
-                                                       float maxDepth, float ftime, float ftimeDelta,
-                                                       unsigned long long* __restrict__ key)
+MF_D int indexPixel(const Rt& tinv, float4 p, float lastTime, uint32_t id, Cam cam, int W, int H, float maxDepth, float ftime, float ftimeDelta,
+                    unsigned long long& k)
+{
+    const float3 ph = xform(tinv, make_float3(p.x, p.y, p.z));
+    if (ph.z > maxDepth || ph.z <= 0 || ftime - lastTime > ftimeDelta) return -1;
+    const float x = ((cam.fx * ph.x) / ph.z) + cam.cx;
+    const float y = ((cam.fy * ph.y) / ph.z) + cam.cy;
+    const float zn = ph.z / maxDepth;
+    if (!(zn < 1.0f)) return -1;
+    const float fx_ = floorf(x), fy_ = floorf(y);
+    if (!(fx_ >= 0 && fy_ >= 0 && fx_ < (float)W && fy_ < (float)H)) return -1;
+    k = ((unsigned long long)__float_as_uint(zn) << 32) | id;
+    return (int)fy_ * W + (int)fx_;
+}
+
+#ifndef INDEX_BLOCKS
+#define INDEX_BLOCKS 6
+#endif
+__global__ void __launch_bounds__(256, INDEX_BLOCKS) k_index_project(const float4* __restrict__ pos, const float* __restrict__ time,
+                                                          const uint32_t* __restrict__ countPtr, const DevPose* __restrict__ dpose, Cam cam, int W, int H,
+                                                          float maxDepth, float ftime, float ftimeDelta,
+                                                          unsigned long long* __restrict__ key)
 {
     const Rt tinv = dpose->tinv;
     const uint32_t count = *countPtr;
-    for (uint32_t id = blockIdx.x * blockDim.x + threadIdx.x; id < count; id += gridDim.x * blockDim.x) {
-        float4 p = ldStream(pos + id);
-        float lastTime = ldStream(col + id).w;
-        float3 ph = xform(tinv, make_float3(p.x, p.y, p.z));
-        if (ph.z > maxDepth || ph.z <= 0 || ftime - lastTime > ftimeDelta) continue;
-        float x = ((cam.fx * ph.x) / ph.z) + cam.cx;
-        float y = ((cam.fy * ph.y) / ph.z) + cam.cy;
-        float zn = ph.z / maxDepth;
-        if (!(zn < 1.0f)) continue;
-        float fx_ = floorf(x), fy_ = floorf(y);
-        if (!(fx_ >= 0 && fy_ >= 0 && fx_ < (float)W && fy_ < (float)H)) continue;
-        unsigned long long k = ((unsigned long long)__float_as_uint(zn) << 32) | id;
-        unsigned long long* dst = key + ((int)fy_ * W + (int)fx_);
-        if (k < *dst) atomicMin(dst, k);
-    }
+    const uint32_t stride = gridDim.x * blockDim.x;
+    uint32_t id = blockIdx.x * blockDim.x + threadIdx.x;
+    float4 pN = make_float4(0, 0, 0, 0); float tN = 0.f;
+    if (id < count) { pN = ldStream(pos + id); tN = ldStream(time + id); }
+    int pixPrev = -1; unsigned long long kPrev = 0, curPrev = 0;
+    for (; id < count; id += stride) {
+        const float4 p = pN; const float t = tN;
+        if (id + stride < count) { pN = ldStream(pos + id + stride); tN = ldStream(time + id + stride); }
+        if (pixPrev >= 0 && kPrev < curPrev) atomicMin(key + pixPrev, kPrev);
+        pixPrev = indexPixel(tinv, p, t, id, cam, W, H, maxDepth, ftime, ftimeDelta, kPrev);
+        if (pixPrev >= 0) curPrev = key[pixPrev];
+    }
+    if (pixPrev >= 0 && kPrev < curPrev) atomicMin(key + pixPrev, kPrev);
 }
 
 __global__ void k_index_resolve(const float4* __restrict__ pos, const float4* __restrict__ col, const float4* __restrict__ nrm,
-                                const DevPose* __restrict__ dpose, int P, unsigned long long* __restrict__ key, uint32_t* __restrict__ idx,
+                                const float* __restrict__ time, const DevPose* __restrict__ dpose, int P, unsigned long long* __restrict__ key, uint32_t* __restrict__ idx,
                                 float4* __restrict__ vertConf, float4* __restrict__ colorTime, float4* __restrict__ normRad,
                                 float4* __restrict__ cleanTex, float cleanConf, float cleanTime)
 {
@@ -49,6 +65,7 @@
     key[i] = KEY_EMPTY;
     uint32_t id = (uint32_t)(k & 0xffffffffull);
     float4 p = pos[id], c = col[id], n = nrm[id];
+    c.w = time[id];
     float3 ph = xform(tinv, make_float3(p.x, p.y, p.z));
     float3 nn = normalize3(rotate(tinv, make_float3(n.x, n.y, n.z)));
     idx[i] = id;
@@ -157,30 +174,32 @@
 __global__ void k_fuse_update(const uint8_t* __restrict__ flag, const uint32_t* __restrict__ best,
                               const float4* __restrict__ m0, const float4* __restrict__ m1, const float4* __restrict__ m2,
                               const uint32_t* __restrict__ slot, int P, int time,
-                              float4* __restrict__ pos, float4* __restrict__ col, float4* __restrict__ nrm)
+                              float4* __restrict__ pos, float4* __restrict__ col, float4* __restrict__ nrm, float* __restrict__ lastSeen)
 {
     int p = blockIdx.x * blockDim.x + threadIdx.x;
     if (p >= P || flag[p] != 1) return;
     uint32_t id = best[p];
     if (slot[id] != (uint32_t)p) return;
-    float4 sp = pos[id], sc = col[id], sn = nrm[id];
-    float4 np_ = m0[p], nc = m1[p], nn = m2[p];
+    float4 sp = pos[id], sn = nrm[id];
+    float4 np_ = m0[p], nn = m2[p];
     float c_k = sp.w, a = np_.w;
+    lastSeen[id] = (float)time;
     if (nn.w < (1.0f + 0.5f) * sn.w) {
+        float4 sc = col[id];
+        const float4 nc = m1[p];
         float d = c_k + a;
         sp = make_float4(((c_k * sp.x) + (a * np_.x)) / d, ((c_k * sp.y) + (a * np_.y)) / d, ((c_k * sp.z) + (a * np_.z)) / d, d);
         float3 oc = decodeColor(sc.x), ncl = decodeColor(nc.x);
         sc.x = encodeColor(((c_k * oc.x) + (a * ncl.x)) / d, ((c_k * oc.y) + (a * ncl.y)) / d, ((c_k * oc.z) + (a * ncl.z)) / d);
-        sc.w = (float)time;
         float4 avg = make_float4(((c_k * sn.x) + (a * nn.x)) / d, ((c_k * sn.y) + (a * nn.y)) / d, ((c_k * sn.z) + (a * nn.z)) / d,
                                  ((c_k * sn.w) + (a * nn.w)) / d);
         float3 u = normalize3(make_float3(avg.x, avg.y, avg.z));
         sn = make_float4(u.x, u.y, u.z, avg.w);
+        col[id] = sc; nrm[id] = sn;
     } else {
         sp.w = c_k + a;
-        sc.w = (float)time;
-    }
-    pos[id] = sp; col[id] = sc; nrm[id] = sn;
+    }
+    pos[id] = sp;
 }
 
 __global__ void k_slot_release(const uint8_t* __restrict__ flag, const uint32_t* __restrict__ best, int P, uint32_t* __restrict__ slot)
@@ -191,7 +210,7 @@
 }
 
 struct CleanParams {
-    Rt tinv; Cam cam; int W, H; int time; float ftimeDelta; float confThreshold; float outlierCoeff; uint8_t maskID;
+    Rt tinv; Cam cam; int W, H; int time; float ftimeDelta; float confThreshold; float outlierF; uint8_t maskID;
 };
 
 struct CleanEntry { float xn, yn, lx, ly, lz, init, rad, lnz; };
@@ -287,23 +306,23 @@
     }
 }
 
-MF_D bool cleanFinish(float4& vp, float4& vc, float x, float y, float lpz, int count, int zCount, const CleanParams& P,
+MF_D bool cleanFinish(float4& vp, float& lastT, float x, float y, float lpz, int count, int zCount, const CleanParams& P,
                       const float* __restrict__ depthFilt, const uint8_t* __restrict__ mask)
 {
     const int W = P.W, H = P.H;
     const float ftime = (float)P.time;
     bool test = true;
     if (count > 8 || zCount > 4) test = false;
-    if (vc.w == -2) vc.w = ftime;
-    if (vc.w == -1 || ((ftime - vc.w) > 20 && vp.w < P.confThreshold)) test = false;
-    if (vc.w > 0 && ftime - vc.w > P.ftimeDelta) test = true;
+    if (lastT == -2) lastT = ftime;
+    if (lastT == -1 || ((ftime - lastT) > 20 && vp.w < P.confThreshold)) test = false;
+    if (lastT > 0 && ftime - lastT > P.ftimeDelta) test = true;
     float fxs = floorf(x), fys = floorf(y);
     int sx = (fxs != fxs) ? 0 : (fxs < 0 ? 0 : (fxs > (float)(W - 1) ? W - 1 : (int)fxs));
     int sy = (fys != fys) ? 0 : (fys < 0 ? 0 : (fys > (float)(H - 1) ? H - 1 : (int)fys));
     float wDepth = depthFilt[sy * W + sx];
     uint8_t maskValue = mask[sy * W + sx];
     if ((maskValue != P.maskID) && maskValue < 255 && (wDepth > lpz - 0.05f && wDepth < lpz + 0.05f)) {
-        float f = (0.5f + 0.5f * (1 - P.outlierCoeff / 10.0f));
+        const float f = P.outlierF;
         if (maskValue == 0) vp.w *= f;
         else if (P.maskID == 0) vp.w *= 0.25f * f;
         else vp.w *= f;
@@ -312,76 +331,95 @@
 }
 
 #define SCAN_BLOCK 512
-#define CAND_BUF 2048
-__global__ void __launch_bounds__(256, 8) k_clean_p1(float4* __restrict__ pos, float4* __restrict__ col, const uint32_t* __restrict__ countPtr,
+#define CAND_HALF 256
+#define CLEAN_U 2
+#ifndef CLEAN_P1_BLOCKS
+#define CLEAN_P1_BLOCKS 4
+#endif
+__global__ void __launch_bounds__(256, CLEAN_P1_BLOCKS) k_clean_p1(float4* __restrict__ pos, float* __restrict__ lastSeen, const uint32_t* __restrict__ countPtr,
                                                   const uint8_t* __restrict__ aflag, float4* __restrict__ m0, float4* __restrict__ m1, int Ppix,
                                                   CleanParams P, const DevPose* __restrict__ dpose, const float* __restrict__ depthFilt, const uint8_t* __restrict__ mask,
                                                   uint8_t* __restrict__ keep, uint32_t* __restrict__ cand, uint32_t* __restrict__ candCount,
                                                   unsigned long long* __restrict__ indexKey, float indexMaxDepth)
 {
-    __shared__ uint32_t sBuf[8][CAND_BUF / 8];
+    __shared__ uint32_t sBuf[8][2][CAND_HALF];
     P.tinv = dpose->tinv;
     const uint32_t count = *countPtr;
     const uint32_t total = count + (uint32_t)Ppix;
     const float cols = (float)P.W, rows = (float)P.H, ftime = (float)P.time;
     const int lane = threadIdx.x & 31, warp = threadIdx.x >> 5;
-    uint32_t staged = 0;
-    auto flush = [&]() {
-        uint32_t gbase = 0;
-        if (lane == 0) gbase = atomicAdd(candCount, staged);
-        gbase = __shfl_sync(0xffffffffu, gbase, 0);
-        for (uint32_t i = lane; i < staged; i += 32) cand[gbase + i] = sBuf[warp][i];
+    uint32_t half = 0, staged = 0, pendN = 0;
+    uint32_t pendRes = 0;
+    auto rotate = [&]() {
+        if (pendN) {
+            const uint32_t gbase = __shfl_sync(0xffffffffu, pendRes, 0);
+            for (uint32_t i = lane; i < pendN; i += 32) cand[gbase + i] = sBuf[warp][half ^ 1u][i];
+        }
+        if (lane == 0 && staged) pendRes = atomicAdd(candCount, staged);
+        pendN = staged; staged = 0; half ^= 1u;
         __syncwarp();
-        staged = 0;
     };
     const uint32_t stride = gridDim.x * blockDim.x;
-    float4 vpN = make_float4(0, 0, 0, 0), vcN = vpN;
-    { const uint32_t e0 = blockIdx.x * blockDim.x + threadIdx.x; if (e0 < count) { vpN = pos[e0]; vcN = col[e0]; } }
-    for (uint32_t base = blockIdx.x * blockDim.x; base < total; base += stride) {
-        const uint32_t e = base + threadIdx.x;
-        bool valid = false, need = false, noWindow = false;
-        const bool isOld = e < count;
-        float4 vp = vpN, vc = vcN;
-        if (e + stride < count) { vpN = pos[e + stride]; vcN = col[e + stride]; }
-        if (isOld) valid = true;
-        else if (e < total) { uint32_t p = e - count; if (aflag[p] == 2) { vp = m0[p]; vc = m1[p]; valid = true; } }
-        if (valid) {
-            float3 lp = xform(P.tinv, make_float3(vp.x, vp.y, vp.z));
-            float x = ((P.cam.fx * lp.x) / lp.z) + P.cam.cx;
-            float y = ((P.cam.fy * lp.y) / lp.z) + P.cam.cy;
-            need = ftime - vc.w < P.ftimeDelta && lp.z > 0 && x > 0 && y > 0 && x < cols && y < rows;
-            if (indexKey && isOld && !(lp.z > indexMaxDepth || lp.z <= 0 || ftime - vc.w > P.ftimeDelta)) {
-                const float zn = lp.z / indexMaxDepth;
-                const float fx_ = floorf(x), fy_ = floorf(y);
-                if (zn < 1.0f && fx_ >= 0 && fy_ >= 0 && fx_ < cols && fy_ < rows) {
-                    const unsigned long long k = ((unsigned long long)__float_as_uint(zn) << 32) | e;
-                    unsigned long long* dst = indexKey + ((int)fy_ * P.W + (int)fx_);
-                    if (k < *dst) atomicMin(dst, k);
-                    if (!need) { need = true; noWindow = true; }
+    for (uint32_t base = blockIdx.x * blockDim.x; base < total; base += CLEAN_U * stride) {
+        float4 vp0 = make_float4(0, 0, 0, 0), vp1 = vp0; float vt0 = 0.f, vt1 = 0.f;
+        {
+            const uint32_t e = base + threadIdx.x;
+            if (e < count) { vp0 = pos[e]; vt0 = lastSeen[e]; }
+            if (e + stride < count) { vp1 = pos[e + stride]; vt1 = lastSeen[e + stride]; }
+        }
+        int pix0 = -1, pix1 = -1; unsigned long long key0 = 0, key1 = 0;
+#pragma unroll 1
+        for (int u = 0; u < CLEAN_U; ++u) {
+            const uint32_t e = base + threadIdx.x + u * stride;
+            float4 vp = u ? vp1 : vp0; float vt = u ? vt1 : vt0;
+            bool valid = false, need = false, noWindow = false;
+            const bool isOld = e < count;
+            if (isOld) valid = true;
+            else if (e < total) { uint32_t p = e - count; if (aflag[p] == 2) { vp = m0[p]; vt = m1[p].w; valid = true; } }
+            if (valid) {
+                float3 lp = xform(P.tinv, make_float3(vp.x, vp.y, vp.z));
+                float x = ((P.cam.fx * lp.x) / lp.z) + P.cam.cx;
+                float y = ((P.cam.fy * lp.y) / lp.z) + P.cam.cy;
+                need = ftime - vt < P.ftimeDelta && lp.z > 0 && x > 0 && y > 0 && x < cols && y < rows;
+                if (indexKey && isOld && !(lp.z > indexMaxDepth || lp.z <= 0 || ftime - vt > P.ftimeDelta)) {
+                    const float zn = lp.z / indexMaxDepth;
+                    const float fx_ = floorf(x), fy_ = floorf(y);
+                    if (zn < 1.0f && fx_ >= 0 && fy_ >= 0 && fx_ < cols && fy_ < rows) {
+                        const unsigned long long k = ((unsigned long long)__float_as_uint(zn) << 32) | e;
+                        const int q = (int)fy_ * P.W + (int)fx_;
+                        if (u) { key1 = k; pix1 = q; } else { key0 = k; pix0 = q; }
+                        if (!need) { need = true; noWindow = true; }
+                    }
                 }
+                if (!need) {
+                    const float w0 = vp.w, t0 = vt;
+                    bool k = cleanFinish(vp, vt, x, y, lp.z, 0, 0, P, depthFilt, mask);
+                    if (isOld) { if (vp.w != w0) pos[e].w = vp.w; if (vt != t0) lastSeen[e] = vt; }
+                    else { uint32_t p = e - count; m0[p].w = vp.w; m1[p].w = vt; }
+                    keep[e] = k ? 1 : 0;
+                }
+            } else if (e < total) keep[e] = 0;
+            const unsigned nb = __ballot_sync(0xffffffffu, need);
+            if (nb) {
+                if (staged + 32 > CAND_HALF) rotate();
+                if (need) sBuf[warp][half][staged + __popc(nb & ((1u << lane) - 1))] = noWindow ? (e | 0x80000000u) : e;
+                staged += (uint32_t)__popc(nb);
+                __syncwarp();
             }
-            if (!need) {
-                const float w0 = vp.w, t0 = vc.w;
-                bool k = cleanFinish(vp, vc, x, y, lp.z, 0, 0, P, depthFilt, mask);
-                if (isOld) { if (vp.w != w0) pos[e].w = vp.w; if (vc.w != t0) col[e].w = vc.w; }
-                else { uint32_t p = e - count; m0[p].w = vp.w; m1[p].w = vc.w; }
-                keep[e] = k ? 1 : 0;
-            }
-        } else if (e < total) keep[e] = 0;
-        const unsigned nb = __ballot_sync(0xffffffffu, need);
-        if (nb) {
-            if (staged + 32 > CAND_BUF / 8) flush();
-            if (need) sBuf[warp][staged + __popc(nb & ((1u << lane) - 1))] = noWindow ? (e | 0x80000000u) : e;
-            staged += (uint32_t)__popc(nb);
-            __syncwarp();
-        }
-    }
-    if (staged) flush();
+        }
+        unsigned long long cur0 = 0, cur1 = 0;
+        if (pix0 >= 0) cur0 = indexKey[pix0];
+        if (pix1 >= 0) cur1 = indexKey[pix1];
+        if (pix0 >= 0 && key0 < cur0) atomicMin(indexKey + pix0, key0);
+        if (pix1 >= 0 && key1 < cur1) atomicMin(indexKey + pix1, key1);
+    }
+    rotate();
+    rotate();
 }
 
 template <bool PACKED>
-__global__ void __launch_bounds__(256, 4) k_clean_p2(float4* __restrict__ pos, float4* __restrict__ col, const float4* __restrict__ nrm,
-                                                  const uint32_t* __restrict__ countPtr, float4* __restrict__ m0, float4* __restrict__ m1,
+__global__ void __launch_bounds__(256, 4) k_clean_p2(float4* __restrict__ pos, const float4* __restrict__ col, const float4* __restrict__ nrm,
+                                                  float* __restrict__ lastSeen, const uint32_t* __restrict__ countPtr, float4* __restrict__ m0, float4* __restrict__ m1,
                                                   const float4* __restrict__ m2, CleanParams P, const DevPose* __restrict__ dpose, CleanTexels cleanTex,
                                                   const float* __restrict__ depthFilt, const uint8_t* __restrict__ mask, uint8_t* __restrict__ keep,
                                                   const uint32_t* __restrict__ cand, const uint32_t* __restrict__ candCount)
@@ -395,9 +433,9 @@
         const uint32_t e = ce_ & 0x7fffffffu;
         const bool isOld = e < count;
         const uint32_t p = e - count;
-        float4 vp, vc, vn;
-        if (isOld) { vp = pos[e]; vc = col[e]; vn = nrm[e]; } else { vp = m0[p]; vc = m1[p]; vn = m2[p]; }
-        const float w0 = vp.w, t0 = vc.w;
+        float4 vp, vc, vn; float vt;
+        if (isOld) { vp = pos[e]; vc = col[e]; vn = nrm[e]; vt = lastSeen[e]; } else { vp = m0[p]; vc = m1[p]; vn = m2[p]; vt = vc.w; }
+        const float w0 = vp.w, t0 = vt;
         float3 lp = xform(P.tinv, make_float3(vp.x, vp.y, vp.z));
         float x = ((P.cam.fx * lp.x) / lp.z) + P.cam.cx;
         float y = ((P.cam.fy * lp.y) / lp.z) + P.cam.cy;
@@ -405,9 +443,9 @@
         CleanEntry ce; ce.xn = x / cols; ce.yn = y / rows; ce.lx = lp.x; ce.ly = lp.y; ce.lz = lp.z; ce.init = vc.z; ce.rad = vn.w; ce.lnz = fabsf(ln.z);
         int c1 = 0, c2 = 0;
         if (!noWindow) cleanWindow<PACKED>(ce, P, cleanTex, c1, c2);
-        bool k = cleanFinish(vp, vc, x, y, lp.z, c1, c2, P, depthFilt, mask);
-        if (isOld) { if (vp.w != w0) pos[e].w = vp.w; if (vc.w != t0) col[e].w = vc.w; }
-        else { m0[p].w = vp.w; m1[p].w = vc.w; }
+        bool k = cleanFinish(vp, vt, x, y, lp.z, c1, c2, P, depthFilt, mask);
+        if (isOld) { if (vp.w != w0) pos[e].w = vp.w; if (vt != t0) lastSeen[e] = vt; }
+        else { m0[p].w = vp.w; m1[p].w = vt; }
         keep[e] = k ? 1 : 0;
     }
 }
@@ -471,11 +509,11 @@
 }
 
 __global__ void __launch_bounds__(SCAN_BLOCK) k_clean_scatter(const float4* __restrict__ pos, const float4* __restrict__ col, const float4* __restrict__ nrm,
-                                                              const uint32_t* __restrict__ countPtr, const float4* __restrict__ m0,
+                                                              const float* __restrict__ lastSeen, const uint32_t* __restrict__ countPtr, const float4* __restrict__ m0,
                                                               const float4* __restrict__ m1, const float4* __restrict__ m2, int Ppix,
                                                               const uint8_t* __restrict__ keep, const uint32_t* __restrict__ blockOffs,
                                                               uint32_t capacity, float4* __restrict__ opos, float4* __restrict__ ocol,
-                                                              float4* __restrict__ onrm)
+                                                              float4* __restrict__ onrm, float* __restrict__ olastSeen)
 {
     const uint32_t count = *countPtr;
     const uint32_t total = count + (uint32_t)Ppix;
@@ -492,17 +530,17 @@
         for (int w = 0; w < warp; ++w) woff += wsum[w];
         uint32_t dst = blockOffs[blk] + woff + __popc(bal & ((1u << lane) - 1));
         if (k && dst < capacity) {
-            float4 a, b, c;
-            if (e < count) { a = ldStream(pos + e); b = ldStream(col + e); c = ldStream(nrm + e); }
-            else { uint32_t p = e - count; a = m0[p]; b = m1[p]; c = m2[p]; }
-            stStream(opos + dst, a); stStream(ocol + dst, b); stStream(onrm + dst, c);
+            float4 a, b, c; float t;
+            if (e < count) { a = ldStream(pos + e); b = ldStream(col + e); c = ldStream(nrm + e); t = ldStream(lastSeen + e); }
+            else { uint32_t p = e - count; a = m0[p]; b = m1[p]; c = m2[p]; t = b.w; b.w = 0.f; }
+            stStream(opos + dst, a); stStream(ocol + dst, b); stStream(onrm + dst, c); stStream(olastSeen + dst, t);
         }
         __syncthreads();
     }
 }
 
 __global__ void __launch_bounds__(SCAN_BLOCK) k_clean_compact(float4* __restrict__ pos, float4* __restrict__ col, float4* __restrict__ nrm,
-                                                              const uint32_t* __restrict__ countPtr, const float4* __restrict__ m0,
+                                                              float* __restrict__ lastSeen, const uint32_t* __restrict__ countPtr, const float4* __restrict__ m0,
                                                               const float4* __restrict__ m1, const float4* __restrict__ m2, int Ppix,
                                                               const uint8_t* __restrict__ keep, const uint32_t* __restrict__ blockOffs,
                                                               uint32_t capacity, uint32_t* __restrict__ ticket, uint32_t* __restrict__ loaded,
@@ -533,12 +571,12 @@
         const uint32_t dst = off + woff + __popc(bal & ((1u << lane) - 1));
         const bool isOld = e < count;
         const bool move = k && dst < capacity && !(isOld && dst == e);
-        float4 a = make_float4(0, 0, 0, 0), b = a, c = a;
+        float4 a = make_float4(0, 0, 0, 0), b = a, c = a; float t = 0.f;
         if (move) {
-            if (isOld) { a = __ldcg(pos + e); b = __ldcg(col + e); c = __ldcg(nrm + e); }
-            else { const uint32_t p = e - count; a = m0[p]; b = m1[p]; c = m2[p]; }
-        }
-        const unsigned probe = __float_as_uint(a.x) & __float_as_uint(b.y) & __float_as_uint(c.z);
+            if (isOld) { a = __ldcg(pos + e); b = __ldcg(col + e); c = __ldcg(nrm + e); t = __ldcg(lastSeen + e); }
+            else { const uint32_t p = e - count; a = m0[p]; b = m1[p]; c = m2[p]; t = b.w; b.w = 0.f; }
+        }
+        const unsigned probe = __float_as_uint(a.x) & __float_as_uint(b.y) & __float_as_uint(c.z) & __float_as_uint(t);
         __syncthreads_or(probe == 0x7fedcba9u);
         if (threadIdx.x == 0) {
             asm volatile("st.release.gpu.global.u32 [%0], %1;" ::"l"(loaded + blk), "r"(epoch) : "memory");
@@ -552,18 +590,19 @@
             }
         }
         __syncthreads();
-        if (move) { stStream(pos + dst, a); stStream(col + dst, b); stStream(nrm + dst, c); }
+        if (move) { stStream(pos + dst, a); stStream(col + dst, b); stStream(nrm + dst, c); stStream(lastSeen + dst, t); }
     }
 }
 
 struct SplatVS { float3 pos; float conf; float3 n; float rad, size, xw, yw; bool ok; };
 
-MF_D SplatVS splatVertex(float4 p, float4 c, float4 nr, const Rt& tinv, Cam cam, int W, int H, float maxDepth,
-                         float confThreshold, float ftime, float fmaxTime, float ftimeDelta)
+MF_D bool splatTimeOK(float lastT, float ftime, float fmaxTime, float ftimeDelta) { return !(ftime - lastT > ftimeDelta || lastT > fmaxTime); }
+
+MF_D SplatVS splatVertex(float4 p, float4 nr, const Rt& tinv, Cam cam, int W, int H, float maxDepth, float confThreshold)
 {
     SplatVS o; o.ok = false;
     float3 ph = xform(tinv, make_float3(p.x, p.y, p.z));
-    if (ph.z > maxDepth || ph.z < 0 || p.w < confThreshold || ftime - c.w > ftimeDelta || c.w > fmaxTime) return o;
+    if (ph.z > maxDepth || ph.z < 0 || p.w < confThreshold) return o;
     o.pos = ph; o.conf = p.w;
     o.n = normalize3(rotate(tinv, make_float3(nr.x, nr.y, nr.z)));
     o.rad = nr.w;
@@ -647,11 +686,12 @@
     if (k < key[pix]) atomicMin(key + pix, k);
 }
 
-__global__ void __launch_bounds__(SPLAT_BS, SPLAT_MIN_BLOCKS) k_splat_project(const float4* __restrict__ pos, const float4* __restrict__ col, const float4* __restrict__ nrm,
+__global__ void __launch_bounds__(SPLAT_BS, SPLAT_MIN_BLOCKS) k_splat_project(const float4* __restrict__ pos, const float4* __restrict__ lastSeen4, const float4* __restrict__ nrm,
                                                        const uint32_t* __restrict__ countPtr, const DevPose* __restrict__ dpose, Cam cam, int W, int H,
                                                        float maxDepth, float confThreshold, float ftime, float fmaxTime, float ftimeDelta,
                                                        uint32_t drawBase, const float4* __restrict__ rayTab, unsigned long long* __restrict__ key)
 {
+    const float* __restrict__ lastSeen = reinterpret_cast<const float*>(lastSeen4);
     constexpr int NW = SPLAT_BS / 32;
     static_assert(SPLAT_BS % 32 == 0 && SPLAT_BS <= 256, "the queue packs the entry slot into 8 bits");
     __shared__ SplatEntry ent[2][SPLAT_BS];
@@ -696,9 +736,12 @@
             float3 ph = xform(tinv, make_float3(p.x, p.y, p.z));
             const float cxw = ((cam.fx * ph.x) / ph.z) + cam.cx, cyw = ((cam.fy * ph.y) / ph.z) + cam.cy;
             if (!(ph.z > maxDepth || ph.z < 0 || p.w < confThreshold) && cxw >= 0 && cxw <= (float)W && cyw >= 0 && cyw <= (float)H) {
-                float4 c = ldStream(col + id), nr = ldStream(nrm + id);
-                v = splatVertex(p, c, nr, tinv, cam, W, H, maxDepth, confThreshold, ftime, fmaxTime, ftimeDelta);
-                if (v.ok) splatRange(v, W, H, x0, x1, y0, y1);
+                const float lt = ldStream(lastSeen + id);
+                const float4 nr = ldStream(nrm + id);
+                if (splatTimeOK(lt, ftime, fmaxTime, ftimeDelta) || (lt != lt && nr.w == nr.w)) {
+                    v = splatVertex(p, nr, tinv, cam, W, H, maxDepth, confThreshold);
+                    if (v.ok) splatRange(v, W, H, x0, x1, y0, y1);
+                }
             }
         }
         const bool draw = v.ok && x1 >= x0 && y1 >= y0;
@@ -778,8 +821,8 @@
 }
 
 __global__ void k_splat_resolve(const float4* __restrict__ pos, const float4* __restrict__ col, const float4* __restrict__ nrm,
-                                const DevPose* __restrict__ dpose, Cam cam, int W, int H, float maxDepth, float confThreshold, float ftime, float fmaxTime,
-                                float ftimeDelta, const float4* __restrict__ rayTab, unsigned long long* __restrict__ key,
+                                const DevPose* __restrict__ dpose, Cam cam, int W, int H, float maxDepth, float confThreshold,
+                                const float4* __restrict__ rayTab, unsigned long long* __restrict__ key,
                                 uchar4* __restrict__ image, float4* __restrict__ vertexConf, float4* __restrict__ normalRad,
                                 uint16_t* __restrict__ timeTex,
                                 int doFill, const float* __restrict__ depthFilt, const uchar4* __restrict__ rgb, int ptVN, int ptImg,
@@ -798,7 +841,7 @@
         key[i] = KEY_EMPTY;
         uint32_t id = (uint32_t)(k & 0xffffffffull);
         float4 p = pos[id], c = col[id], n = nrm[id];
-        SplatVS v = splatVertex(p, c, n, tinv, cam, W, H, maxDepth, confThreshold, ftime, fmaxTime, ftimeDelta);
+        SplatVS v = splatVertex(p, n, tinv, cam, W, H, maxDepth, confThreshold);
         float3 cp; float fcx = (float)px + 0.5f, fcy = (float)py + 0.5f;
         const float4 l4 = __ldg(rayTab + i);
         splatFragmentRay(v, make_float3(l4.x, l4.y, l4.z), cp);
@@ -857,7 +900,7 @@
                                                              const uint8_t* __restrict__ fr, const uint8_t* __restrict__ ff,
                                                              const uint32_t* __restrict__ offR, const uint32_t* __restrict__ offF,
                                                              uint32_t capacity, float4* __restrict__ pos, float4* __restrict__ col,
-                                                             float4* __restrict__ nrm)
+                                                             float4* __restrict__ nrm, float* __restrict__ lastSeen)
 {
     const int P = W * H;
     __shared__ uint32_t ws[2][SCAN_BLOCK / 32];
@@ -881,7 +924,8 @@
             float3 vp = getVertex(depthRaw, W, H, i, j, x, y, cam, ifx, ify);
             uchar4 c8 = rgb[j * W + i];
             pos[dst] = make_float4(vp.x, vp.y, vp.z, surfelConfidence(x, y, 1.0f, cam.cx, cam.cy));
-            col[dst] = make_float4(encodeColor((float)c8.x / 255.0f, (float)c8.y / 255.0f, (float)c8.z / 255.0f), 0.f, 1.f, (float)time);
+            col[dst] = make_float4(encodeColor((float)c8.x / 255.0f, (float)c8.y / 255.0f, (float)c8.z / 255.0f), 0.f, 1.f, 0.f);
+            lastSeen[dst] = (float)time;
         }
     }
     if (kf) {
@@ -936,17 +980,23 @@
     if (i < to) p[i] = make_float4(0, 0, 0, 0);
 }
 
-__global__ void k_planes_to_aos(const float4* __restrict__ pos, const float4* __restrict__ col, const float4* __restrict__ nrm, uint32_t n, float4* __restrict__ out)
+__global__ void k_planes_to_aos(const float4* __restrict__ pos, const float4* __restrict__ col, const float4* __restrict__ nrm, const float* __restrict__ time,
+                                uint32_t n, float4* __restrict__ out)
 {
     uint32_t i = blockIdx.x * blockDim.x + threadIdx.x;
     if (i >= n) return;
-    out[(size_t)i * 3] = pos[i]; out[(size_t)i * 3 + 1] = col[i]; out[(size_t)i * 3 + 2] = nrm[i];
-}
-__global__ void k_aos_to_planes(const float4* __restrict__ in, uint32_t n, float4* __restrict__ pos, float4* __restrict__ col, float4* __restrict__ nrm)
+    float4 c = col[i];
+    if (time) c.w = time[i];
+    out[(size_t)i * 3] = pos[i]; out[(size_t)i * 3 + 1] = c; out[(size_t)i * 3 + 2] = nrm[i];
+}
+__global__ void k_aos_to_planes(const float4* __restrict__ in, uint32_t n, float4* __restrict__ pos, float4* __restrict__ col, float4* __restrict__ nrm,
+                                float* __restrict__ time)
 {
     uint32_t i = blockIdx.x * blockDim.x + threadIdx.x;
     if (i >= n) return;
-    pos[i] = in[(size_t)i * 3]; col[i] = in[(size_t)i * 3 + 1]; nrm[i] = in[(size_t)i * 3 + 2];
+    float4 c = in[(size_t)i * 3 + 1];
+    time[i] = c.w; c.w = 0.f;
+    pos[i] = in[(size_t)i * 3]; col[i] = c; nrm[i] = in[(size_t)i * 3 + 2];
 }
 
 static int g_numSMs = 0;
@@ -976,10 +1026,10 @@
 void launch_predict_indices(const SurfelPlanes& sp, const uint32_t* count, const DevPose* tinv, Cam cam, int W, int H, float maxDepth, int time,
                             int timeDelta, uint64_t* key, uint32_t* idx, float4* vertConf, float4* colorTime, float4* normRad, float4* cleanTex, float cleanConf, cudaStream_t s)
 {
-    prof_mark(s, "k_index_project"); k_index_project<<<persistentBlocks(8), 256, 0, s>>>(sp.pos, sp.col, count, tinv, cam, W, H, maxDepth, (float)time, (float)timeDelta,
+    prof_mark(s, "k_index_project"); k_index_project<<<persistentBlocks(INDEX_BLOCKS), 256, 0, s>>>(sp.pos, sp.time, count, tinv, cam, W, H, maxDepth, (float)time, (float)timeDelta,
                                                         (unsigned long long*)key);
     int P = W * H;
-    prof_mark(s, "k_index_resolve"); k_index_resolve<<<(P + 255) / 256, 256, 0, s>>>(sp.pos, sp.col, sp.nrm, tinv, P, (unsigned long long*)key, idx, vertConf, colorTime, normRad, cleanTex, cleanConf, (float)time);
+    prof_mark(s, "k_index_resolve"); k_index_resolve<<<(P + 255) / 256, 256, 0, s>>>(sp.pos, sp.col, sp.nrm, sp.time, tinv, P, (unsigned long long*)key, idx, vertConf, colorTime, normRad, cleanTex, cleanConf, (float)time);
 }
 
 void launch_associate(const uchar4* rgb, const float* depthRaw, const float* depthFilt, const uint8_t* mask, const uint32_t* idx,
@@ -994,7 +1044,7 @@
 void launch_fuse_update(const uint8_t* flag, const uint32_t* best, float4* const* meas, uint32_t* slot, int P, int time,
                         const SurfelPlanes& sp, cudaStream_t s)
 {
-    prof_mark(s, "k_fuse_update"); k_fuse_update<<<(P + 255) / 256, 256, 0, s>>>(flag, best, meas[0], meas[1], meas[2], slot, P, time, sp.pos, sp.col, sp.nrm);
+    prof_mark(s, "k_fuse_update"); k_fuse_update<<<(P + 255) / 256, 256, 0, s>>>(flag, best, meas[0], meas[1], meas[2], slot, P, time, sp.pos, sp.col, sp.nrm, sp.time);
     prof_mark(s, "k_slot_release"); k_slot_release<<<(P + 255) / 256, 256, 0, s>>>(flag, best, P, slot);
 }
 
@@ -1008,26 +1058,26 @@
     CleanParams P;
     P.tinv = Rt{};
     P.cam = cam; P.W = W; P.H = H; P.time = time; P.ftimeDelta = (float)timeDelta; P.confThreshold = confThreshold;
-    P.outlierCoeff = outlierCoeff; P.maskID = maskID;
+    P.outlierF = (0.5f + 0.5f * (1 - outlierCoeff / 10.0f)); P.maskID = maskID;
     int Ppix = W * H;
     int blocks = persistentBlocks(4);
-    prof_mark(s, "k_clean_p1"); k_clean_p1<<<persistentBlocks(8), 256, 0, s>>>(src.pos, src.col, count, aflag, meas[0], meas[1], Ppix, P, tinv, depthFilt, mask, keep, cand, candCount,
+    prof_mark(s, "k_clean_p1"); k_clean_p1<<<persistentBlocks(CLEAN_P1_BLOCKS), 256, 0, s>>>(src.pos, src.time, count, aflag, meas[0], meas[1], Ppix, P, tinv, depthFilt, mask, keep, cand, candCount,
                                                                                fused ? (unsigned long long*)fused->key : nullptr, fused ? fused->maxDepth : 0.f);
     if (fused) {
-        prof_mark(s, "k_index_resolve"); k_index_resolve<<<(Ppix + 255) / 256, 256, 0, s>>>(src.pos, src.col, src.nrm, tinv, Ppix, (unsigned long long*)fused->key, fused->idx, fused->vertConf,
+        prof_mark(s, "k_index_resolve"); k_index_resolve<<<(Ppix + 255) / 256, 256, 0, s>>>(src.pos, src.col, src.nrm, src.time, tinv, Ppix, (unsigned long long*)fused->key, fused->idx, fused->vertConf,
                                                                                           fused->colorTime, fused->normRad, fused->cleanTex, confThreshold, (float)time);
     }
     prof_mark(s, "k_clean_p2");
-    if (texels.packed) k_clean_p2<true><<<persistentBlocks(8), 256, 0, s>>>(src.pos, src.col, src.nrm, count, meas[0], meas[1], meas[2], P, tinv, texels, depthFilt, mask, keep, cand, candCount);
-    else k_clean_p2<false><<<persistentBlocks(8), 256, 0, s>>>(src.pos, src.col, src.nrm, count, meas[0], meas[1], meas[2], P, tinv, texels, depthFilt, mask, keep, cand, candCount);
+    if (texels.packed) k_clean_p2<true><<<persistentBlocks(8), 256, 0, s>>>(src.pos, src.col, src.nrm, src.time, count, meas[0], meas[1], meas[2], P, tinv, texels, depthFilt, mask, keep, cand, candCount);
+    else k_clean_p2<false><<<persistentBlocks(8), 256, 0, s>>>(src.pos, src.col, src.nrm, src.time, count, meas[0], meas[1], meas[2], P, tinv, texels, depthFilt, mask, keep, cand, candCount);
     prof_mark(s, "k_keep_block_sums"); k_keep_block_sums<<<persistentBlocks(8), 256, 0, s>>>(keep, count, Ppix, blockSums, candCount, inplace.ticket);
     prof_mark(s, "k_scan_block_sums"); k_scan_block_sums<<<1, 1024, 0, s>>>(blockSums, count, Ppix, capacity, newCount, inplace.firstMoved);
     if (!inplace.pingPong) {
-        prof_mark(s, "k_clean_compact"); k_clean_compact<<<blocks, SCAN_BLOCK, 0, s>>>(src.pos, src.col, src.nrm, count, meas[0], meas[1], meas[2], Ppix, keep, blockSums, capacity,
+        prof_mark(s, "k_clean_compact"); k_clean_compact<<<blocks, SCAN_BLOCK, 0, s>>>(src.pos, src.col, src.nrm, src.time, count, meas[0], meas[1], meas[2], Ppix, keep, blockSums, capacity,
                                                       inplace.ticket, inplace.loaded, inplace.firstMoved, inplace.epoch);
     } else {
-        prof_mark(s, "k_clean_scatter"); k_clean_scatter<<<blocks, SCAN_BLOCK, 0, s>>>(src.pos, src.col, src.nrm, count, meas[0], meas[1], meas[2], Ppix, keep, blockSums, capacity,
-                                                      dst.pos, dst.col, dst.nrm);
+        prof_mark(s, "k_clean_scatter"); k_clean_scatter<<<blocks, SCAN_BLOCK, 0, s>>>(src.pos, src.col, src.nrm, src.time, count, meas[0], meas[1], meas[2], Ppix, keep, blockSums, capacity,
+                                                      dst.pos, dst.col, dst.nrm, dst.time);
     }
 }
 
@@ -1056,12 +1106,12 @@
                              float4* normalRad, uint16_t* timeTex, int doFill, const float* depthFilt, const uchar4* rgb, int ptVN, int ptImg,
                              uchar4* fillImage, float4* fillVertex, float4* fillNormal, uint32_t* nonBlackSamples, cudaStream_t s, uint32_t capacity)
 {
-    prof_mark(s, "k_splat_project"); k_splat_project<<<splatGrid(capacity, W, H), SPLAT_BS, 0, s>>>(sp.pos, sp.col, sp.nrm, count, tinv, cam, W, H, maxDepth, confThreshold, (float)time,
+    prof_mark(s, "k_splat_project"); k_splat_project<<<splatGrid(capacity, W, H), SPLAT_BS, 0, s>>>(sp.pos, reinterpret_cast<const float4*>(sp.time), sp.nrm, count, tinv, cam, W, H, maxDepth, confThreshold, (float)time,
                                                         (float)maxTime, (float)timeDelta, 0u, rayTab, (unsigned long long*)key);
     if (nonBlackSamples) cudaMemsetAsync(nonBlackSamples, 0, sizeof(uint32_t), s);
     dim3 b(32, 8), g((W + 31) / 32, (H + 7) / 8);
-    prof_mark(s, "k_splat_resolve"); k_splat_resolve<<<g, b, 0, s>>>(sp.pos, sp.col, sp.nrm, tinv, cam, W, H, maxDepth, confThreshold, (float)time, (float)maxTime,
-                                    (float)timeDelta, rayTab, (unsigned long long*)key, image, vertexConf, normalRad, timeTex, doFill, depthFilt, rgb,
+    prof_mark(s, "k_splat_resolve"); k_splat_resolve<<<g, b, 0, s>>>(sp.pos, sp.col, sp.nrm, tinv, cam, W, H, maxDepth, confThreshold,
+                                    rayTab, (unsigned long long*)key, image, vertexConf, normalRad, timeTex, doFill, depthFilt, rgb,
                                     ptVN, ptImg, fillImage, fillVertex, fillNormal, nonBlackSamples);
 }
 
@@ -1074,11 +1124,11 @@
     prof_mark(s, "k_init_flags"); k_init_flags<<<nb, SCAN_BLOCK, 0, s>>>(depthRaw, depthFilt, W, H, maxDepth, fr, ff, sumR, sumF);
     prof_mark(s, "k_scan_small"); k_scan_small<<<1, 1024, 0, s>>>(sumR, nb, capacity, count);
     prof_mark(s, "k_scan_small"); k_scan_small<<<1, 1024, 0, s>>>(sumF, nb, capacity, nullptr);
-    prof_mark(s, "k_init_scatter"); k_init_scatter<<<nb, SCAN_BLOCK, 0, s>>>(rgb, depthRaw, depthFilt, cam, W, H, time, fr, ff, sumR, sumF, capacity, sp.pos, sp.col, sp.nrm);
-}
-
-void launch_planes_to_aos(const SurfelPlanes& sp, uint32_t n, float4* out, cudaStream_t s) { if (n) k_planes_to_aos<<<(n + 255) / 256, 256, 0, s>>>(sp.pos, sp.col, sp.nrm, n, out); }
-void launch_aos_to_planes(const float4* in, uint32_t n, const SurfelPlanes& sp, cudaStream_t s) { if (n) k_aos_to_planes<<<(n + 255) / 256, 256, 0, s>>>(in, n, sp.pos, sp.col, sp.nrm); }
+    prof_mark(s, "k_init_scatter"); k_init_scatter<<<nb, SCAN_BLOCK, 0, s>>>(rgb, depthRaw, depthFilt, cam, W, H, time, fr, ff, sumR, sumF, capacity, sp.pos, sp.col, sp.nrm, sp.time);
+}
+
+void launch_planes_to_aos(const SurfelPlanes& sp, uint32_t n, float4* out, cudaStream_t s) { if (n) k_planes_to_aos<<<(n + 255) / 256, 256, 0, s>>>(sp.pos, sp.col, sp.nrm, sp.time, n, out); }
+void launch_aos_to_planes(const float4* in, uint32_t n, const SurfelPlanes& sp, cudaStream_t s) { if (n) k_aos_to_planes<<<(n + 255) / 256, 256, 0, s>>>(in, n, sp.pos, sp.col, sp.nrm, sp.time); }
 
 }
 
@@ -1087,7 +1137,7 @@
                                int time, int maxTime, int timeDelta, uint32_t drawBase, const float4* rayTab, uint64_t* key, cudaStream_t s, uint32_t capacity)
 {
     prof_mark(s, "k_splat_project_ids");
-    k_splat_project<<<splatGrid(capacity, W, H), SPLAT_BS, 0, s>>>(sp.pos, sp.col, sp.nrm, count, tinv, cam, W, H, maxDepth, confThreshold, (float)time,
+    k_splat_project<<<splatGrid(capacity, W, H), SPLAT_BS, 0, s>>>(sp.pos, reinterpret_cast<const float4*>(sp.time), sp.nrm, count, tinv, cam, W, H, maxDepth, confThreshold, (float)time,
                                                         (float)maxTime, (float)timeDelta, drawBase, rayTab, (unsigned long long*)key);
 }
 }
```

After: 731.6, median of 6. About the same (+0.2%).
